# geekieo/collaborative-deep-metric-learning

Measured on AMD Instinct MI355X. Metric: triplets/sec, higher is better.
Workload: dtype f32 values as 3 exact bf16 planes (hi + mid + lo == the f32 value), 6 bf16-MFMA plane products per f32 product, f32 accumulate

## Files before the change

### __graft_entry__.py

```python
import glob
import os
import subprocess
import sys

ROOT = os.path.dirname(os.path.abspath(__file__))
PKG = os.path.join(ROOT, "collaborative-deep-metric-learning_amd")
CSRC = os.path.join(PKG, "csrc")
LIB = os.path.join(PKG, "lib", "libcdml_hip.so")
if ROOT not in sys.path:
    sys.path.insert(0, ROOT)


def _stale(target, sources):
    if not os.path.exists(target):
        return True
    t = os.path.getmtime(target)
    return any(os.path.getmtime(s) > t for s in sources)


def _ids():
    import importlib.util
    spec = importlib.util.spec_from_file_location("_cdml_lib_ids", os.path.join(PKG, "_lib.py"))
    m = importlib.util.module_from_spec(spec)
    spec.loader.exec_module(m)
    return m.source_id, m.embedded_id


def _compile_objects(srcs, hdrs, objdir, hipcc, flags, force=False):
    from concurrent.futures import ThreadPoolExecutor
    os.makedirs(objdir, exist_ok=True)
    jobs = []
    import re
    for s in srcs:
        o = os.path.join(objdir, os.path.basename(s)[:-4] + ".o")
        inc = [os.path.join(os.path.dirname(s), m) for m in re.findall(r'#include "([^"]+\.hip)"', open(s).read())]
        if force or _stale(o, [s] + inc + hdrs):
            jobs.append([hipcc] + flags + ["-c", "-o", o, s])
    if jobs:
        print("[build] compiling %d of %d sources" % (len(jobs), len(srcs)), flush=True)

        def run(c):
            r = subprocess.run(c + ["-Rpass-analysis=kernel-resource-usage"], cwd=CSRC, stderr=subprocess.PIPE, text=True)
            o = c[c.index("-o") + 1]
            with open(o[:-2] + ".remarks", "w") as f:
                f.write(r.stderr)
            if r.returncode:
                sys.stderr.write("\n".join(ln for ln in r.stderr.splitlines() if "remark:" not in ln)[-4000:] + "\n")
            return r
        with ThreadPoolExecutor(max_workers=min(len(jobs), max(1, (os.cpu_count() or 2) - 1))) as ex:
            for r in ex.map(run, jobs):
                if r.returncode:
                    raise RuntimeError("hipcc failed: " + " ".join(r.args))
    objs = [os.path.join(objdir, os.path.basename(s)[:-4] + ".o") for s in srcs]
    _check_no_scratch(objs)
    return objs


HIPCC_FLAGS = ["--offload-arch=gfx950", "-O3", "-std=c++17", "-fPIC",
               "-Wno-array-bounds"]
NPAIR_KERNELS = ("k_npair", "k_mixed", "k_npdp")
IVF_F16_KERNELS = ("k_ivf_scan_f16", "k_ivf_refine")
IVF_FILTER_KERNELS = ("k_ivf_filter_f32", "k_ivf_filter_f16")
KNN_WRITER_KERNELS = ("k_line_sizes", "k_line_write")
IVF_PQ_KERNELS = ("k_ivf_scan_pq", "k_pq_encode")
IVF_PQR_KERNELS = ("k_ivf_scan_pqr", "k_pqr_encode")


def _check_no_scratch(objs):
    import re
    bad = []
    for o in objs:
        rem = o[:-2] + ".remarks"
        if not os.path.exists(rem):
            continue
        name = None
        for ln in open(rem):
            m = re.search(r"Function Name: (\S+)", ln)
            if m:
                name = m.group(1)
            m = re.search(r"ScratchSize \[bytes/lane\]: (\d+)", ln)
            if m and name and int(m.group(1)) > 0 and any(k in name for k in ("k_gemm",) + NPAIR_KERNELS + IVF_F16_KERNELS
                                                          + IVF_FILTER_KERNELS + KNN_WRITER_KERNELS + IVF_PQ_KERNELS
                                                          + IVF_PQR_KERNELS):
                bad.append("%s: %s bytes of scratch per lane (%s)" % (name, m.group(1), os.path.basename(o)))
    if bad:
        raise RuntimeError("kernels with a scratch frame (GEMMs: spills inside hand-counted vmcnt pipelines; N-pair launches "
                           "(k_npair / k_mixed / k_npdp): spills in bandwidth-bound passes):\n  " + "\n  ".join(bad))


def build(force=False, csrc=None, lib=None, objdir=None):
    variant = csrc is not None
    csrc = csrc or CSRC
    lib = lib or LIB
    objdir = objdir or os.path.join(ROOT, "build", "obj")
    srcs = sorted(glob.glob(os.path.join(csrc, "*.hip")))
    hdrs = glob.glob(os.path.join(csrc, "*.h")) + [os.path.join(ROOT, "include", "cdml.h")] \
        + glob.glob(os.path.join(ROOT, "include", "cdml_*.h"))
    source_id, embedded_id = _ids()
    sid = source_id(csrc, os.path.join(ROOT, "include", "cdml.h"))
    if force or embedded_id(lib) != sid:
        os.makedirs(os.path.dirname(lib), exist_ok=True)
        hipcc = os.environ.get("HIPCC", "/opt/rocm/bin/hipcc")
        flags = HIPCC_FLAGS + ["-I" + CSRC]
        objs = _compile_objects(srcs, hdrs, objdir, hipcc, flags, force)
        idsrc = os.path.join(objdir, "build_id.cpp")
        with open(idsrc, "w") as f:
            f.write('extern "C" const char *cdml_build_id(void) { return "CDML_BUILD_ID=%s"; }\n' % sid)
        subprocess.run([hipcc, "-O1", "-fPIC", "-c", "-o", idsrc[:-4] + ".o", idsrc], check=True)
        objs.append(idsrc[:-4] + ".o")
        cmd = [hipcc, "--offload-arch=gfx950", "-fPIC", "-shared", "-o", lib] + objs
        print("[build]", " ".join(cmd), flush=True)
        subprocess.run(cmd, check=True, cwd=csrc)
    if variant:
        return
    import cdml_amd
    from cdml_amd import _lib
    lib = _lib.load_library()
    assert lib.cdml_version() >= 1000
    for name in list(_lib.SIGNATURES) + list(_lib.SIGNATURES_MIXED) + list(_lib.SIGNATURES_DP) + list(_lib.SIGNATURES_BF16) \
            + list(_lib.SIGNATURES_HARDNEG) + list(_lib.SIGNATURES_WIDE) + list(_lib.SIGNATURES_NEGW) \
            + list(_lib.SIGNATURES_F8) + list(_lib.SIGNATURES_IVF) + list(_lib.SIGNATURES_IVF_F16) \
            + list(_lib.SIGNATURES_IVF_FILTER) + list(_lib.SIGNATURES_KNN_WRITER) + list(_lib.SIGNATURES_IVF_PQ) \
            + list(_lib.SIGNATURES_IVF_PQR):
        getattr(lib, name)
    assert lib.cdml_build_id().decode() == "CDML_BUILD_ID=" + sid
    print("[build] ok:", LIB, "version", lib.cdml_version(), lib.cdml_build_id().decode())


def smoke():
    import numpy as np
    import torch
    build()
    from cdml_amd import engine, train
    from oracle import sampler as osampler, synth as osynth, tower as otower

    dev = torch.device("cuda:0")
    N, F, H, D, B = 512, 96, 200, 32, 128
    table = engine.FeatureTable.synthetic(N, F, seed=0, device=dev)
    feats = osynth.features_philox(0, N, F, 0)
    assert np.array_equal(table.data[:, :F].cpu().numpy(), feats), "table differs"
    pairs_np = osynth.cowatch_pairs(N, 64, seed=0)
    pairs = torch.from_numpy(pairs_np).to(dev)
    idx = osampler.device_triplets_vec(pairs_np, N, 1234, 0, B)
    x = feats[idx.reshape(-1)]
    for precision in ("f32x3", "f32", "f16x2"):
        ts = train.TrainStep(table, pairs, B, hidden_size=H, output_size=D, margin=0.8, mode="uniform",
                             optimizer="adam", base_learning_rate=0.01, device=dev, precision=precision)
        W = [t.detach().cpu().numpy().copy() for t in ts.params.unpadded()]
        ts.step()
        torch.cuda.synchronize()
        assert np.array_equal(ts.idx.view(B, 3).cpu().numpy(), idx), "sampled indices differ"
        fwd, loss, grads = otower.train_step_grads(x, W, 0.8, np.float32)
        e = ts.ws.e[:, :D].cpu().numpy()
        assert np.abs(e - fwd["l2_norm"]).max() < 1e-5, "embeddings differ (%s)" % precision
        assert abs(ts.loss() - float(loss["hinge_loss"])) < 1e-5, "loss differs (%s)" % precision
        gW1 = ts.params.unpadded(grads=True)[0].cpu().numpy()
        assert np.abs(gW1 - grads["dW1"]).max() < 1e-5, "dW1 differs (%s)" % precision
        w1, _, _ = otower.adam_step(W[0], gW1, 0 * W[0], 0 * W[0], 1, 0.01)
        assert np.abs(ts.params.unpadded()[0].cpu().numpy() - w1).max() < 1e-6, "Adam update differs (%s)" % precision
        if precision == "f32x3":
            L = ts.layout
            w1t = ts.ws.W1T[:, :L.Fp].float() + ts.ws.W1T[:, L.Fp:2 * L.Fp].float() + ts.ws.W1T[:, 2 * L.Fp:].float()
            assert torch.equal(w1t, ts.params.W1.t()), "weight planes differ from the master weights"
        if precision == "f16x2":
            L, sw = ts.layout, ts.ws.scales.w1
            w1t = (ts.ws.W1T[:, :L.Fp].double() + ts.ws.W1T[:, L.Fp:2 * L.Fp].double()) / sw
            assert (w1t - ts.params.W1.t().double()).abs().max().item() <= 2.0 ** -22 * ts.params.W1.abs().max().item(), \
                "fp16 weight planes differ from the master weights"
        print("[smoke] %s ok: loss %.6f (oracle %.6f)" % (precision, ts.loss(), float(loss["hinge_loss"])))


if __name__ == "__main__":
    build(force="--force" in sys.argv)
    if "--smoke" in sys.argv:
        smoke()
```

### collaborative-deep-metric-learning_amd/_lib.py

```python
import ctypes as C
import os

_HERE = os.path.dirname(os.path.abspath(__file__))
_LIB_NAME = "libcdml_hip.so"


class CdmlError(RuntimeError):

    def __init__(self, code, message):
        super().__init__(f"cdml status {code}: {message}")
        self.code = code


def lib_path():
    return os.environ.get("CDML_LIB_PATH") or os.path.join(_HERE, "lib", _LIB_NAME)


def source_id(csrc=None, header=None):
    import glob
    import hashlib
    csrc = csrc or os.path.join(_HERE, "csrc")
    header = header or os.path.join(os.path.dirname(_HERE), "include", "cdml.h")
    files = sorted(glob.glob(os.path.join(csrc, "*.hip")) + glob.glob(os.path.join(csrc, "*.h")))
    if not files or not os.path.exists(header):
# ... 116 lines not shown
    "cdml_gather_rows_x3": (_i, [_p, _i64, _i64, _p, _i, _i, _i, _p, _i64, _p, _p]),
    "cdml_sample_gather_x3k": (_i, [_i, _p, _i64, _u64, _u64, _p, _i, _i64, _i64, _p, _i64, _i64, _i,
                                    _p, _p, _p, _i64, _i, _i64, _i64, _p, _p, _i64, _p]),
    "cdml_split_f32_bf16x3": (_i, [_p, _i64, _i, _i, _p, _i64, _i64, _i, _p]),
    "cdml_gemm_bf16x3_workspace": (_sz, [_i, _i, _i, _i, _i]),
    "cdml_gemm_bf16x3_nt": (_i, [_i, _p, _i64, _i64, _p, _i64, _i64, _i, _i, _i, _i, _p, _i64, _i64, _p, _p, _i64, _f,
                                 _p, _p, _sz, _p]),
    "cdml_gemm_bf16x3_tn": (_i, [_p, _i64, _i64, _p, _i64, _i64, _i, _i, _i, _i, _p, _i64, _p, _f, _p, _p, _sz, _p]),
    "cdml_split_f32_f16x2": (_i, [_p, _i64, _i, _i, _p, _i64, _i64, _i, _f, _p]),
    "cdml_gemm_f16x2_workspace": (_sz, [_i, _i, _i, _i]),
    "cdml_gemm_f16x2_nt": (_i, [_i, _p, _i64, _i64, _p, _i64, _i64, _i, _i, _i, _p, _i64, _i64, _p, _p, _i64, _f, _f, _f,
                                _p, _sz, _p]),
    "cdml_gemm_f16x2_tn": (_i, [_p, _i64, _i64, _p, _i64, _i64, _i, _i, _i, _p, _i64, _f, _p, _f, _p, _sz, _p]),
    "cdml_interleave8_bf16x3": (_i, [_p, _i64, _i64, _i, _i, _p, _p]),
    "cdml_gemm_bf16x3_tnk": (_i, [_p, _i, _i, _p, _i, _i, _i, _i, _i, _p, _i64, _p, _p, _sz, _p]),
    "cdml_transpose_to_bf16": (_i, [_i, _p, _i64, _i, _i, _p, _i64, _p]),
    "cdml_cast_f32_bf16": (_i, [_p, _i64, _i, _i, _p, _i64, _p]),
    "cdml_colsum_workspace_floats": (_sz, [_i, _i]),
    "cdml_colsum": (_i, [_i, _p, _i64, _i, _i, _p, _p, _p]),
    "cdml_fill_uniform_table_f16": (_i, [_p, _i64, _i64, _i, _i64, _u64, _p]),
    "cdml_gather_rows_f16": (_i, [_p, _i64, _i64, _i64, _p, _i, _i, _p, _i64, _p, _p]),
    "cdml_ew_combine": (_i, [_i, _p, _i64, _p, _i64, _i, _i, _p, _i64, _p]),
    "cdml_ew_fusion_bwd": (_i, [_i, _p, _i64, _p, _i64, _p, _i64, _i, _i, _f, _p, _i64, _p, _i64, _p]),
    "cdml_lrelu_bwd": (_i, [_p, _i64, _p, _i64, _i, _i, _f, _p, _i64, _p]),
    "cdml_adam_step": (_i, [_p, _p, _p, _p, _i64, _f, _p, _f, _f, _f, _i64, _p, _i, _p, _p]),
    "cdml_adam_matrix_bf16": (_i, [_p, _p, _p, _p, _i, _i, _f, _p, _f, _f, _f, _i64, _p, _p, _i64, _p, _i64,
                                   _p, _p, _p, _p, _i, _i, _p, _p]),
    "cdml_adam_matrix_planes": (_i, [_p, _p, _p, _p, _i, _i, _f, _p, _f, _f, _f, _i64, _p, _p, _i64, _i64, _p, _i64, _i64,
                                     _p, _p, _p, _p, _i, _i, _p, _p]),
    "cdml_adam_matrix_h2": (_i, [_p, _p, _p, _p, _i, _i, _f, _p, _f, _f, _f, _i64, _p, _p, _i64, _i64, _p, _i64, _i64, _f,
                                 _p, _p, _p, _p, _i, _i, _p, _p]),
    "cdml_table_adam_rows": (_i, [_p, _i64, _i64, _i64, _i, _p, _i, _p, _i64, _p, _p, _p, _p, _f, _f, _p, _f, _f, _f,
                                  _i64, _p, _p]),
    "cdml_grad_prepare": (_i, [_p, _p, _i64, _f, _f, _p, _p, _p]),
    "cdml_momentum_step": (_i, [_p, _p, _p, _i64, _f, _p, _f, _i, _p]),
    "cdml_lars_scratch_floats": (_sz, []),
    "cdml_lars_step": (_i, [_p, _p, _p, _i64, _f, _p, _f, _f, _f, _f, _p, _p]),
    "cdml_lars_multi_scratch_floats": (_sz, []),
    "cdml_lars_multi": (_i, [_p, _p, _p, _p, _p, _i, _f, _p, _f, _f, _f, _f, _p, _p, _p, _p, _p]),
    "cdml_lars_multi_norms": (_i, [_p, _p, _p, _p, _i, _p, _p]),
    "cdml_lars_matrix": (_i, [_p, _p, _p, _p, _p, _i, _i, _i, _i, _i, _f, _p, _f, _f, _f, _f, _p, _p, _p, _i64, _i64, _p,
                              _i64, _i64, _i, _p, _p, _p]),
    "cdml_momentum_matrix": (_i, [_p, _p, _p, _i, _i, _f, _p, _f, _i, _p, _i64, _i64, _p, _i64, _i64, _i, _p, _p, _p, _i,
                                  _p, _p, _p]),
    "cdml_lars_matrix_h2": (_i, [_p, _p, _p, _p, _p, _i, _i, _i, _i, _i, _f, _p, _f, _f, _f, _f, _p, _p, _p, _i64, _i64, _p,
                                 _i64, _i64, _f, _p, _p, _p]),
    "cdml_momentum_matrix_h2": (_i, [_p, _p, _p, _i, _i, _f, _p, _f, _i, _p, _i64, _i64, _p, _i64, _i64, _f, _p, _p, _p, _i,
                                     _p, _p, _p]),
}

SIGNATURES_MIXED = {
    "cdml_npair_mixed_workspace": (_sz, [_i, _i]),
    "cdml_npair_mixed_stats": (_i, [_p, _i64, _p, _i, _i64, _i64, _p, _i, _p, _f, _p, _f, _i, _p, _p, _p, _sz, _p]),
    "cdml_npair_mixed_grad_x3": (_i, [_p, _i64, _p, _i, _i64, _i64, _p, _i, _p, _f, _p, _f, _i, _p, _p, _i64, _i64, _p]),
    "cdml_npair_mixed_grad_f32": (_i, [_p, _i64, _p, _i, _i64, _i64, _p, _i, _p, _f, _p, _f, _i, _p, _p, _i64, _p]),
    "cdml_npair_mixed_split_x3": (_i, [_p, _i64, _i, _i, _p, _i64, _i64, _p, _i64, _i64, _p, _i64, _i64, _i64, _p]),
}

SIGNATURES_DP = {
    "cdml_npair_dp_workspace": (_sz, [_i, _i]),
    "cdml_npair_dp_local_stats": (_i, [_p, _i64, _p, _i, _i, _i, _f, _i, _p, _p, _p, _sz, _p]),
    "cdml_npair_dp_col_fold": (_i, [_p, _i, _i, _p, _p]),
    "cdml_npair_dp_stats": (_i, [_p, _i64, _i, _i, _i, _f, _i, _p, _p, _p, _sz, _p]),
    "cdml_npair_dp_grad_x3": (_i, [_p, _i64, _p, _i, _i, _i, _f, _i, _p, _p, _p, _i64, _i64, _p]),
    "cdml_npair_dp_grad_f32": (_i, [_p, _i64, _p, _i, _i, _i, _f, _i, _p, _p, _p, _i64, _p]),
    "cdml_npair_dp_pos_fold": (_i, [_p, _i64, _i, _i, _i, _p, _i64, _p]),
}

SIGNATURES_BF16 = {
    "cdml_npair_operands_bf16": (_i, [_p, _i64, _i, _i, _p, _i64, _p, _i64, _p, _i64, _p]),
    "cdml_npair_grad_bf16": (_i, [_p, _i64, _p, _i, _f, _i, _p, _p, _i64, _p]),
    "cdml_npair_logq_grad_bf16": (_i, [_p, _i64, _p, _i, _p, _f, _i, _p, _p, _i64, _p]),
    "cdml_npair_memory_grad_bf16": (_i, [_p, _i64, _p, _i, _i64, _p, _i, _f, _i, _p, _p, _i64, _p]),
    "cdml_npair_memory_logq_grad_bf16": (_i, [_p, _i64, _p, _i, _i64, _p, _p, _i, _f, _i, _p, _p, _i64, _p]),
    "cdml_npair_memory_push_bf16": (_i, [_p, _i64, _p, _i, _i, _u64, _p, _i64, _i, _p, _i64, _p, _p, _i64, _p, _i64, _p]),
}

SIGNATURES_HARDNEG = {
    "cdml_sample_listed": (_i, [_p, _i64, _i64, _u64, _u64, _p, _i, _i64, _i64, _p, _i64, _i, _u64, _p, _p, _p]),
    "cdml_sample_gather_listed": (_i, [_p, _i64, _u64, _u64, _p, _i, _i64, _i64, _p, _i64, _i64, _i, _p, _i64, _i, _u64,
                                       _p, _p, _p, _i64, _i, _i64, _i64, _i64, _p, _p]),
    "cdml_sample_gather_listed_x3": (_i, [_p, _i64, _u64, _u64, _p, _i, _i64, _i64, _p, _i64, _i64, _i, _p, _i64, _i, _u64,
                                          _p, _p, _p, _i64, _i, _i64, _i64, _i64, _p, _p, _i64, _p]),
    "cdml_sample_gather_listed_f16": (_i, [_p, _i64, _u64, _u64, _p, _i, _i64, _i64, _p, _i64, _i64, _i, _p, _i64, _i, _u64,
                                           _p, _p, _p, _i64, _i, _i64, _i64, _i64, _p, _p]),
}

SIGNATURES_NEGW = {
    "cdml_sample_weighted": (_i, [_p, _i64, _i64, _u64, _u64, _p, _i, _i64, _i64, _p, _i64, _p, _i, _p, _p, _p]),
    "cdml_sample_gather_weighted": (_i, [_p, _i64, _u64, _u64, _p, _i, _i64, _i64, _p, _i64, _i64, _i, _p, _i64, _p, _i,
                                         _p, _p, _p, _i64, _i, _i64, _i64, _i64, _p, _p]),
    "cdml_sample_gather_weighted_x3": (_i, [_p, _i64, _u64, _u64, _p, _i, _i64, _i64, _p, _i64, _i64, _i, _p, _i64, _p, _i,
                                            _p, _p, _p, _i64, _i, _i64, _i64, _i64, _p, _p, _i64, _p]),
    "cdml_sample_gather_weighted_f16": (_i, [_p, _i64, _u64, _u64, _p, _i, _i64, _i64, _p, _i64, _i64, _i, _p, _i64, _p, _i,
                                             _p, _p, _p, _i64, _i, _i64, _i64, _i64, _p, _p]),
    "cdml_npair_mixed_stats_nb": (_i, [_p, _i64, _p, _i, _i64, _i64, _p, _i, _p, _p, _p, _f, _i, _p, _p, _p, _sz, _p]),
    "cdml_npair_mixed_grad_x3_nb": (_i, [_p, _i64, _p, _i, _i64, _i64, _p, _i, _p, _p, _p, _f, _i, _p, _p, _i64, _i64, _p]),
    "cdml_npair_mixed_grad_f32_nb": (_i, [_p, _i64, _p, _i, _i64, _i64, _p, _i, _p, _p, _p, _f, _i, _p, _p, _i64, _p]),
    "cdml_negw_bias": (_i, [_p, _i64, _p, _i, _f, _p, _p]),
}

SIGNATURES_WIDE = {
    "cdml_gemm_bf16x3_tn_kb": (_i, [_p, _i64, _i64, _p, _i, _i, _i, _i, _i, _p, _i64, _p, _p, _sz, _p]),
}

SIGNATURES_F8 = {
    "cdml_sample_gather_f8": (_i, [_i, _p, _i64, _u64, _u64, _p, _i, _i64, _i64, _p, _i64, _i64, _i,
                                   _p, _p, _p, _i64, _i, _i64, _i64, _p, _p]),
    "cdml_sample_gather_listed_f8": (_i, [_p, _i64, _u64, _u64, _p, _i, _i64, _i64, _p, _i64, _i64, _i, _p, _i64, _i, _u64,
                                          _p, _p, _p, _i64, _i, _i64, _i64, _i64, _p, _p]),
    "cdml_sample_gather_weighted_f8": (_i, [_p, _i64, _u64, _u64, _p, _i, _i64, _i64, _p, _i64, _i64, _i, _p, _i64, _p, _i,
                                            _p, _p, _p, _i64, _i, _i64, _i64, _i64, _p, _p]),
    "cdml_gather_rows_f8": (_i, [_p, _i64, _i64, _i64, _p, _i, _i, _p, _i64, _p, _p]),
    "cdml_quantize_rows_f8_f32": (_i, [_p, _i64, _i64, _i, _p, _i64, _i64, _p, _p]),
    "cdml_quantize_rows_f8_f16": (_i, [_p, _i64, _i64, _i, _p, _i64, _i64, _p, _p]),
}

SIGNATURES_IVF = {
    "cdml_ivf_centroid_sums": (_i, [_p, _i64, _p, _p, _i, _i, _p, _i64, _p]),
    "cdml_ivf_scan_f32": (_i, [_p, _i64, _i, _p, _p, _p, _p, _i64, _p, _i, _p, _i, _p, _p]),
    "cdml_ivf_merge": (_i, [_p, _p, _p, _p, _i, _i, _p, _p, _p, _p, _i, _p, _p, _p]),
}

SIGNATURES_IVF_F16 = {
    "cdml_ivf_scan_f16": (_i, [_p, _i64, _i, _p, _p, _p, _p, _i64, _p, _i, _p, _i, _p, _p]),
    "cdml_ivf_refine": (_i, [_p, _i64, _i, _p, _i64, _i64, _i, _p, _i, _i, _p, _p, _p]),
}

_IVF_FILTER_ARGS = [_p, _i64, _i, _p, _p, _p, _p, _p, _p, _i64, _p, _p, _p, _i, _p, _i, _p, _i, _p]
SIGNATURES_IVF_FILTER = {
    "cdml_ivf_filter_f32": (_i, _IVF_FILTER_ARGS),
    "cdml_ivf_filter_f16": (_i, list(_IVF_FILTER_ARGS)),
}

SIGNATURES_KNN_WRITER = {
    "cdml_f32_shortest": (_i, [_f, C.c_char_p]),
    "cdml_knn_line_sizes": (_i, [_p, _i64, _p, _i64, _i64, _i, _i, _p, _i64, _i64, _p, _p, _p]),
    "cdml_knn_line_write": (_i, [_p, _i64, _p, _i64, _i64, _i, _i, _p, _p, _i64, _i64, _p, _p, _i64, _p]),
}

SIGNATURES_IVF_PQ = {
    "cdml_pq_encode": (_i, [_p, _i64, _i64, _p, _i, _i, _p, _i64, _p, _i64, _p]),
    "cdml_pq_lut": (_i, [_p, _i64, _i, _p, _i, _i, _p, _p]),
    "cdml_ivf_pq_tile": (_i, [_i, _p, _p]),
    "cdml_ivf_scan_pq": (_i, [_p, _i, _p, _p, _p, _p, _i64, _p, _i, _p, _i, _p, _p]),
}

SIGNATURES_IVF_PQR = {
    "cdml_pqr_encode": (_i, [_p, _i64, _i64, _p, _i64, _i, _p, _p, _i, _i, _p, _i64, _p, _i64, _p]),
    "cdml_ivf_slot_dots": (_i, [_p, _i64, _i, _p, _i64, _i, _p, _p, _i, _p, _p]),
    "cdml_ivf_scan_pqr": (_i, [_p, _i, _p, _p, _p, _p, _p, _i64, _p, _i, _p, _i, _p, _p]),
}

_lib = None


def load_library():
    global _lib
    if _lib is not None:
        return _lib
    path = lib_path()
    if not os.path.exists(path):
        raise CdmlError(-2, f"{path} not found: build it with "
                            f"`python -c 'import __graft_entry__ as g; g.build()'` "
                            f"(there is no CPU fallback)")
    import torch
    lib = C.CDLL(path)
    for name, (res, args) in (list(SIGNATURES.items()) + list(SIGNATURES_MIXED.items()) + list(SIGNATURES_DP.items())
                               + list(SIGNATURES_BF16.items()) + list(SIGNATURES_HARDNEG.items()) + list(SIGNATURES_WIDE.items())
                               + list(SIGNATURES_NEGW.items()) + list(SIGNATURES_F8.items()) + list(SIGNATURES_IVF.items())
                               + list(SIGNATURES_IVF_F16.items()) + list(SIGNATURES_IVF_FILTER.items())
                               + list(SIGNATURES_KNN_WRITER.items()) + list(SIGNATURES_IVF_PQ.items())
                               + list(SIGNATURES_IVF_PQR.items())):
        fn = getattr(lib, name)
        fn.restype = res
        fn.argtypes = args
    want = source_id()
    if want is not None and not os.environ.get("CDML_LIB_PATH") and os.environ.get("CDML_ALLOW_STALE_LIB") != "1":
        have = lib.cdml_build_id().decode()
        if have != "CDML_BUILD_ID=" + want:
            raise CdmlError(-2, f"{path} was built from other sources ({have}; this tree is {want}): rebuild it with "
                                f"`python -c 'import __graft_entry__ as g; g.build()'`")
    _lib = lib
    return lib


def call(name, *args):
    lib = load_library()
    rc = getattr(lib, name)(*args)
    if rc != 0:
        raise CdmlError(rc, lib.cdml_last_error().decode("utf-8", "replace"))
    return rc
```

### collaborative-deep-metric-learning_amd/csrc/gemm_bf16.h

```cpp
#pragma once
#include "common.h"

namespace cdml {

using bf16 = __bf16;

enum { BE_BIAS_LRELU_BF16 = 0, BE_BIAS_LRELU_F32 = 1, BE_MASK_BF16 = 2, BE_F32 = 3, BE_BIAS_LRELU_BF16_BITS = 4,
       BE_MASKBITS_BF16 = 5,
       BE_BIAS_LRELU_X3 = 6, BE_MASK_X3 = 7,
       BE_ROWBIAS_LRELU_X3 = 8,
       BE_BIAS_LRELU_X3_BITS = 9, BE_MASKBITS_X3 = 10,
       BE_MINE_X3 = 11,
       BE_MASKBITS_X3_KI = 12,
       BE_KNN_X3 = 13,
       BE_RANK_X3 = 14 };

struct alignas(16) MineCand { float out_d; int out_c; float in_d; int in_c; };

struct BArgs {
  const bf16 *A; int64_t lda;
  const bf16 *B; int64_t ldb;
  void *C; int64_t ldc;
  const float *bias;
  const bf16 *aux; int64_t ldaux;
  float alpha;
  int M, N, K;
  int k_per_split;
  int64_t slab_stride;
  int tiles_m, tiles_n;
  float *colsum_partial;
  uint8_t *mask_out; int64_t ldmask;
  int aux_bits;
  int x3_tpp;
  int x3_products;
  int64_t x3_plane_a, x3_plane_b, x3_plane_c;
  int grid_tiles, narrow_first;
  int stagger_lead;
  int c_kint;
  const float *mine_sqn; const int32_t *mine_ids; const float *mine_dp; MineCand *mine_out; int64_t mine_ld;
  const float *knn_qsq, *knn_bsq, *knn_tau; int32_t *knn_cnt; uint2 *knn_cand; int knn_cap, knn_col0, knn_n_valid;
  const float *rank_qsq, *rank_tau; const int32_t *rank_pos, *rank_self; int32_t *rank_cnt; float *rank_tau_out;
  float out_scale, c_scale;
};

bool gemm_bf16_256_usable(int M, int N, int K, int64_t lda, int64_t ldb);
int launch_gemm_bf16_256(const BArgs &g, int epilogue, int splits, hipStream_t stream);
int launch_gemm_bf16_256_x3(const BArgs &g, bool tn, int epilogue, int splits, hipStream_t stream);
int launch_gemm_f16x2_256(const BArgs &g, bool tn, int epilogue, int splits, hipStream_t stream);
int launch_gemm_f16x2_mine(const BArgs &g, hipStream_t stream);
int launch_gemm_f16x2_knn(const BArgs &g, hipStream_t stream);
int launch_gemm_x3_mine(const BArgs &g, hipStream_t stream);
int launch_gemm_x3_knn(const BArgs &g, hipStream_t stream);
int launch_gemm_x3_rank(const BArgs &g, hipStream_t stream);
int launch_gemm_f16x2_rank(const BArgs &g, hipStream_t stream);
int launch_gemm_x3_tnk(const BArgs &g, int splits, hipStream_t stream);
int launch_gemm_x3_tnkb(const BArgs &g, int splits, hipStream_t stream);

bool gemm_bf16_k256_usable(int M, int N, int K, int64_t lda, int64_t ldb, int64_t ldc, int64_t ldaux, bool has_aux);
int launch_gemm_bf16_k256(const BArgs &g, hipStream_t stream);

bool gemm_bf16_tn_usable(int M, int N, int K, int64_t lda, int64_t ldb);
int launch_gemm_bf16_tn(const BArgs &g, int splits, hipStream_t stream);

size_t gemm_bf16_tn2_workspace(int M1, int N1, int M2, int N2, int K);
int launch_gemm_bf16_tn2(const BArgs &g1, const BArgs &g2, float *db1, float *db2, void *workspace,
                         size_t workspace_bytes, hipStream_t stream);

}
```

### collaborative-deep-metric-learning_amd/csrc/gemm_bf16_256.hip

```cpp
#include "gemm_tile.h"
#include <stdlib.h>

#ifndef CDML_BF16_MFMA_DEFAULT
#define CDML_BF16_MFMA_DEFAULT 16
#endif

namespace cdml {
namespace {

template <class V>
__device__ __forceinline__ void run_tile(const BArgs &g, const int tm, const int m0, const int n0, const int k_begin,
                                         const int n_ktiles, void *c_base, const int64_t c_ld, const int c_row0,
                                         const int c_col0, float *cs_row, const int64_t cs_grp_stride,
                                         unsigned char *smem) {
  constexpr bool TN = V::TN, S16 = V::S16, X3 = V::X3, F6 = V::F6, NTCS = V::NTCS, NARROW = V::NARROW, WIDEB = V::WIDEB;
  constexpr int EPI = V::EPI;
  constexpr bool KIA = V::KIA, KIB = V::KIB, kSwap = V::kSwap, kR6 = V::kR6, kFast6 = V::kFast6;
  constexpr bool kRowBias = V::kRowBias, kBiasEpi = V::kBiasEpi, kMaskEpi = V::kMaskEpi, kPlanes = V::kPlanes;
  const int t = threadIdx.x;
  const int lane = t & 63;
  const int wave = __builtin_amdgcn_readfirstlane(t >> 6);
  const int grp = wave >> 2, wc = wave & 3;
  const int l31 = lane & 31, h = lane >> 5;

  const int k_rows = X3 ? g.x3_tpp * kTileK : g.K;
  const i32x4 srd_a = make_srd(g.A, KIA ? 3 * g.x3_plane_a * 2 : (int64_t)(TN ? k_rows : g.M) * g.lda * 2);
  const i32x4 srd_b = make_srd(g.B, KIB ? 3 * g.x3_plane_b * 2 : (int64_t)(TN ? k_rows : g.N) * g.ldb * 2);

  uint32_t va[2], vb[2];
#pragma unroll
  for (int i = 0; i < 2; ++i) {
    if constexpr (!TN) {
      const int r = (wave * 2 + i) * 8 + (lane >> 3);
      const int sc = (lane & 7) ^ ((r >> 1) & 7);
      const int row_a = NARROW ? r : (r >> 6) * 128 + (r & 63);
      const int col_b = (r >> 5) * 64 + (r & 31);
      va[i] = (uint32_t)(((int64_t)(m0 + row_a) * g.lda + sc * 8) * 2);
      vb[i] = (uint32_t)(((int64_t)(n0 + col_b) * g.ldb + sc * 8) * 2);
    } else {
      const int pc = wave * 2 + i;
      const int r = pc * 4 + (lane >> 4);
      const int sc = (lane & 15) ^ (((r & 3) << 2) | ((r >> 2) & 3));
      if constexpr (KIA) va[i] = (uint32_t)(((int64_t)(pc >> 1) * g.lda + (int64_t)(m0 + (pc & 1) * 64 + lane) * 8) * 2);
      else va[i] = (uint32_t)(((int64_t)r * g.lda + m0 + sc * 8) * 2);
      if constexpr (KIB) vb[i] = (uint32_t)(((int64_t)(pc >> 1) * g.ldb + (int64_t)(n0 + (pc & 1) * 64 + lane) * 8) * 2);
      else vb[i] = (uint32_t)(((int64_t)r * g.ldb + n0 + sc * 8) * 2);
    }
  }
  const uint32_t d_a = TN ? 256u : (uint32_t)(64 * g.lda * 2), d_b = TN ? 256u : (uint32_t)(32 * g.ldb * 2);
  const uint32_t lds_piece = __builtin_amdgcn_readfirstlane(lds_off(smem) + wave * 2048);

  const bool x3_kmajor = X3 && g.x3_products > 0;
  const float x3_inv = X3 ? __builtin_bit_cast(float, __builtin_amdgcn_readfirstlane(__builtin_bit_cast(
                                int, 1.0f / (float)(x3_kmajor ? g.x3_products : g.x3_tpp)))) : 0.f;
  const int x3_t0 = k_begin / kTileK;
  auto x3_div = [&](int v) { return __builtin_amdgcn_readfirstlane((int)(((float)v + 0.5f) * x3_inv)); };
  auto x3_where = [&](int v, int &sgm, int &w) {
    const int qd = x3_div(v);
    const int rem = v - qd * (x3_kmajor ? g.x3_products : g.x3_tpp);
    sgm = x3_kmajor ? rem : qd;
    w = x3_kmajor ? qd : rem;
  };
  auto x3_segment = [&](int v) { int sgm, w; x3_where(v, sgm, w); return sgm; };
  auto stage = [&](int img, int hh, int tile, int buf) {
    int64_t k_elems;
    if constexpr (X3) {
      int sgm, w;
      x3_where(x3_t0 + tile, sgm, w);
      const int plane = ((img == 0 ? 0x120100 : 0x102010) >> (4 * sgm)) & 3;
      k_elems = (int64_t)w * kTileK * (TN ? (img == 0 ? g.lda : g.ldb) : 1) + plane * (img == 0 ? g.x3_plane_a : g.x3_plane_b);
    } else {
      k_elems = (int64_t)(k_begin + tile * kTileK) * (TN ? (img == 0 ? g.lda : g.ldb) : 1);
    }
    const uint32_t kb = tile < n_ktiles ? (uint32_t)(k_elems * 2) : 0x80000000u;
#pragma unroll
    for (int i = 0; i < 2; ++i) {
      const uint32_t voff = (img == 0 ? va[i] + hh * d_a : vb[i] + hh * d_b) + kb;
      dma(img == 0 ? srd_a : srd_b, voff, lds_piece + i * 1024 + img * (4 * IMG) + buf * (2 * IMG) + hh * IMG);
    }
  };

  const bool x3_run = X3 && !F6 && x3_kmajor;
  auto x3_pack = [&](int v) { const int qd = x3_div(v); return qd * 8 + (v - qd * g.x3_products); };
  auto x3_step = [&](int pos) { return ((pos & 7) + 1 == g.x3_products) ? (pos & ~7) + 8 : pos + 1; };
  int xp_c = 0, xp_a = 0, xp_b = 0;
  if (x3_run) { xp_c = x3_pack(x3_t0); xp_a = x3_pack(x3_t0 + 1); xp_b = x3_pack(x3_t0 + 2); }
  auto stage_pw = [&](int img, int hh, int plane, int w, int tile, int buf) {
    const int64_t k_elems = (int64_t)w * kTileK * (TN ? (img == 0 ? g.lda : g.ldb) : 1) +
                            plane * (img == 0 ? g.x3_plane_a : g.x3_plane_b);
    const uint32_t kb = tile < n_ktiles ? (uint32_t)(k_elems * 2) : 0x80000000u;
#pragma unroll
    for (int i = 0; i < 2; ++i) {
      const uint32_t voff = (img == 0 ? va[i] + hh * d_a : vb[i] + hh * d_b) + kb;
      dma(img == 0 ? srd_a : srd_b, voff, lds_piece + i * 1024 + img * (4 * IMG) + buf * (2 * IMG) + hh * IMG);
    }
  };

  const int x = (l31 >> 1) & 7;
  const unsigned char *a_rd = smem + (grp * 64 + l31) * 128;
  const unsigned char *b_rd = smem + 4 * IMG + (wc * 32 + l31) * 128;
  int sw[4];
#pragma unroll
  for (int ks = 0; ks < 4; ++ks) sw[ks] = ((2 * ks + h) ^ x) * 16;
  const int tq = (lane >> 2) & 3, tp = lane & 3, tmb = (lane >> 4) & 1;
  auto tr_off = [&](int c0, int sh) {
    const int row = 8 * h + 4 * sh + tq;
    const int swz = (tq << 2) | ((2 * h + sh) & 3);
    return 256 * row + 16 * ((c0 + tmb * 2 + (tp >> 1)) ^ swz) + 8 * (tp & 1);
  };
  int ta[2][2], tb[2];
#pragma unroll
  for (int sh = 0; sh < 2; ++sh) {
    ta[0][sh] = tr_off(grp * 8, sh);
    ta[1][sh] = tr_off(grp * 8 + 4, sh);
    tb[sh] = tr_off(wc * 4, sh);
  }
  auto tr_read = [&](const unsigned char *img, int off0, int off1) {
    const bf16x4 lo = __builtin_amdgcn_ds_read_tr16_b64_v4bf16(
        (__attribute__((address_space(3))) bf16x4 *)(img + off0));
    const bf16x4 hi = __builtin_amdgcn_ds_read_tr16_b64_v4bf16(
        (__attribute__((address_space(3))) bf16x4 *)(img + off1));
    return __builtin_shufflevector(lo, hi, 0, 1, 2, 3, 4, 5, 6, 7);
  };
  auto read_a = [&](int buf, int hh, int mi, int ks) {
    if constexpr (!TN)
      return *reinterpret_cast<const bf16x8 *>(a_rd + buf * (2 * IMG) + hh * IMG + mi * 4096 + sw[ks]);
    else
      return tr_read(smem + buf * (2 * IMG) + hh * IMG + ks * 4096, ta[mi][0], ta[mi][1]);
  };
  auto read_b = [&](int buf, int hh, int ks) {
    if constexpr (!TN)
      return *reinterpret_cast<const bf16x8 *>(b_rd + buf * (2 * IMG) + hh * IMG + sw[ks]);
    else
      return tr_read(smem + 4 * IMG + buf * (2 * IMG) + hh * IMG + ks * 4096, tb[0], tb[1]);
  };

  const int l15 = lane & 15, q16 = lane >> 4;
  const unsigned char *a16_rd = smem + (grp * 64 + l15) * 128;
  const unsigned char *b16_rd = smem + 4 * IMG + (wc * 32 + l15) * 128;
  const int sw16[2] = {((q16) ^ ((l15 >> 1) & 7)) * 16, ((4 + q16) ^ ((l15 >> 1) & 7)) * 16};
  auto tr_off16 = [&](int c0, int sh) {
    const int row = 8 * q16 + 4 * sh + tq;
    const int swz = (tq << 2) | ((2 * q16 + sh) & 3);
    return 256 * row + 16 * ((c0 + (tp >> 1)) ^ swz) + 8 * (tp & 1);
  };
  int ta16[4][2], tb16[2][2];
#pragma unroll
  for (int sh = 0; sh < 2; ++sh) {
#pragma unroll
    for (int rb = 0; rb < 4; ++rb) ta16[rb][sh] = tr_off16((WIDEB ? (grp * 2 + (wc >> 1)) * 4 : grp * 8) + 2 * rb, sh);
#pragma unroll
    for (int cb = 0; cb < 2; ++cb) tb16[cb][sh] = tr_off16(wc * 4 + 2 * cb, sh);
  }
  auto read_a16 = [&](int buf, int hh, int rb, int ks2) {
    if constexpr (!TN)
      return *reinterpret_cast<const bf16x8 *>(a16_rd + buf * (2 * IMG) + hh * IMG + rb * 2048 + sw16[ks2]);
    else
      return tr_read(smem + buf * (2 * IMG) + hh * IMG + ks2 * 8192, ta16[rb][0], ta16[rb][1]);
  };
  auto read_b16 = [&](int buf, int hh, int cb, int ks2) {
    if constexpr (!TN)
      return *reinterpret_cast<const bf16x8 *>(b16_rd + buf * (2 * IMG) + hh * IMG + cb * 2048 + sw16[ks2]);
    else
      return tr_read(smem + 4 * IMG + buf * (2 * IMG) + hh * IMG + ks2 * 8192, tb16[cb][0], tb16[cb][1]);
  };

  f32x16 acc[S16 ? 1 : 4][S16 ? 1 : 2];
  f32x4 acc16[S16 ? 8 : 1][S16 ? 4 : 1];
#pragma unroll
  for (int i = 0; i < (S16 ? 1 : 4); ++i)
#pragma unroll
    for (int j = 0; j < (S16 ? 1 : 2); ++j)
#pragma unroll
      for (int r = 0; r < 16; ++r) acc[i][j][r] = 0.f;
#pragma unroll
  for (int i = 0; i < (S16 ? 8 : 1); ++i)
#pragma unroll
    for (int j = 0; j < (S16 ? 4 : 1); ++j) acc16[i][j] = f32x4{0.f, 0.f, 0.f, 0.f};
  bf16x8 fbx[WIDEB ? 16 : 1];
  float csw[WIDEB ? 8 : 1];
#pragma unroll
  for (int i = 0; i < (WIDEB ? 8 : 1); ++i) csw[i] = 0.f;
  bf16x8 fa[2][4], fb0[4], fb1[4];

  float cs[2] = {0.f, 0.f};
  float cs16[4] = {0.f, 0.f, 0.f, 0.f};
  const bool cs_on = (TN || (NTCS && X3 && S16)) && cs_row != nullptr;
  const int cs_period = 2 * g.tiles_m;
  const int cs_owner = (2 * tm + grp + cs_period - (k_begin / kTileK) % cs_period) % cs_period;
  auto dot_sum = [&](const bf16x8 &f, float acc) {
#ifdef CDML_F16X2
    const half8 hf = __builtin_bit_cast(half8, f);
    const half2v one = {(_Float16)1.0f, (_Float16)1.0f};
#pragma unroll
    for (int e = 0; e < 4; ++e) {
      const half2v pr = {hf[2 * e], hf[2 * e + 1]};
      acc = __builtin_amdgcn_fdot2(pr, one, acc, false);
    }
#else
    using bf16x2 = __attribute__((ext_vector_type(2))) __bf16;
    const bf16x2 one = {(__bf16)1.0f, (__bf16)1.0f};
#pragma unroll
    for (int e = 0; e < 4; ++e) {
      const bf16x2 pr = {f[2 * e], f[2 * e + 1]};
      acc = __builtin_amdgcn_fdot2_f32_bf16(pr, one, acc, false);
    }
#endif
    return acc;
  };
  int cs_left = __builtin_amdgcn_readfirstlane(cs_on ? cs_owner : 0x40000000);
  auto frag_sum = [&](const bf16x8 &f) {
    float s = 0.f;
#pragma unroll
    for (int e = 0; e < 8; ++e) s += (float)f[e];
    return s;
  };

  auto pin_a = [&]() {
    if constexpr (WIDEB)
      asm volatile("" : "+v"(fa[0][0]), "+v"(fa[0][1]), "+v"(fa[1][0]), "+v"(fa[1][1]));
    else
      asm volatile("" : "+v"(fa[0][0]), "+v"(fa[0][1]), "+v"(fa[0][2]), "+v"(fa[0][3]),
                        "+v"(fa[1][0]), "+v"(fa[1][1]), "+v"(fa[1][2]), "+v"(fa[1][3]));
  };
  auto pin_b = [&]() {
    if constexpr (WIDEB)
      asm volatile("" : "+v"(fbx[0]), "+v"(fbx[1]), "+v"(fbx[2]), "+v"(fbx[3]), "+v"(fbx[4]), "+v"(fbx[5]), "+v"(fbx[6]), "+v"(fbx[7]),
                        "+v"(fbx[8]), "+v"(fbx[9]), "+v"(fbx[10]), "+v"(fbx[11]), "+v"(fbx[12]), "+v"(fbx[13]), "+v"(fbx[14]), "+v"(fbx[15]));
    else
      asm volatile("" : "+v"(fb0[0]), "+v"(fb0[1]), "+v"(fb0[2]), "+v"(fb0[3]),
                        "+v"(fb1[0]), "+v"(fb1[1]), "+v"(fb1[2]), "+v"(fb1[3]));
  };
  auto load_b16 = [&](auto rd) {
    if constexpr (WIDEB) {
#pragma unroll
      for (int hh = 0; hh < 2; ++hh)
#pragma unroll
        for (int cb = 0; cb < 4; ++cb)
#pragma unroll
          for (int ks2 = 0; ks2 < 2; ++ks2) fbx[hh * 8 + cb * 2 + ks2] = rd(hh, cb, ks2);
    } else {
#pragma unroll
      for (int cb = 0; cb < 2; ++cb)
#pragma unroll
        for (int ks2 = 0; ks2 < 2; ++ks2) {
          fb0[2 * cb + ks2] = rd(0, cb, ks2);
          fb1[2 * cb + ks2] = rd(1, cb, ks2);
        }
    }
  };
  auto load_a16 = [&](auto rd) {
#pragma unroll
    for (int ks2 = 0; ks2 < 2; ++ks2)
#pragma unroll
      for (int rb = 0; rb < (WIDEB ? 2 : 4); ++rb) fa[ks2][rb] = rd(rb, ks2);
  };
  auto sum_b16 = [&](auto add) {
    if constexpr (WIDEB) {
#pragma unroll
      for (int hc = 0; hc < 8; ++hc)
#pragma unroll
        for (int ks2 = 0; ks2 < 2; ++ks2) csw[hc] = add(fbx[hc * 2 + ks2], csw[hc]);
    } else {
#pragma unroll
      for (int cb = 0; cb < 2; ++cb)
#pragma unroll
        for (int ks2 = 0; ks2 < 2; ++ks2) {
          cs16[cb] = add(fb0[2 * cb + ks2], cs16[cb]);
          cs16[2 + cb] = add(fb1[2 * cb + ks2], cs16[2 + cb]);
        }
    }
  };
  auto mfma16 = [&](const int r0) {
    __builtin_amdgcn_s_setprio(1);
    if constexpr (WIDEB) {
#pragma unroll
      for (int ks2 = 0; ks2 < 2; ++ks2)
#pragma unroll
        for (int rb = 0; rb < 2; ++rb)
#pragma unroll
          for (int hh = 0; hh < 2; ++hh)
#pragma unroll
            for (int cb = 0; cb < 4; ++cb)
              acc16[r0 + 2 * hh + rb][cb] = CDML_MFMA16(fa[ks2][rb], fbx[hh * 8 + cb * 2 + ks2], acc16[r0 + 2 * hh + rb][cb]);
    } else {
#pragma unroll
      for (int ks2 = 0; ks2 < 2; ++ks2)
#pragma unroll
        for (int rb = 0; rb < 4; ++rb)
#pragma unroll
          for (int cb = 0; cb < 2; ++cb) {
            if constexpr (kSwap) {
              acc16[r0 + rb][cb] = CDML_MFMA16(fb0[2 * cb + ks2], fa[ks2][rb], acc16[r0 + rb][cb]);
              acc16[r0 + rb][2 + cb] = CDML_MFMA16(fb1[2 * cb + ks2], fa[ks2][rb], acc16[r0 + rb][2 + cb]);
            } else {
              acc16[r0 + rb][cb] = CDML_MFMA16(fa[ks2][rb], fb0[2 * cb + ks2], acc16[r0 + rb][cb]);
              acc16[r0 + rb][2 + cb] = CDML_MFMA16(fa[ks2][rb], fb1[2 * cb + ks2], acc16[r0 + rb][2 + cb]);
            }
          }
    }
    __builtin_amdgcn_s_setprio(0);
  };
  auto do_tile2_s16 = [&](const int buf, const int tile) {
    load_b16([&](int hh, int cb, int ks2) { return read_b16(buf, hh, cb, ks2); });
    load_a16([&](int rb, int ks2) { return read_a16(buf, 0, rb, ks2); });
    if (X3 && x3_run) {
      const int pl = (0x120100 >> (4 * (xp_a & 7))) & 3;
      stage_pw(0, 0, pl, xp_a >> 3, tile + 1, buf ^ 1);
      stage_pw(0, 1, pl, xp_a >> 3, tile + 1, buf ^ 1);
    } else {
      stage(0, 0, tile + 1, buf ^ 1);
      stage(0, 1, tile + 1, buf ^ 1);
    }
    asm volatile("s_waitcnt vmcnt(8)" ::: "memory");
    pin_b();
    pin_a();
    const bool cs_mine = cs_left == 0;
    cs_left = cs_mine ? cs_period - 1 : cs_left - 1;
    if (cs_mine && (!X3 || ((0xB >> (x3_run ? (xp_c & 7) : x3_segment(x3_t0 + tile))) & 1))) sum_b16(dot_sum);
    CDML_BARRIER();
    mfma16(0);
    CDML_BARRIER();
    load_a16([&](int rb, int ks2) { return read_a16(buf, 1, rb, ks2); });
    if (X3 && x3_run) {
      const int pl = (0x102010 >> (4 * (xp_b & 7))) & 3;
      stage_pw(1, 0, pl, xp_b >> 3, tile + 2, buf);
      stage_pw(1, 1, pl, xp_b >> 3, tile + 2, buf);
    } else {
      stage(1, 0, tile + 2, buf);
      stage(1, 1, tile + 2, buf);
    }
    asm volatile("s_waitcnt vmcnt(6)" ::: "memory");
    pin_a();
    CDML_BARRIER();
    mfma16(4);
    CDML_BARRIER();
    if (X3 && x3_run) { xp_c = x3_step(xp_c); xp_a = x3_step(xp_a); xp_b = x3_step(xp_b); }
  };
  auto step6 = [&](auto Sc, const int tile, const int w) {
    constexpr int S = decltype(Sc)::value;
    constexpr int PA[6] = {0, 0, 1, 0, 2, 1}, PB[6] = {0, 1, 0, 2, 0, 1};
    constexpr int buf = S & 1;
    constexpr bool skip_a = (S >= 1 && S <= 4) && PA[(S + 1) % 6] == PA[(S + 5) % 6];
    constexpr bool skip_b = (S <= 3) && PB[(S + 2) % 6] == PB[S];
    constexpr int SP = (S + 5) % 6;
    constexpr bool b_next_issued = !((SP <= 3) && PB[(SP + 2) % 6] == PB[SP]);
    load_b16([&](int hh, int cb, int ks2) { return read_b16(buf, hh, cb, ks2); });
    load_a16([&](int rb, int ks2) { return read_a16(buf, 0, rb, ks2); });
    if constexpr (!skip_a) {
      stage_pw(0, 0, PA[(S + 1) % 6], w + (S == 5 ? 1 : 0), tile + 1, buf ^ 1);
      stage_pw(0, 1, PA[(S + 1) % 6], w + (S == 5 ? 1 : 0), tile + 1, buf ^ 1);
    }
    asm volatile("s_waitcnt vmcnt(%0)" :: "n"(4 * (int)b_next_issued + 4 * (int)!skip_a) : "memory");
    pin_b();
    pin_a();
    if (cs_on && ((0xB >> S) & 1) && (tile % cs_period) == cs_owner)
      sum_b16([&](const bf16x8 &f, float sum) { return sum + frag_sum(f); });
    CDML_BARRIER();
    mfma16(0);
    CDML_BARRIER();
    load_a16([&](int rb, int ks2) { return read_a16(buf, 1, rb, ks2); });
    if constexpr (!skip_b) {
      stage_pw(1, 0, PB[(S + 2) % 6], w + (S >= 4 ? 1 : 0), tile + 2, buf);
      stage_pw(1, 1, PB[(S + 2) % 6], w + (S >= 4 ? 1 : 0), tile + 2, buf);
    }
    asm volatile("s_waitcnt vmcnt(%0)" :: "n"(2 * (int)!skip_a + 4 * (int)!skip_b) : "memory");
    pin_a();
    CDML_BARRIER();
    mfma16(4);
    CDML_BARRIER();
  };
  auto do_tile2 = [&](const int buf, const int tile) {
#pragma unroll
    for (int ks = 0; ks < 4; ++ks) fb0[ks] = read_b(buf, 0, ks);
#pragma unroll
    for (int ks = 0; ks < 4; ++ks) fb1[ks] = read_b(buf, 1, ks);
#pragma unroll
    for (int mi = 0; mi < 2; ++mi)
#pragma unroll
      for (int ks = 0; ks < 4; ++ks) fa[mi][ks] = read_a(buf, 0, mi, ks);
    stage(0, 0, tile + 1, buf ^ 1);
    stage(0, 1, tile + 1, buf ^ 1);
    asm volatile("s_waitcnt vmcnt(8)" ::: "memory");
    pin_b();
    pin_a();
    if (TN && cs_on && (tile % cs_period) == cs_owner && (!X3 || ((0xB >> x3_segment(x3_t0 + tile)) & 1))) {
#pragma unroll
      for (int ks = 0; ks < 4; ++ks) {
        cs[0] += frag_sum(fb0[ks]);
        cs[1] += frag_sum(fb1[ks]);
      }
    }
    CDML_BARRIER();
    __builtin_amdgcn_s_setprio(1);
#pragma unroll
    for (int ks = 0; ks < 4; ++ks)
#pragma unroll
      for (int mi = 0; mi < 2; ++mi) {
        acc[mi][0] = __builtin_amdgcn_mfma_f32_32x32x16_bf16(fa[mi][ks], fb0[ks], acc[mi][0], 0, 0, 0);
        acc[mi][1] = __builtin_amdgcn_mfma_f32_32x32x16_bf16(fa[mi][ks], fb1[ks], acc[mi][1], 0, 0, 0);
      }
    __builtin_amdgcn_s_setprio(0);
    CDML_BARRIER();
#pragma unroll
    for (int mi = 0; mi < 2; ++mi)
#pragma unroll
      for (int ks = 0; ks < 4; ++ks) fa[mi][ks] = read_a(buf, 1, mi, ks);
    stage(1, 0, tile + 2, buf);
    stage(1, 1, tile + 2, buf);
    asm volatile("s_waitcnt vmcnt(6)" ::: "memory");
    pin_a();
    CDML_BARRIER();
    __builtin_amdgcn_s_setprio(1);
#pragma unroll
    for (int ks = 0; ks < 4; ++ks)
#pragma unroll
      for (int mi = 0; mi < 2; ++mi) {
        acc[2 + mi][0] = __builtin_amdgcn_mfma_f32_32x32x16_bf16(fa[mi][ks], fb0[ks], acc[2 + mi][0], 0, 0, 0);
        acc[2 + mi][1] = __builtin_amdgcn_mfma_f32_32x32x16_bf16(fa[mi][ks], fb1[ks], acc[2 + mi][1], 0, 0, 0);
      }
    __builtin_amdgcn_s_setprio(0);
    CDML_BARRIER();
  };

  if constexpr (kR6) {
    constexpr int kPer = kF16 ? 3 : 6;
    const int n_per = n_ktiles / kPer;
    if (n_per > 0) {
      const int w_first = x3_t0 / kPer, w_last = w_first + n_per - 1;
      const uint32_t ws_a = KIA ? (uint32_t)(8 * g.lda * 2) : TN ? (uint32_t)(kTileK * g.lda * 2) : (uint32_t)(kTileK * 2);
      const uint32_t ws_b = KIB ? (uint32_t)(8 * g.ldb * 2) : TN ? (uint32_t)(kTileK * g.ldb * 2) : (uint32_t)(kTileK * 2);
      const uint32_t ps_a = (uint32_t)(g.x3_plane_a * 2), ps_b = (uint32_t)(g.x3_plane_b * 2);
      const unsigned char *b16r = smem + 6 * IMG + (wc * 32 + l15) * 128;
      int ta_w2[4][2], tb_w[2][2];
      if constexpr (TN && !KIA) {
#pragma unroll
        for (int sh = 0; sh < 2; ++sh)
#pragma unroll
          for (int rb = 0; rb < (WIDEB ? 2 : 4); ++rb) {
            ta_w2[rb][sh] = ta16[rb][sh] + 4 * IMG;
            asm volatile("" : "+v"(ta_w2[rb][sh]));
          }
      }
      if constexpr (TN && !KIB) {
#pragma unroll
        for (int sh = 0; sh < 2; ++sh)
#pragma unroll
          for (int cb = 0; cb < 2; ++cb) {
            tb_w[cb][sh] = tb16[cb][sh] + 6 * IMG;
            asm volatile("" : "+v"(tb_w[cb][sh]));
          }
      }
      const unsigned char *ka_rd = smem + (q16 * 128 + grp * 64 + l15) * 16;
      const unsigned char *kb_rd = smem + 6 * IMG + (q16 * 128 + (WIDEB ? (wc & 1) * 64 : wc * 32) + l15) * 16;
      auto rd_a = [&](int slot, int hh, int rb, int ks2) {
        if constexpr (!TN)
          return *reinterpret_cast<const bf16x8 *>(a16_rd + slot * 2 * IMG + hh * IMG + rb * 2048 + sw16[ks2]);
        else if constexpr (KIA)
          return *reinterpret_cast<const bf16x8 *>(ka_rd + slot * 2 * IMG + hh * IMG + ks2 * 8192 + rb * 256);
        else if (slot < 2)
          return tr_read(smem + slot * 2 * IMG + hh * IMG + ks2 * 8192, ta16[rb][0], ta16[rb][1]);
        else
          return tr_read(smem + hh * IMG + ks2 * 8192, ta_w2[rb][0], ta_w2[rb][1]);
      };
      auto rd_b = [&](int slot, int hh, int cb, int ks2) {
        if constexpr (!TN)
          return *reinterpret_cast<const bf16x8 *>(b16r + slot * 2 * IMG + hh * IMG + cb * 2048 + sw16[ks2]);
        else if constexpr (KIB)
          return *reinterpret_cast<const bf16x8 *>(kb_rd + slot * 2 * IMG + hh * IMG + ks2 * 8192 + cb * 256);
        else
          return tr_read(smem + slot * 2 * IMG + hh * IMG + ks2 * 8192, tb_w[cb][0], tb_w[cb][1]);
      };
      uint32_t va_h1[2] = {va[0] + d_a, va[1] + d_a}, vb_h1[2] = {vb[0] + d_b, vb[1] + d_b};
      auto issue = [&](int img, int pl, int hh, int slot, uint32_t kw) {
        const uint32_t so = (img == 0 ? pl * ps_a : pl * ps_b) + kw + ((img == 0 ? KIA : KIB) ? hh * 2048u : TN ? hh * 256u : 0u);
        const uint32_t dst = lds_piece + (img == 0 ? 0 : 6 * IMG) + slot * 2 * IMG + hh * IMG;
        const bool h1 = !TN && hh == 1;
        dma_s(img == 0 ? srd_a : srd_b, img == 0 ? (h1 ? va_h1[0] : va[0]) : (h1 ? vb_h1[0] : vb[0]), so, dst);
        dma_s(img == 0 ? srd_a : srd_b, img == 0 ? (h1 ? va_h1[1] : va[1]) : (h1 ? vb_h1[1] : vb[1]), so, dst + 1024);
      };
      if constexpr (kF16) {
      auto phase3 = [&](auto phc, auto parc, const uint32_t kwb_c, const uint32_t kwa_n, const uint32_t kwb_n, const bool own) {
        constexpr int PH = decltype(phc)::value, PAR = decltype(parc)::value;
        constexpr int S = PH >> 1, HALF = PH & 1;
        constexpr int PA3[3] = {0, 1, 0}, PB3[3] = {0, 0, 1};
        constexpr int SLOT_A3[2][2] = {{0, 1}, {2, 1}};
        constexpr int sa = SLOT_A3[PAR][PA3[S]];
        constexpr bool rdB = HALF == 0 && (S == 0 || S == 2);
        if constexpr (rdB) {
          constexpr int sb = PB3[S];
          load_b16([&](int hh, int cb, int ks2) { return rd_b(sb, hh, cb, ks2); });
        }
        load_a16([&](int rb, int ks2) { return rd_a(sa, HALF, rb, ks2); });
        constexpr int SCH = TN ? 0 : 1;
        if constexpr (SCH == 0 && PH == 0) { issue(1, 1, 0, 1, kwb_c); issue(1, 1, 1, 1, kwb_c); }
        if constexpr (SCH == 0 && PH == 1) { issue(0, 0, 0, SLOT_A3[PAR ^ 1][0], kwa_n); }
        if constexpr (SCH == 0 && PH == 2) { issue(0, 0, 1, SLOT_A3[PAR ^ 1][0], kwa_n); }
        if constexpr (SCH == 0 && PH == 3) { issue(1, 0, 0, 0, kwb_n); }
        if constexpr (SCH == 0 && PH == 4) { issue(1, 0, 1, 0, kwb_n); issue(0, 1, 0, 1, kwa_n); }
        if constexpr (SCH == 0 && PH == 5) { issue(0, 1, 1, 1, kwa_n); }
        if constexpr (SCH == 1 && PH == 0) { issue(1, 1, 0, 1, kwb_c); }
        if constexpr (SCH == 1 && PH == 1) { issue(1, 1, 1, 1, kwb_c); issue(0, 0, 0, SLOT_A3[PAR ^ 1][0], kwa_n); }
        if constexpr (SCH == 1 && PH == 2) { issue(0, 0, 1, SLOT_A3[PAR ^ 1][0], kwa_n); }
        if constexpr (SCH == 1 && PH == 3) { issue(1, 0, 0, 0, kwb_n); issue(1, 0, 1, 0, kwb_n); }
        if constexpr (SCH == 1 && PH == 4) { issue(0, 1, 0, 1, kwa_n); }
        if constexpr (SCH == 1 && PH == 5) { issue(0, 1, 1, 1, kwa_n); }
        constexpr int VM3[2][6] = {{8, 8, 8, 6, 10, 4}, {6, 8, 8, 8, 10, 4}};
        asm volatile("s_waitcnt vmcnt(%0)" :: "n"(VM3[SCH][PH]) : "memory");
        if constexpr (rdB) pin_b();
        pin_a();
        if constexpr (rdB) {
          if (own) sum_b16(dot_sum);
        }
        CDML_BARRIER();
        mfma16(4 * HALF);
        CDML_BARRIER();
      };
      auto period3 = [&](auto parc, const int w, const bool own) {
        const int wn = min(w + 1, w_last);
        const uint32_t kwb_c = (uint32_t)w * ws_b, kwa_n = (uint32_t)wn * ws_a, kwb_n = (uint32_t)wn * ws_b;
        unroll<6>([&](auto phc) { phase3(phc, parc, kwb_c, kwa_n, kwb_n, own); });
      };
      {
        const uint32_t ka3 = (uint32_t)w_first * ws_a, kb3 = (uint32_t)w_first * ws_b;
        issue(0, 0, 0, 0, ka3); issue(0, 0, 1, 0, ka3);
        issue(1, 0, 0, 0, kb3); issue(1, 0, 1, 0, kb3);
        issue(0, 1, 0, 1, ka3); issue(0, 1, 1, 1, ka3);
        asm volatile("s_waitcnt vmcnt(4)" ::: "memory");
      }
      CDML_BARRIER();
      if (grp == 1) CDML_BARRIER();
      int cs_wait3 = __builtin_amdgcn_readfirstlane(cs_on ? (2 * tm + grp + cs_period - w_first % cs_period) % cs_period : 0x40000000);
      for (int w = w_first;;) {
        bool own = cs_wait3 == 0;
        cs_wait3 = own ? cs_period - 1 : cs_wait3 - 1;
        period3(std::integral_constant<int, 0>{}, w, own);
        if (++w > w_last) break;
        own = cs_wait3 == 0;
        cs_wait3 = own ? cs_period - 1 : cs_wait3 - 1;
        period3(std::integral_constant<int, 1>{}, w, own);
        if (++w > w_last) break;
      }
      } else if constexpr (!NARROW) {
      auto phase = [&](auto phc, auto parc, const uint32_t kwa_c, const uint32_t kwb_c, const uint32_t kwa_n,
                       const uint32_t kwb_n, const bool own) {
        constexpr int PH = decltype(phc)::value, PAR = decltype(parc)::value;
        constexpr int S = PH >> 1, HALF = PH & 1;
        constexpr int PA[6] = {0, 1, 2, 0, 1, 0}, PB[6] = {0, 0, 0, 1, 1, 2};
        constexpr int SLOT_A[2][3] = {{0, 1, 2}, {2, 1, 0}};
        constexpr int sa = SLOT_A[PAR][PA[S]];
        constexpr bool rdB = HALF == 0 && (S == 0 || S == 3 || S == 5);
        if constexpr (rdB) {
          constexpr int sb = (PB[S] & 1) ^ PAR;
          load_b16([&](int hh, int cb, int ks2) { return rd_b(sb, hh, cb, ks2); });
        }
        load_a16([&](int rb, int ks2) { return rd_a(sa, HALF, rb, ks2); });
        if constexpr (PH == 0) issue(0, 2, 1, SLOT_A[PAR][2], kwa_c);
        if constexpr (PH == 1) issue(1, 1, 0, 1 ^ PAR, kwb_c);
        if constexpr (PH == 2) issue(1, 1, 1, 1 ^ PAR, kwb_c);
        if constexpr (PH == 3) issue(1, 2, 0, PAR, kwb_c);
        if constexpr (PH == 4) issue(1, 2, 1, PAR, kwb_c);
        if constexpr (PH == 5) issue(0, 0, 0, SLOT_A[PAR ^ 1][0], kwa_n);
        if constexpr (PH == 6) issue(0, 0, 1, SLOT_A[PAR ^ 1][0], kwa_n);
        if constexpr (PH == 7) issue(1, 0, 0, PAR ^ 1, kwb_n);
        if constexpr (PH == 8) issue(1, 0, 1, PAR ^ 1, kwb_n);
        if constexpr (PH == 9) issue(0, 1, 0, 1, kwa_n);
        if constexpr (PH == 10) issue(0, 1, 1, 1, kwa_n);
        if constexpr (PH == 11) issue(0, 2, 0, SLOT_A[PAR ^ 1][2], kwa_n);
        constexpr int VM[12] = {8, 8, 8, 8, 8, 6, 8, 10, 12, 10, 12, 6};
        asm volatile("s_waitcnt vmcnt(%0)" :: "n"(VM[PH]) : "memory");
        if constexpr (rdB) pin_b();
        pin_a();
        if constexpr (rdB) {
          if constexpr (WIDEB) {
            if (own && (wc >> 1) == 0) sum_b16(dot_sum);
          } else {
            if (own) sum_b16(dot_sum);
          }
        }
        CDML_BARRIER();
        mfma16(4 * HALF);
        CDML_BARRIER();
      };
      auto period = [&](auto parc, const int w, const bool own) {
        const int wn = min(w + 1, w_last);
        const uint32_t kwa_c = (uint32_t)w * ws_a, kwb_c = (uint32_t)w * ws_b;
        const uint32_t kwa_n = (uint32_t)wn * ws_a, kwb_n = (uint32_t)wn * ws_b;
        unroll<12>([&](auto phc) { phase(phc, parc, kwa_c, kwb_c, kwa_n, kwb_n, own); });
      };
      {
        const uint32_t ka = (uint32_t)w_first * ws_a, kb_ = (uint32_t)w_first * ws_b;
        issue(0, 0, 0, 0, ka); issue(0, 0, 1, 0, ka);
        issue(1, 0, 0, 0, kb_); issue(1, 0, 1, 0, kb_);
        issue(0, 1, 0, 1, ka); issue(0, 1, 1, 1, ka);
        issue(0, 2, 0, 2, ka);
        asm volatile("s_waitcnt vmcnt(6)" ::: "memory");
      }
      CDML_BARRIER();
      if (grp == 1) CDML_BARRIER();
      int cs_wait = __builtin_amdgcn_readfirstlane(cs_on ? (2 * tm + grp + cs_period - w_first % cs_period) % cs_period : 0x40000000);
      for (int w = w_first;;) {
        bool own = cs_wait == 0;
        cs_wait = own ? cs_period - 1 : cs_wait - 1;
        period(std::integral_constant<int, 0>{}, w, own);
        if (++w > w_last) break;
        own = cs_wait == 0;
        cs_wait = own ? cs_period - 1 : cs_wait - 1;
        period(std::integral_constant<int, 1>{}, w, own);
        if (++w > w_last) break;
      }
      } else {
      auto rd_an = [&](int slot, int rb, int ks2) {
        return *reinterpret_cast<const bf16x8 *>(a16_rd + slot * IMG + rb * 2048 + sw16[ks2]);
      };
      const unsigned char *b16n = smem + 4 * IMG + (wc * 32 + l15) * 128;
      auto rd_bn = [&](int slot, int hh, int cb, int ks2) {
        return *reinterpret_cast<const bf16x8 *>(b16n + slot * 2 * IMG + hh * IMG + cb * 2048 + sw16[ks2]);
      };
      auto issue_n = [&](int img, int pl, int hh, int slot, uint32_t kw) {
        const uint32_t so = (img == 0 ? pl * ps_a : pl * ps_b) + kw;
        const uint32_t dst = lds_piece + (img == 0 ? slot * IMG : 4 * IMG + slot * 2 * IMG + hh * IMG);
        const bool h1 = hh == 1;
        dma_s(img == 0 ? srd_a : srd_b, img == 0 ? va[0] : (h1 ? vb_h1[0] : vb[0]), so, dst);
        dma_s(img == 0 ? srd_a : srd_b, img == 0 ? va[1] : (h1 ? vb_h1[1] : vb[1]), so, dst + 1024);
      };
      auto phase_n = [&](auto sc, auto parc, const uint32_t kwb_c, const uint32_t kwa_n, const uint32_t kwb_n) {
        constexpr int S = decltype(sc)::value, PAR = decltype(parc)::value;
        constexpr int PA[6] = {0, 1, 2, 0, 1, 0}, PB[6] = {0, 0, 0, 1, 1, 2};
        constexpr int NSLOT_A[2][3] = {{0, 1, 2}, {3, 2, 1}};
        constexpr bool rdB = S == 0 || S == 3 || S == 5;
        if constexpr (rdB) load_b16([&](int hh, int cb, int ks2) { return rd_bn(PB[S], hh, cb, ks2); });
        load_a16([&](int rb, int ks2) { return rd_an(NSLOT_A[PAR][PA[S]], rb, ks2); });
        if constexpr (S == 0) { issue_n(1, 2, 0, 2, kwb_c); issue_n(1, 2, 1, 2, kwb_c); }
        if constexpr (S == 1) { issue_n(1, 0, 0, 0, kwb_n); issue_n(0, 0, 0, NSLOT_A[PAR ^ 1][0], kwa_n); }
        if constexpr (S == 2) { issue_n(1, 0, 1, 0, kwb_n); }
        if constexpr (S == 3) { issue_n(0, 1, 0, NSLOT_A[PAR ^ 1][1], kwa_n); }
        if constexpr (S == 4) { issue_n(1, 1, 0, 1, kwb_n); issue_n(1, 1, 1, 1, kwb_n); }
        if constexpr (S == 5) { issue_n(0, 2, 0, NSLOT_A[PAR ^ 1][2], kwa_n); }
        constexpr int NVM[6] = {10, 8, 10, 12, 12, 8};
        asm volatile("s_waitcnt vmcnt(%0)" :: "n"(NVM[S]) : "memory");
        if constexpr (rdB) pin_b();
        pin_a();
        CDML_BARRIER();
        mfma16(0);
        CDML_BARRIER();
      };
      auto period_n = [&](auto parc, const int w) {
        const int wn = min(w + 1, w_last);
        const uint32_t kwb_c = (uint32_t)w * ws_b, kwa_n = (uint32_t)wn * ws_a, kwb_n = (uint32_t)wn * ws_b;
        unroll<6>([&](auto sc) { phase_n(sc, parc, kwb_c, kwa_n, kwb_n); });
      };
      {
        const uint32_t ka = (uint32_t)w_first * ws_a, kb_ = (uint32_t)w_first * ws_b;
        issue_n(1, 0, 0, 0, kb_); issue_n(0, 0, 0, 0, ka);
        issue_n(1, 0, 1, 0, kb_);
        issue_n(0, 1, 0, 1, ka);
        issue_n(1, 1, 0, 1, kb_); issue_n(1, 1, 1, 1, kb_);
        issue_n(0, 2, 0, 2, ka);
        asm volatile("s_waitcnt vmcnt(8)" ::: "memory");
      }
      CDML_BARRIER();
      if (grp == 1) CDML_BARRIER();
      for (int w = w_first;;) {
        period_n(std::integral_constant<int, 0>{}, w);
        if (++w > w_last) break;
        period_n(std::integral_constant<int, 1>{}, w);
        if (++w > w_last) break;
      }
      }
      if (grp == 0) CDML_BARRIER();
      asm volatile("s_waitcnt vmcnt(0)" ::: "memory");
      CDML_BARRIER();
    }
  } else {
  stage(1, 0, 0, 0); stage(1, 1, 0, 0); stage(0, 0, 0, 0); stage(0, 1, 0, 0);
  stage(1, 0, 1, 1); stage(1, 1, 1, 1);
  asm volatile("s_waitcnt vmcnt(6)" ::: "memory");
  CDML_BARRIER();
  if (grp == 1) CDML_BARRIER();
  if constexpr (kFast6) {
    {
      int w = x3_t0 / 6;
      for (int tile = 0; tile < n_ktiles; tile += 6, ++w) {
        step6(std::integral_constant<int, 0>{}, tile, w);
        step6(std::integral_constant<int, 1>{}, tile + 1, w);
        step6(std::integral_constant<int, 2>{}, tile + 2, w);
        step6(std::integral_constant<int, 3>{}, tile + 3, w);
        step6(std::integral_constant<int, 4>{}, tile + 4, w);
        step6(std::integral_constant<int, 5>{}, tile + 5, w);
      }
    }
  } else {
    for (int tile = 0; tile < n_ktiles; tile += 2) {
      if constexpr (S16) {
        do_tile2_s16(0, tile);
        do_tile2_s16(1, tile + 1);
      } else {
        do_tile2(0, tile);
        do_tile2(1, tile + 1);
      }
    }
  }

  if (grp == 0) CDML_BARRIER();
  asm volatile("s_waitcnt vmcnt(0)" ::: "memory");
  CDML_BARRIER();
  }

  if (TN && cs_on && !S16) {
#pragma unroll
    for (int ct = 0; ct < 2; ++ct) {
      const float v = cs[ct] + __shfl_xor(cs[ct], 32, 64);
      if (h == 0) cs_row[grp * cs_grp_stride + ct * 128 + wc * 32 + l31] = v;
    }
  }
  if (!TN && cs_on && S16) {
#pragma unroll
    for (int cbt = 0; cbt < 4; ++cbt) {
      float v = cs16[cbt] + __shfl_xor(cs16[cbt], 16, 64);
      v += __shfl_xor(v, 32, 64);
      if (q16 == 0) cs_row[grp * cs_grp_stride + wc * 64 + (cbt >> 1) * 32 + (cbt & 1) * 16 + l15] = v;
    }
  }
  if (WIDEB && cs_on) {
    if ((wc >> 1) == 0) {
#pragma unroll
      for (int hc = 0; hc < 8; ++hc) {
        float v = csw[hc] + __shfl_xor(csw[hc], 16, 64);
        v += __shfl_xor(v, 32, 64);
        if (q16 == 0) cs_row[grp * cs_grp_stride + (hc >> 2) * 128 + (wc & 1) * 64 + (hc & 3) * 16 + l15] = v;
      }
    }
  }
  if (TN && !WIDEB && cs_on && S16) {
#pragma unroll
    for (int cbt = 0; cbt < 4; ++cbt) {
      float v = cs16[cbt] + __shfl_xor(cs16[cbt], 16, 64);
      v += __shfl_xor(v, 32, 64);
      if (q16 == 0) cs_row[grp * cs_grp_stride + (cbt >> 1) * 128 + wc * 32 + (cbt & 1) * 16 + l15] = v;
    }
  }

  if constexpr (EPI == BE_MINE_X3) {
    int lane_e = lane;
    asm volatile("" : "+v"(lane_e));
    const int l15 = lane_e & 15, q16 = lane_e >> 4;
    const float inf = __builtin_huge_valf();
    const int cbase = n0 + wc * 64 + 4 * q16;
    f32x4 ncv[4];
    i32x4 idv[4];
#pragma unroll
    for (int cb = 0; cb < 4; ++cb) {
      ncv[cb] = *reinterpret_cast<const f32x4 *>(g.mine_sqn + cbase + cb * 16);
      idv[cb] = *reinterpret_cast<const i32x4 *>(g.mine_ids + cbase + cb * 16);
    }
    const int row_base = m0 + grp * 128 + l15;
    float sa8[8], dp8[8];
    int va8[8], vp8[8];
#pragma unroll
    for (int rbb = 0; rbb < 8; ++rbb) {
      const int i = min(row_base + rbb * 16, g.M - 1);
      sa8[rbb] = g.mine_sqn[2 * i];
      dp8[rbb] = g.mine_dp[i];
      va8[rbb] = g.mine_ids[2 * i];
      vp8[rbb] = g.mine_ids[2 * i + 1];
    }
    const float two_s = kF16 ? 2.0f * g.out_scale : 2.0f;
    auto closer = [](float d, int c, float bd, int bc) { return d < bd || (d == bd && c < bc); };
    auto farther = [](float d, int c, float bd, int bc) { return d > bd || (d == bd && c < bc); };
    MineCand *dst = g.mine_out + (int64_t)((n0 / kTileN) * 4 + wc) * g.mine_ld;
#pragma unroll
    for (int rbb = 0; rbb < 8; ++rbb) {
      const float sa = sa8[rbb], dpv = dp8[rbb];
      const int va = va8[rbb], vp = vp8[rbb];
      float od = inf, id_ = -inf;
      int oc = 0x7fffffff, ic = 0x7fffffff;
#pragma unroll
      for (int cb = 0; cb < 4; ++cb)
#pragma unroll
        for (int r = 0; r < 4; ++r) {
          const int c = cbase + cb * 16 + r;
          const float d = (sa + ncv[cb][r]) - two_s * acc16[rbb][cb][r];
          const int vid = idv[cb][r];
          if (vid != va && vid != vp && d > dpv && d < od) { od = d; oc = c; }
        }
#pragma unroll
      for (int off = 16; off < 64; off <<= 1) {
        const float od2 = __shfl_xor(od, off, 64);
        const int oc2 = __shfl_xor(oc, off, 64);
        if (closer(od2, oc2, od, oc)) { od = od2; oc = oc2; }
      }
      if (__ballot(oc == 0x7fffffff) != 0ull) {
#pragma unroll
        for (int cb = 0; cb < 4; ++cb)
#pragma unroll
          for (int r = 0; r < 4; ++r) {
            const int c = cbase + cb * 16 + r;
            const float d = (sa + ncv[cb][r]) - two_s * acc16[rbb][cb][r];
            const int vid = idv[cb][r];
            if (vid != va && vid != vp && d > id_) { id_ = d; ic = c; }
          }
#pragma unroll
        for (int off = 16; off < 64; off <<= 1) {
          const float id2 = __shfl_xor(id_, off, 64);
          const int ic2 = __shfl_xor(ic, off, 64);
          if (farther(id2, ic2, id_, ic)) { id_ = id2; ic = ic2; }
        }
        if (oc != 0x7fffffff) { id_ = -inf; ic = 0x7fffffff; }
      }
      const int i = row_base + rbb * 16;
      if (q16 == 0 && i < g.M) dst[i] = MineCand{od, oc, id_, ic};
    }
    return;
  }

  if constexpr (EPI == BE_KNN_X3) {
    int lane_e = lane;
    asm volatile("" : "+v"(lane_e));
    const int l15 = lane_e & 15, q16 = lane_e >> 4;
    const int cbase = n0 + wc * 64 + 4 * q16;
// ... 765 lines not shown
```

### collaborative-deep-metric-learning_amd/csrc/gemm_bf16x3.hip

```cpp
#include "gemm_bf16.h"
#include "../../include/cdml_x3_wide.h"
#include <stdlib.h>

namespace cdml {
namespace {

using bf16x4 = __attribute__((ext_vector_type(4))) __bf16;
using f32x4 = __attribute__((ext_vector_type(4))) float;
constexpr int kThreads = 256;

__device__ __forceinline__ void split3(float v, bf16 &h, bf16 &m, bf16 &l) {
  h = (bf16)v;
  const float r = v - (float)h;
  m = (bf16)r;
  l = (bf16)(r - (float)m);
}

__global__ void __launch_bounds__(kThreads)
k_split3(const float *__restrict__ src, int64_t lds_, int rows, int cols, bf16 *__restrict__ dst, int64_t ldd,
         int64_t plane) {
  const int c4n = cols >> 2;
  const int64_t total = (int64_t)rows * c4n;
  for (int64_t i = (int64_t)blockIdx.x * blockDim.x + threadIdx.x; i < total; i += (int64_t)gridDim.x * blockDim.x) {
    const int64_t r = i / c4n;
    const int c = (int)(i - r * c4n) * 4;
    const f32x4 v = *reinterpret_cast<const f32x4 *>(src + r * lds_ + c);
    bf16x4 h, m, l;
#pragma unroll
    for (int j = 0; j < 4; ++j) {
      bf16 a, b, c_;
      split3(v[j], a, b, c_);
      h[j] = a; m[j] = b; l[j] = c_;
    }
    bf16 *d = dst + r * ldd + c;
    *reinterpret_cast<bf16x4 *>(d) = h;
    *reinterpret_cast<bf16x4 *>(d + plane) = m;
    *reinterpret_cast<bf16x4 *>(d + 2 * plane) = l;
  }
}

__global__ void __launch_bounds__(kThreads)
k_split3_transpose(const float *__restrict__ src, int64_t lds_, int rows, int cols, bf16 *__restrict__ dst,
                   int64_t ldd, int64_t plane) {
  __shared__ float tile[64][65];
  const int r0 = blockIdx.y * 64, c0 = blockIdx.x * 64;
  const int tx = threadIdx.x & 63, ty = threadIdx.x >> 6;
  for (int j = ty; j < 64; j += 4) {
    const int r = r0 + j, c = c0 + tx;
    tile[j][tx] = (r < rows && c < cols) ? src[(int64_t)r * lds_ + c] : 0.f;
  }
  __syncthreads();
  for (int j = ty; j < 64; j += 4) {
    const int c = c0 + j, r = r0 + tx;
    if (c < cols && r < rows) {
      bf16 h, m, l;
      split3(tile[tx][j], h, m, l);
      bf16 *d = dst + (int64_t)c * ldd + r;
      d[0] = h; d[plane] = m; d[2 * plane] = l;
    }
  }
}

using half4v = __attribute__((ext_vector_type(4))) _Float16;
__device__ __forceinline__ void split2h(float v, float scale, _Float16 &h, _Float16 &l) {
  const float s = __builtin_amdgcn_fmed3f(v * scale, -65504.f, 65504.f);
  h = (_Float16)s;
  l = (_Float16)(s - (float)h);
}

__global__ void __launch_bounds__(kThreads)
k_split2h(const float *__restrict__ src, int64_t lds_, int rows, int cols, _Float16 *__restrict__ dst, int64_t ldd,
          int64_t plane, float scale) {
  const int c4n = cols >> 2;
  const int64_t total = (int64_t)rows * c4n;
  for (int64_t i = (int64_t)blockIdx.x * blockDim.x + threadIdx.x; i < total; i += (int64_t)gridDim.x * blockDim.x) {
    const int64_t r = i / c4n;
    const int c = (int)(i - r * c4n) * 4;
    const f32x4 v = *reinterpret_cast<const f32x4 *>(src + r * lds_ + c);
    half4v h, l;
#pragma unroll
    for (int j = 0; j < 4; ++j) {
      _Float16 a, b;
      split2h(v[j], scale, a, b);
      h[j] = a; l[j] = b;
    }
    _Float16 *d = dst + r * ldd + c;
    *reinterpret_cast<half4v *>(d) = h;
    *reinterpret_cast<half4v *>(d + plane) = l;
  }
}

__global__ void __launch_bounds__(kThreads)
k_split2h_transpose(const float *__restrict__ src, int64_t lds_, int rows, int cols, _Float16 *__restrict__ dst,
                    int64_t ldd, int64_t plane, float scale) {
  __shared__ float tile[64][65];
  const int r0 = blockIdx.y * 64, c0 = blockIdx.x * 64;
  const int tx = threadIdx.x & 63, ty = threadIdx.x >> 6;
  for (int j = ty; j < 64; j += 4) {
    const int r = r0 + j, c = c0 + tx;
    tile[j][tx] = (r < rows && c < cols) ? src[(int64_t)r * lds_ + c] : 0.f;
  }
  __syncthreads();
  for (int j = ty; j < 64; j += 4) {
    const int c = c0 + j, r = r0 + tx;
    if (c < cols && r < rows) {
      _Float16 h, l;
      split2h(tile[tx][j], scale, h, l);
      _Float16 *d = dst + (int64_t)c * ldd + r;
      d[0] = h; d[plane] = l;
    }
  }
}

int grid1d(int64_t n) {
  const int64_t b = (n + kThreads - 1) / kThreads;
  return (int)(b < 1 ? 1 : (b > 65535 * 16 ? 65535 * 16 : b));
}

bool x3_kmajor() {
  const char *e = getenv("CDML_X3_ORDER");
  return !(e && e[0] == 'p');
}

thread_local int tl_slab_steps = 0;
int x3_slab_steps() {
  const char *e = getenv("CDML_X3_SLAB_STEPS");
  return e && atoi(e) >= 12 ? atoi(e) / 6 * 6 : tl_slab_steps;
}

}
}

using namespace cdml;

extern "C" int cdml_split_f32_bf16x3(const float *src, int64_t ld_src, int rows, int cols, uint16_t *dst,
                                     int64_t ld_dst, int64_t plane, int transpose, cdml_stream_t stream) {
  CDML_REQUIRE(src && dst && rows > 0 && cols > 0, CDML_E_BADARG, "split_f32_bf16x3: bad argument");
  const int out_cols = transpose ? rows : cols;
  CDML_REQUIRE(plane >= out_cols && ld_dst >= 2 * plane + out_cols && ld_src >= cols, CDML_E_BADARG,
               "split_f32_bf16x3: planes of %d columns need plane >= %d and ld_dst >= 2 plane + %d", out_cols, out_cols, out_cols);
  hipStream_t s = (hipStream_t)stream;
  if (transpose) {
    hipLaunchKernelGGL(k_split3_transpose, dim3((cols + 63) / 64, (rows + 63) / 64), dim3(kThreads), 0, s, src, ld_src,
                       rows, cols, reinterpret_cast<bf16 *>(dst), ld_dst, plane);
  } else {
    CDML_REQUIRE((cols & 3) == 0 && (ld_src & 3) == 0 && (ld_dst & 3) == 0 && (plane & 3) == 0 && aligned16(src) &&
                     (reinterpret_cast<uintptr_t>(dst) & 7) == 0,
                 CDML_E_ALIGN, "split_f32_bf16x3: columns, strides and plane must be multiples of 4");
    hipLaunchKernelGGL(k_split3, dim3(grid1d((int64_t)rows * (cols / 4))), dim3(kThreads), 0, s, src, ld_src, rows, cols,
                       reinterpret_cast<bf16 *>(dst), ld_dst, plane);
  }
  return check_launch("split_f32_bf16x3");
}

extern "C" int cdml_split_f32_f16x2(const float *src, int64_t ld_src, int rows, int cols, uint16_t *dst, int64_t ld_dst,
                                    int64_t plane, int transpose, float scale, cdml_stream_t stream) {
  CDML_REQUIRE(src && dst && rows > 0 && cols > 0 && scale > 0.f, CDML_E_BADARG, "split_f32_f16x2: bad argument");
  const int out_cols = transpose ? rows : cols;
  CDML_REQUIRE(plane >= out_cols && ld_dst >= plane + out_cols && ld_src >= cols, CDML_E_BADARG,
               "split_f32_f16x2: planes of %d columns need plane >= %d and ld_dst >= plane + %d", out_cols, out_cols, out_cols);
  hipStream_t s = (hipStream_t)stream;
  if (transpose) {
    hipLaunchKernelGGL(k_split2h_transpose, dim3((cols + 63) / 64, (rows + 63) / 64), dim3(kThreads), 0, s, src, ld_src,
                       rows, cols, reinterpret_cast<_Float16 *>(dst), ld_dst, plane, scale);
  } else {
    CDML_REQUIRE((cols & 3) == 0 && (ld_src & 3) == 0 && (ld_dst & 3) == 0 && (plane & 3) == 0 && aligned16(src) &&
                     (reinterpret_cast<uintptr_t>(dst) & 7) == 0,
                 CDML_E_ALIGN, "split_f32_f16x2: columns, strides and plane must be multiples of 4");
    hipLaunchKernelGGL(k_split2h, dim3(grid1d((int64_t)rows * (cols / 4))), dim3(kThreads), 0, s, src, ld_src, rows, cols,
                       reinterpret_cast<_Float16 *>(dst), ld_dst, plane, scale);
  }
  return check_launch("split_f32_f16x2");
}

extern "C" int cdml_x3_slab_steps(int steps) {
  const int prev = tl_slab_steps;
  tl_slab_steps = steps >= 12 ? steps / 6 * 6 : 0;
  return prev;
}

extern "C" size_t cdml_gemm_bf16x3_workspace(int tn, int M, int N, int K, int products) {
  return x3_workspace_bytes(tn, M, N, K, products, tn ? 0 : x3_slab_steps());
}

extern "C" size_t cdml_gemm_f16x2_workspace(int tn, int M, int N, int K) {
  const size_t a = cdml_gemm_bf16x3_workspace(tn, M, N, K, 6), b = cdml_gemm_bf16x3_workspace(tn, M, N, K, 3);
  return a > b ? a : b;
}

namespace cdml {
namespace {
__device__ __forceinline__ void x3_colsum_block(const float *__restrict__ partial, int n_rows, int N, float *__restrict__ out,
                                                int blk, float scale) {
  __shared__ float red[16][17];
  const int cl = threadIdx.x & 15, rl = threadIdx.x >> 4;
  const int c = blk * 16 + cl;
  float s0 = 0.f, s1 = 0.f, s2 = 0.f, s3 = 0.f;
  if (c < N) {
    int r = rl;
    for (; r + 48 < n_rows; r += 64) {
      s0 += partial[(int64_t)r * N + c];
      s1 += partial[(int64_t)(r + 16) * N + c];
      s2 += partial[(int64_t)(r + 32) * N + c];
      s3 += partial[(int64_t)(r + 48) * N + c];
    }
    for (; r < n_rows; r += 16) s0 += partial[(int64_t)r * N + c];
  }
  red[rl][cl] = (s0 + s1) + (s2 + s3);
  __syncthreads();
  if (rl == 0 && c < N) {
    float t = red[0][cl];
#pragma unroll
    for (int j = 1; j < 16; ++j) t += red[j][cl];
    out[c] = t * scale;
  }
}

__global__ void __launch_bounds__(kThreads)
k_x3_sum_slabs(const float *__restrict__ slabs, int64_t slab_stride, int splits, int rows, int N,
               const float *__restrict__ bias, float alpha, float *__restrict__ out, int64_t ldo, int slab_blocks,
               const float *__restrict__ cs_partial, int cs_rows, float *__restrict__ cs_out, float cs_scale) {
  if ((int)blockIdx.x >= slab_blocks) {
    x3_colsum_block(cs_partial, cs_rows, N, cs_out, blockIdx.x - slab_blocks, cs_scale);
    return;
  }
  const int n4 = N >> 2;
  const int64_t total = (int64_t)rows * n4;
  for (int64_t i = (int64_t)blockIdx.x * blockDim.x + threadIdx.x; i < total; i += (int64_t)slab_blocks * blockDim.x) {
    const int64_t r = i / n4;
    const int c = (int)(i - r * n4);
    f32x4 s = reinterpret_cast<const f32x4 *>(slabs)[i];
    for (int z = 1; z < splits; ++z) s += reinterpret_cast<const f32x4 *>(slabs + (int64_t)z * slab_stride)[i];
    if (bias) {
      s += reinterpret_cast<const f32x4 *>(bias)[c];
      s.x = fmaxf(s.x, s.x * alpha); s.y = fmaxf(s.y, s.y * alpha);
      s.z = fmaxf(s.z, s.z * alpha); s.w = fmaxf(s.w, s.w * alpha);
    }
    reinterpret_cast<f32x4 *>(out + r * ldo)[c] = s;
  }
}

int x3_sum_slabs(const char *entry, const char *stage, const BArgs &g, const KSplitPlan &p, const void *slabs, const float *bias,
                 float alpha, float *C, int64_t ldc, float *colsum, float cs_scale, hipStream_t s) {
  const int sb = slabs ? grid1d((int64_t)g.M * g.N / 4) : 0, cb = colsum ? (g.N + 15) / 16 : 0;
  hipLaunchKernelGGL(k_x3_sum_slabs, dim3(sb + cb), dim3(kThreads), 0, s, static_cast<const float *>(slabs), g.slab_stride,
                     p.splits, g.M, g.N, bias, alpha, C, ldc, sb, g.colsum_partial, (int)p.cs_rows, colsum, cs_scale);
  const hipError_t e = hipGetLastError();
  return e == hipSuccess ? CDML_OK : fail(CDML_E_HIP, "%s %s: %s", entry, stage, hipGetErrorString(e));
}

int x3_run_tn(const char *entry, BArgs &g, const KSplitPlan &p, int (*launch)(const BArgs &, int, hipStream_t), float *C, int64_t ldc,
              const float *bias, float alpha, float *colsum, float cs_scale, void *workspace, size_t workspace_bytes, hipStream_t s) {
  CDML_REQUIRE(p.need == 0 || (workspace && workspace_bytes >= p.need && aligned16(workspace)), CDML_E_BADARG,
               "%s: workspace of %zu bytes required (cdml_gemm_bf16x3_workspace)", entry, p.need);
  g.K = p.ktiles * 64;
  g.tiles_m = g.M / 256; g.tiles_n = g.N / 256;
  g.k_per_split = p.per * 64;
  g.slab_stride = (int64_t)g.M * g.N;
  g.C = p.slabs ? workspace : static_cast<void *>(C);
  g.ldc = p.slabs ? g.N : ldc;
  g.colsum_partial = colsum ? reinterpret_cast<float *>(static_cast<char *>(workspace) + p.slab_bytes) : nullptr;
  const int rc = launch(g, p.splits, s);
  if (rc || !(p.slabs || colsum)) return rc;
  return x3_sum_slabs(entry, "combine", g, p, p.slabs ? workspace : nullptr, bias, alpha, C, ldc, colsum, cs_scale, s);
}
}
}

static int gemm_x3_nt_impl(bool f16, float out_scale, float c_scale, int epilogue, const uint16_t *A, int64_t lda, int64_t plane_a,
                           const uint16_t *B, int64_t ldb, int64_t plane_b, int M, int N, int K, int products, void *C,
                           int64_t ldc, int64_t plane_c, const float *bias, const uint16_t *aux,
                           int64_t ldaux, float alpha, float *colsum, void *workspace,
                           size_t workspace_bytes, cdml_stream_t stream) {
  CDML_REQUIRE(A && B && C && M > 0 && N > 0 && K > 0, CDML_E_BADARG, "gemm_bf16x3_nt: bad argument");
  const int np1 = f16 ? 1 : 2;
  CDML_REQUIRE(!f16 || (products == 3 && epilogue != BE_MASKBITS_X3_KI && epilogue != BE_ROWBIAS_LRELU_X3 && !colsum &&
                        out_scale > 0.f && c_scale > 0.f),
               CDML_E_UNSUPPORTED, "gemm_f16x2_nt: epilogues 1, 3, 6, 7, 9, 10, positive scales, no column sums");
  const bool kint_out = epilogue == BE_MASKBITS_X3_KI;
  const bool bits_out = epilogue == BE_BIAS_LRELU_X3_BITS, bits_in = epilogue == BE_MASKBITS_X3 || (kint_out && aux);
  if (bits_out) epilogue = BE_BIAS_LRELU_X3;
  if (bits_in || kint_out) epilogue = BE_MASK_X3;
  CDML_REQUIRE(epilogue == BE_BIAS_LRELU_F32 || epilogue == BE_F32 || epilogue == BE_BIAS_LRELU_X3 || epilogue == BE_MASK_X3 ||
                   epilogue == BE_ROWBIAS_LRELU_X3,
               CDML_E_BADARG, "gemm_bf16x3_nt: epilogue must be 1, 3, 6, 7, 8, 9, 10 or 12");
  CDML_REQUIRE(!(bits_out || bits_in) || (aux && N % 8 == 0 && ldaux >= N / 8), CDML_E_BADARG,
               "gemm_bf16x3_nt: epilogues 9 / 10 need the bitmask in aux (ldaux >= N / 8 bytes)");
  CDML_REQUIRE(products == 3 || products == 6, CDML_E_BADARG, "gemm_bf16x3_nt: products must be 3 or 6");
  CDML_REQUIRE(N % 256 == 0 && K % 64 == 0, CDML_E_UNSUPPORTED,
               "gemm_bf16x3_nt: N must be a multiple of 256 and K of 64, got N=%d K=%d", N, K);
  CDML_REQUIRE(aligned16(A) && aligned16(B) && aligned16(C) && !(lda & 7) && !(ldb & 7) && !(plane_a & 7) && !(plane_b & 7) &&
                   plane_a >= K && plane_b >= K && lda >= np1 * plane_a + K && ldb >= np1 * plane_b + K,
               CDML_E_ALIGN, "gemm_bf16x3_nt: 16-B aligned bases, strides multiples of 8, ld >= 2 plane + K (fp16 form: plane + K)");
  const bool planes_out = epilogue == BE_BIAS_LRELU_X3 || epilogue == BE_MASK_X3 || epilogue == BE_ROWBIAS_LRELU_X3;
  CDML_REQUIRE(kint_out ? (M % 8 == 0 && !(ldc & 7) && ldc >= N && plane_c >= (int64_t)(M / 8) * ldc * 8 &&
                           (int64_t)3 * plane_c * 2 < ((int64_t)1 << 32))
                        : planes_out ? (!(ldc & 7) && !(plane_c & 7) && plane_c >= N && ldc >= np1 * plane_c + N) : (!(ldc & 3) && ldc >= N),
               CDML_E_ALIGN, "gemm_bf16x3_nt: ldc (plane outputs: ldc and plane_c multiples of 8, ldc >= 2 plane_c + N; epilogue 12: M a "
               "multiple of 8, ldc = columns per row group >= N, plane_c >= M ldc)");
  CDML_REQUIRE(epilogue != BE_MASK_X3 || !aux || bits_in || (aligned16(aux) && !(ldaux & 7) && ldaux >= N), CDML_E_ALIGN,
               "gemm_bf16x3_nt: aux must be 16-B aligned with ldaux a multiple of 8");
  CDML_REQUIRE((epilogue != BE_BIAS_LRELU_F32 && epilogue != BE_BIAS_LRELU_X3 && epilogue != BE_ROWBIAS_LRELU_X3) || bias,
               CDML_E_BADARG, "gemm_bf16x3_nt: bias required");
  CDML_REQUIRE(!colsum || (M % 256 == 0 && products == 6 && epilogue == BE_F32), CDML_E_UNSUPPORTED,
               "gemm_bf16x3_nt: colsum (sum over k of B[n][k]) goes with epilogue 3, M a multiple of 256 and six products");
  CDML_REQUIRE(((int64_t)M + 256) * lda * 2 < ((int64_t)1 << 31) && (int64_t)N * ldb * 2 < ((int64_t)1 << 31), CDML_E_UNSUPPORTED,
               "gemm_bf16x3_nt: an operand exceeds the 2 GiB buffer-descriptor range");
  BArgs g{};
  g.A = reinterpret_cast<const bf16 *>(A); g.lda = lda;
  g.B = reinterpret_cast<const bf16 *>(B); g.ldb = ldb;
  g.C = C; g.ldc = ldc; g.bias = bias; g.alpha = alpha;
  g.aux = reinterpret_cast<const bf16 *>(aux); g.ldaux = ldaux;
  if (bits_out) { g.mask_out = reinterpret_cast<uint8_t *>(const_cast<uint16_t *>(aux)); g.ldmask = ldaux; g.aux = nullptr; g.ldaux = 0; }
  g.aux_bits = bits_in ? 1 : 0;
  g.c_kint = kint_out ? 1 : 0;
  g.M = M; g.N = N;
  g.x3_tpp = K / 64; g.x3_plane_a = plane_a; g.x3_plane_b = plane_b; g.x3_plane_c = plane_c;
  g.x3_products = (f16 || x3_kmajor()) ? products : 0;
  g.out_scale = out_scale; g.c_scale = c_scale;
  CDML_REQUIRE(products * g.x3_tpp % 2 == 0, CDML_E_UNSUPPORTED, "gemm_bf16x3_nt: products * K / 64 must be even");
  const KSplitPlan p = x3_plan_nt(M, N, K, products, f16, planes_out, colsum != nullptr, planes_out ? 0 : x3_slab_steps(), 6,
                                  workspace != nullptr);
  g.K = p.ktiles * 64; g.k_per_split = g.K;
  g.tiles_m = (M + 255) / 256; g.tiles_n = N / 256;
  hipStream_t s = (hipStream_t)stream;
  auto launch = [&](int epi, int n_splits) {
    return f16 ? launch_gemm_f16x2_256(g, false, epi, n_splits, s) : launch_gemm_bf16_256_x3(g, false, epi, n_splits, s);
  };
  CDML_REQUIRE(!p.slabs || (workspace_bytes >= p.need && aligned16(workspace)), CDML_E_BADARG,
               "gemm_bf16x3_nt: the slab form needs a 16-B aligned workspace of %zu bytes (cdml_gemm_bf16x3_workspace); pass "
               "NULL for the single-pass form", p.need);
  if (colsum) {
    CDML_REQUIRE(workspace && aligned16(workspace) && workspace_bytes >= p.need, CDML_E_BADARG,
                 "gemm_bf16x3_nt: colsum needs a workspace (cdml_gemm_bf16x3_workspace)");
    g.colsum_partial = reinterpret_cast<float *>(static_cast<char *>(workspace) + p.slab_bytes);
  }
  if (!p.slabs) {
    const int rc = launch(epilogue, 1);
    if (rc || !colsum) return rc;
    return x3_sum_slabs("gemm_bf16x3_nt", "bias gradient", g, p, nullptr, nullptr, 0.f, nullptr, 0, colsum, 1.0f, s);
  }
  g.k_per_split = p.per * 64;
  g.slab_stride = (int64_t)M * N;
  g.C = workspace; g.ldc = N;
  const int rc = launch(BE_F32, p.splits);
  if (rc) return rc;
  return x3_sum_slabs("gemm_bf16x3_nt", "combine", g, p, workspace, epilogue == BE_BIAS_LRELU_F32 ? bias : nullptr, alpha,
                      static_cast<float *>(C), ldc, colsum, 1.0f, s);
}

extern "C" int cdml_gemm_bf16x3_nt(int epilogue, const uint16_t *A, int64_t lda, int64_t plane_a, const uint16_t *B,
                                   int64_t ldb, int64_t plane_b, int M, int N, int K, int products, void *C,
                                   int64_t ldc, int64_t plane_c, const float *bias, const uint16_t *aux,
                                   int64_t ldaux, float alpha, float *colsum, void *workspace,
                                   size_t workspace_bytes, cdml_stream_t stream) {
  return gemm_x3_nt_impl(false, 1.0f, 1.0f, epilogue, A, lda, plane_a, B, ldb, plane_b, M, N, K, products, C, ldc, plane_c, bias, aux,
                         ldaux, alpha, colsum, workspace, workspace_bytes, stream);
}

extern "C" int cdml_gemm_f16x2_nt(int epilogue, const uint16_t *A, int64_t lda, int64_t plane_a, const uint16_t *B,
                                  int64_t ldb, int64_t plane_b, int M, int N, int K, void *C, int64_t ldc, int64_t plane_c,
                                  const float *bias, const uint16_t *aux, int64_t ldaux, float alpha, float out_scale,
                                  float c_scale, void *workspace, size_t workspace_bytes, cdml_stream_t stream) {
  return gemm_x3_nt_impl(true, out_scale, c_scale, epilogue, A, lda, plane_a, B, ldb, plane_b, M, N, K, 3, C, ldc, plane_c, bias, aux,
                         ldaux, alpha, nullptr, workspace, workspace_bytes, stream);
}

static int gemm_x3_tn_impl(bool f16, float out_scale, float cs_scale, const uint16_t *A, int64_t lda, int64_t plane_a,
                           const uint16_t *B, int64_t ldb, int64_t plane_b, int M, int N, int K, int products, float *C, int64_t ldc,
                           const float *bias, float alpha, float *colsum, void *workspace,
                           size_t workspace_bytes, cdml_stream_t stream) {
  CDML_REQUIRE(A && B && C && M > 0 && N > 0 && K > 0, CDML_E_BADARG, "gemm_bf16x3_tn: bad argument");
  const int np1 = f16 ? 1 : 2;
  CDML_REQUIRE(!f16 || (products == 3 && out_scale > 0.f && cs_scale > 0.f), CDML_E_BADARG, "gemm_f16x2_tn: positive scales");
  CDML_REQUIRE(products == 3 || products == 6, CDML_E_BADARG, "gemm_bf16x3_tn: products must be 3 or 6");
  CDML_REQUIRE(M % 256 == 0 && N % 256 == 0 && K % 128 == 0, CDML_E_UNSUPPORTED,
               "gemm_bf16x3_tn: M, N must be multiples of 256 and K of 128, got M=%d N=%d K=%d", M, N, K);
  CDML_REQUIRE(aligned16(A) && aligned16(B) && aligned16(C) && !(lda & 7) && !(ldb & 7) && !(plane_a & 7) && !(plane_b & 7) &&
                   !(ldc & 3) && plane_a >= M && plane_b >= N && lda >= np1 * plane_a + M && ldb >= np1 * plane_b + N && ldc >= N,
               CDML_E_ALIGN, "gemm_bf16x3_tn: 16-B aligned bases, strides multiples of 8, ld >= 2 plane + columns");
  CDML_REQUIRE((int64_t)K * lda * 2 < ((int64_t)1 << 31) && (int64_t)K * ldb * 2 < ((int64_t)1 << 31), CDML_E_UNSUPPORTED,
               "gemm_bf16x3_tn: an operand exceeds the 2 GiB buffer-descriptor range");
  BArgs g{};
  g.A = reinterpret_cast<const bf16 *>(A); g.lda = lda;
  g.B = reinterpret_cast<const bf16 *>(B); g.ldb = ldb;
  g.M = M; g.N = N;
  g.x3_tpp = K / 64; g.x3_plane_a = plane_a; g.x3_plane_b = plane_b;
  g.x3_products = (f16 || x3_kmajor()) ? products : 0;
  g.out_scale = out_scale; g.c_scale = 1.0f;
  const KSplitPlan p = x3_plan_tn(M, N, K, products, x3_tn_period(products, g.x3_products != 0, f16), bias != nullptr, colsum != nullptr);
  const auto launch = f16 ? +[](const BArgs &a, int splits, hipStream_t s) { return launch_gemm_f16x2_256(a, true, BE_F32, splits, s); }
                          : +[](const BArgs &a, int splits, hipStream_t s) { return launch_gemm_bf16_256_x3(a, true, BE_F32, splits, s); };
  return x3_run_tn("gemm_bf16x3_tn", g, p, launch, C, ldc, bias, alpha, colsum, cs_scale, workspace, workspace_bytes, (hipStream_t)stream);
}

extern "C" int cdml_gemm_bf16x3_tn(const uint16_t *A, int64_t lda, int64_t plane_a, const uint16_t *B, int64_t ldb,
                                   int64_t plane_b, int M, int N, int K, int products, float *C, int64_t ldc,
                                   const float *bias, float alpha, float *colsum, void *workspace,
                                   size_t workspace_bytes, cdml_stream_t stream) {
  return gemm_x3_tn_impl(false, 1.0f, 1.0f, A, lda, plane_a, B, ldb, plane_b, M, N, K, products, C, ldc, bias, alpha, colsum, workspace,
                         workspace_bytes, stream);
}

extern "C" int cdml_gemm_f16x2_tn(const uint16_t *A, int64_t lda, int64_t plane_a, const uint16_t *B, int64_t ldb,
                                  int64_t plane_b, int M, int N, int K, float *C, int64_t ldc, float out_scale, float *colsum,
                                  float colsum_scale, void *workspace, size_t workspace_bytes, cdml_stream_t stream) {
  return gemm_x3_tn_impl(true, out_scale, colsum_scale, A, lda, plane_a, B, ldb, plane_b, M, N, K, 3, C, ldc, nullptr, 0.f, colsum,
                         workspace, workspace_bytes, stream);
}

namespace cdml {
namespace {

__global__ void __launch_bounds__(kThreads)
k_mine_prep(const float *__restrict__ e_in, float *__restrict__ e_out, int64_t lde, const float *__restrict__ z, int64_t ldz,
            int B, int D, bf16 *__restrict__ e3, int64_t ld3, int64_t plane, float *__restrict__ sqn, float *__restrict__ dp,
            float h2_scale) {
  const int lane = threadIdx.x & 63, wave = threadIdx.x >> 6;
  const int nq = D >> 2;
  for (int i = blockIdx.x * (kThreads / 64) + wave; i < B; i += gridDim.x * (kThreads / 64)) {
    if (z) {
      const float *za = z + (int64_t)(2 * i) * ldz, *zp = za + ldz;
      float *ea = e_out + (int64_t)(2 * i) * lde, *ep = ea + lde;
      float s0 = 0.f, s1 = 0.f;
      for (int q = lane; q < nq; q += 64) {
        const f32x4 x = reinterpret_cast<const f32x4 *>(za)[q], y = reinterpret_cast<const f32x4 *>(zp)[q];
        s0 += x.x * x.x + x.y * x.y + x.z * x.z + x.w * x.w;
        s1 += y.x * y.x + y.y * y.y + y.z * y.z + y.w * y.w;
      }
      s0 = wave_sum(s0);
      s1 = wave_sum(s1);
      const float i0 = 1.0f / sqrtf(fmaxf(s0, 1e-12f)), i1 = 1.0f / sqrtf(fmaxf(s1, 1e-12f));
      for (int q = lane; q < nq; q += 64) {
        const f32x4 x = reinterpret_cast<const f32x4 *>(za)[q], y = reinterpret_cast<const f32x4 *>(zp)[q];
        reinterpret_cast<f32x4 *>(ea)[q] = f32x4{x.x * i0, x.y * i0, x.z * i0, x.w * i0};
        reinterpret_cast<f32x4 *>(ep)[q] = f32x4{y.x * i1, y.y * i1, y.z * i1, y.w * i1};
      }
    }
    const float *e = z ? e_out : e_in;
    const float *a = e + (int64_t)(2 * i) * lde, *p = a + lde;
    float sa = 0.f, sp = 0.f, ap = 0.f;
    for (int q = lane; q < nq; q += 64) {
      const f32x4 x = reinterpret_cast<const f32x4 *>(a)[q], y = reinterpret_cast<const f32x4 *>(p)[q];
      sa += x.x * x.x + x.y * x.y + x.z * x.z + x.w * x.w;
      sp += y.x * y.x + y.y * y.y + y.z * y.z + y.w * y.w;
      ap += x.x * y.x + x.y * y.y + x.z * y.z + x.w * y.w;
      bf16x4 h, m, l;
#pragma unroll
      for (int r = 0; r < 2; ++r) {
        const f32x4 v = r ? y : x;
        if (h2_scale > 0.f) {
          half4v hh, hl;
#pragma unroll
          for (int j = 0; j < 4; ++j) {
            _Float16 a, b;
            split2h(v[j], h2_scale, a, b);
            hh[j] = a; hl[j] = b;
          }
          _Float16 *d = reinterpret_cast<_Float16 *>(e3) + (int64_t)(2 * i + r) * ld3 + 4 * q;
          *reinterpret_cast<half4v *>(d) = hh;
          *reinterpret_cast<half4v *>(d + plane) = hl;
          continue;
        }
#pragma unroll
        for (int j = 0; j < 4; ++j) {
          bf16 b0, b1, b2;
          split3(v[j], b0, b1, b2);
          h[j] = b0; m[j] = b1; l[j] = b2;
        }
        bf16 *d = e3 + (int64_t)(2 * i + r) * ld3 + 4 * q;
        *reinterpret_cast<bf16x4 *>(d) = h;
        *reinterpret_cast<bf16x4 *>(d + plane) = m;
        *reinterpret_cast<bf16x4 *>(d + 2 * plane) = l;
      }
    }
    sa = wave_sum(sa); sp = wave_sum(sp); ap = wave_sum(ap);
    if (lane == 0) {
      sqn[2 * i] = sa;
      sqn[2 * i + 1] = sp;
      dp[i] = (sa + sp) - 2.0f * ap;
    }
  }
}

__global__ void __launch_bounds__(kThreads)
k_semihard_finish(const MineCand *__restrict__ part, int64_t ld, int n_strips, int B, int32_t *__restrict__ neg_row) {
  __shared__ MineCand red[4][64];
  const int a = blockIdx.x * 64 + (threadIdx.x & 63), grp = threadIdx.x >> 6;
  const float inf = __builtin_huge_valf();
  MineCand best{inf, 0x7fffffff, -inf, 0x7fffffff};
  auto merge = [&](const MineCand &o) {
    if (o.out_d < best.out_d || (o.out_d == best.out_d && o.out_c < best.out_c)) { best.out_d = o.out_d; best.out_c = o.out_c; }
    if (o.in_d > best.in_d || (o.in_d == best.in_d && o.in_c < best.in_c)) { best.in_d = o.in_d; best.in_c = o.in_c; }
  };
  if (a < B) {
    int s = grp;
    for (; s + 12 < n_strips; s += 16) {
      const MineCand c0 = part[(int64_t)s * ld + a], c1 = part[(int64_t)(s + 4) * ld + a];
      const MineCand c2 = part[(int64_t)(s + 8) * ld + a], c3 = part[(int64_t)(s + 12) * ld + a];
      merge(c0); merge(c1); merge(c2); merge(c3);
    }
    for (; s < n_strips; s += 4) merge(part[(int64_t)s * ld + a]);
  }
  red[grp][threadIdx.x & 63] = best;
  __syncthreads();
  if (grp == 0 && a < B) {
    merge(red[1][threadIdx.x]); merge(red[2][threadIdx.x]); merge(red[3][threadIdx.x]);
    neg_row[a] = best.out_c != 0x7fffffff ? best.out_c : (best.in_c != 0x7fffffff ? best.in_c : -1);
  }
}

}
}

extern "C" size_t cdml_semihard_mine_x3_workspace(int B) {
  if (B < 1 || (2 * (int64_t)B) % 256) return 0;
  return (size_t)(2 * B / 256) * 4 * (size_t)B * sizeof(MineCand);
// ... 145 lines not shown
```

### collaborative-deep-metric-learning_amd/csrc/gemm_plan.h

```cpp
#pragma once
#include <stddef.h>
#include <stdint.h>

namespace cdml {

constexpr int kPlanNumCU = 256;

inline int gemm_bf16_256_splits(int M, int N, int K) {
  const int64_t tiles = (int64_t)((M + 255) / 256) * (N / 256);
  const int max_by_k = K / 1024 > 0 ? K / 1024 : 1;
  int best = 1;
  double best_eff = 0.0;
  for (int s = 1; s <= 16 && s <= max_by_k; ++s) {
    const int64_t blocks = tiles * s;
    const double eff = (double)blocks / (double)(((blocks + kPlanNumCU - 1) / kPlanNumCU) * kPlanNumCU);
    if (eff > best_eff + 0.02) { best_eff = eff; best = s; }
  }
  return best;
}

inline int x3_nt_splits(int N, int ktiles, int tiles_m, int slab_steps, bool half_steps = false) {
  if (N / 256 != 1) return 1;
  if (half_steps) ktiles *= 2;
  int steps = slab_steps;
  if (steps < 12) {
    int s120 = ktiles / 120;
    s120 = s120 < 1 ? 1 : (s120 > 16 ? 16 : s120);
    steps = tiles_m * s120 <= 64 ? 60 : 120;
  }
  const int s = ktiles / steps;
  return s < 1 ? 1 : (s > 16 ? 16 : s);
}

inline void x3_split_geometry(int ktiles, int requested, int period, int &per, int &splits) {
  per = (ktiles + requested - 1) / requested;
  per = (per + period - 1) / period * period;
  splits = (ktiles + per - 1) / per;
}

struct KSplitPlan {
  int ktiles, period, per, splits;
  bool slabs;
  size_t slab_bytes, cs_rows, cs_bytes, need;
};

inline void ksplit_bytes(KSplitPlan &p, int M, int N, bool unsplit_slab, bool colsum) {
  p.slabs = p.splits > 1 || unsplit_slab;
  p.slab_bytes = p.slabs ? (size_t)p.splits * M * N * sizeof(float) : 0;
  p.cs_rows = (size_t)p.splits * ((M + 255) / 256) * 2;
  p.cs_bytes = p.cs_rows * N * sizeof(float);
  p.need = p.slab_bytes + (colsum ? p.cs_bytes : 0);
}

inline KSplitPlan ksplit_plan(int M, int N, int ktiles, int requested, int period, bool unsplit_slab, bool colsum) {
  KSplitPlan p{};
  p.ktiles = ktiles; p.period = period;
  x3_split_geometry(ktiles, requested, period, p.per, p.splits);
  ksplit_bytes(p, M, N, unsplit_slab, colsum);
  return p;
}

inline int x3_tn_period(int products, bool kmajor, bool f16) { return ((products == 6 && kmajor) || f16) ? 6 : 2; }

inline KSplitPlan x3_plan_tn(int M, int N, int K, int products, int period, bool bias, bool colsum) {
  const int ktiles = products * (K / 64);
  return ksplit_plan(M, N, ktiles, gemm_bf16_256_splits(M, N, ktiles * 64), period, bias, colsum);
}

inline KSplitPlan x3_plan_nt(int M, int N, int K, int products, bool f16, bool planes_out, bool colsum, int slab_steps,
                             int period, bool have_workspace) {
  const int ktiles = products * (K / 64);
  int requested = planes_out ? 1 : x3_nt_splits(N, ktiles, (M + 255) / 256, slab_steps, f16);
  if (requested > 1) {
    const KSplitPlan p = ksplit_plan(M, N, ktiles, requested, period, false, colsum);
    if (p.splits > 1 && have_workspace) return p;
  }
  KSplitPlan p = ksplit_plan(M, N, ktiles, 1, 1, false, colsum);
  p.period = period;
  return p;
}

inline size_t x3_workspace_bytes(int tn, int M, int N, int K, int products, int slab_steps = 0) {
  if (M <= 0 || N <= 0 || K <= 0 || (products != 3 && products != 6) || K % 64) return 0;
  size_t need = 0;
  auto take = [&](const KSplitPlan &p) { if (p.need > need) need = p.need; };
  const int periods[2] = {6, 2}, lengths[3] = {60, 120, slab_steps};
  for (int period : periods) {
    take(ksplit_plan(M, N, products * (K / 64), 1, period, true, true));
    if (tn) take(x3_plan_tn(M, N, K, products, period, true, true));
    else for (int steps : lengths) take(x3_plan_nt(M, N, K, products, false, false, true, steps, period, true));
  }
  return need + (size_t)N * sizeof(float);
}

inline KSplitPlan bf16_tn_plan(int M, int N, int K, bool colsum) {
  KSplitPlan p{};
  p.ktiles = K / 64; p.period = 2;
  p.splits = gemm_bf16_256_splits(M, N, K);
  p.per = p.splits > 1 ? ((K + p.splits - 1) / p.splits + 127) / 128 * 2 : p.ktiles;
  ksplit_bytes(p, M, N, false, colsum);
  return p;
}

}
```

### collaborative-deep-metric-learning_amd/csrc/gemm_tile.h

```cpp
#pragma once
#include "gemm_bf16.h"
#include <type_traits>
#include <utility>

namespace cdml {
namespace {

using bf16x8 = __attribute__((ext_vector_type(8))) __bf16;
using bf16x4 = __attribute__((ext_vector_type(4))) __bf16;
using f32x16 = __attribute__((ext_vector_type(16))) float;
using f32x4 = __attribute__((ext_vector_type(4))) float;
using f32x2 = __attribute__((ext_vector_type(2))) float;
using i32x4 = __attribute__((ext_vector_type(4))) int;

constexpr int kT = 512;
constexpr int kTileM = 256, kTileN = 256, kTileK = 64;
constexpr int IMG = 16384;
constexpr int BUF = 4 * IMG;
constexpr int SMEM = 2 * BUF;
constexpr int SMEM_R6 = 10 * IMG;

__device__ __forceinline__ uint32_t lds_off(const void *p) {
  return (uint32_t)(uintptr_t)(__attribute__((address_space(3))) const void *)p;
}
__device__ __forceinline__ void dma(i32x4 srd, uint32_t voff, uint32_t lds_base) {
  asm volatile("s_mov_b32 m0, %0\n\ts_nop 0\n\tbuffer_load_dwordx4 %1, %2, 0 offen lds"
               :: "s"(lds_base), "v"(voff), "s"(srd) : "memory", "m0");
}
__device__ __forceinline__ void dma_s(i32x4 srd, uint32_t voff, uint32_t soff, uint32_t lds_base) {
  asm volatile("s_mov_b32 m0, %0\n\ts_nop 0\n\tbuffer_load_dwordx4 %1, %2, %3 offen lds"
               :: "s"(lds_base), "v"(voff), "s"(srd), "s"(soff) : "memory", "m0");
}
using u32x4 = __attribute__((ext_vector_type(4))) uint32_t;
using bf16x2 = __attribute__((ext_vector_type(2))) __bf16;
#ifdef CDML_F16X2
constexpr bool kF16 = true;
using half8 = __attribute__((ext_vector_type(8))) _Float16;
using half2v = __attribute__((ext_vector_type(2))) _Float16;
#define CDML_MFMA16(a, b, c) \
  __builtin_amdgcn_mfma_f32_16x16x32_f16(__builtin_bit_cast(half8, a), __builtin_bit_cast(half8, b), c, 0, 0, 0)
__device__ __forceinline__ uint32_t pack2(float a, float b) {
  uint32_t w = __builtin_bit_cast(uint32_t, half2v{(_Float16)a, (_Float16)b});
  asm("" : "+v"(w));
  return w;
}
__device__ __forceinline__ float lo_of(uint32_t w) { return (float)__builtin_bit_cast(half2v, w)[0]; }
__device__ __forceinline__ float hi_of(uint32_t w) { return (float)__builtin_bit_cast(half2v, w)[1]; }
#else
constexpr bool kF16 = false;
#define CDML_MFMA16(a, b, c) __builtin_amdgcn_mfma_f32_16x16x32_bf16(a, b, c, 0, 0, 0)
__device__ __forceinline__ uint32_t pack2(float a, float b) {
  uint32_t w = __builtin_bit_cast(uint32_t, bf16x2{(__bf16)a, (__bf16)b});
  asm("" : "+v"(w));
  return w;
}
__device__ __forceinline__ float lo_of(uint32_t w) { return __builtin_bit_cast(float, w << 16); }
__device__ __forceinline__ float hi_of(uint32_t w) { return __builtin_bit_cast(float, w & 0xffff0000u); }
#endif
constexpr int kPlanesOut = kF16 ? 2 : 3;
__device__ __forceinline__ i32x4 make_srd(const void *base, int64_t bytes) {
  const uint64_t a = (uint64_t)(uintptr_t)base;
  i32x4 r;
  r.x = __builtin_amdgcn_readfirstlane((int)(uint32_t)a);
  r.y = __builtin_amdgcn_readfirstlane((int)(uint32_t)((a >> 32) & 0xffff));
  r.z = __builtin_amdgcn_readfirstlane((int)(bytes > 0 ? bytes : 0));
  r.w = 0x00020000;
  return r;
}

template <class F, int... I>
__device__ __forceinline__ void unroll_seq(F &&f, std::integer_sequence<int, I...>) {
  (f(std::integral_constant<int, I>{}), ...);
}
template <int N, class F>
__device__ __forceinline__ void unroll(F &&f) {
  unroll_seq(f, std::make_integer_sequence<int, N>{});
}

#define CDML_BARRIER()                         \
  do {                                         \
    __builtin_amdgcn_sched_barrier(0);         \
    asm volatile("s_barrier" ::: "memory");    \
    __builtin_amdgcn_sched_barrier(0);         \
  } while (0)

template <bool TN_, int EPI_, bool S16_, bool X3_ = false, bool F6_ = false, bool NTCS_ = false, bool R6_ = false,
          bool NARROW_ = false, bool KI_ = false, bool WIDEB_ = false>
struct Variant {
  static constexpr bool TN = TN_, S16 = S16_, X3 = X3_, F6 = F6_, NTCS = NTCS_, R6 = R6_, NARROW = NARROW_, KI = KI_, WIDEB = WIDEB_;
  static constexpr int EPI = EPI_;
  static constexpr bool KIA = KI, KIB = KI || WIDEB;
  static constexpr bool kR6 = X3 && S16 && R6;
  static constexpr bool kFast6 = X3 && S16 && F6;
  static constexpr bool kSwap = EPI == BE_MINE_X3 || EPI == BE_KNN_X3 || EPI == BE_RANK_X3;
  static constexpr bool kRowBias = EPI == BE_ROWBIAS_LRELU_X3;
  static constexpr bool kBiasEpi = EPI == BE_BIAS_LRELU_BF16 || EPI == BE_BIAS_LRELU_X3 || kRowBias;
  static constexpr bool kMaskEpi = EPI == BE_MASK_BF16 || EPI == BE_MASK_X3;
  static constexpr bool kPlanes = EPI == BE_BIAS_LRELU_X3 || EPI == BE_MASK_X3 || kRowBias;
  static constexpr int kSmem = R6 ? SMEM_R6 : SMEM;
  static_assert(!TN || EPI == BE_F32, "the k-strided form only serves the weight gradients");
  static_assert(!NARROW || (X3 && S16 && R6 && !TN && (EPI == BE_BIAS_LRELU_X3 || EPI == BE_MASK_X3 || EPI == BE_ROWBIAS_LRELU_X3 || EPI == BE_F32)),
                "the 128 x 256 half tile exists for the plane-output products of the resident-plane walk and for the fp32 slabs of the narrow layer");
  static_assert(X3 || (EPI != BE_BIAS_LRELU_X3 && EPI != BE_MASK_X3 && EPI != BE_ROWBIAS_LRELU_X3),
                "plane outputs belong to the split-fp32 form");
  static_assert((EPI != BE_MINE_X3 && EPI != BE_KNN_X3 && EPI != BE_RANK_X3) || (X3 && S16 && R6 && !TN && !NARROW),
                "the mining / kNN-filter / rank-count epilogues ride on the resident-plane walk");
  static_assert(!KI || (TN && X3 && S16 && R6), "the k8-interleaved operands exist for the k-strided resident-plane walk");
  static_assert(!WIDEB || (TN && X3 && S16 && R6 && !KI && !kF16 && !NARROW && EPI == BE_F32),
                "the wide column operand exists for the bf16 k-strided resident-plane walk");
  static_assert(!(kF16 && kR6) || (!NARROW && !KI), "the fp16 form has the full tile on row-major operands only");
};
template <bool TN, int EPI, bool S16> using PlainLoop = Variant<TN, EPI, S16>;
template <bool TN, int EPI> using X3General = Variant<TN, EPI, true, true>;
template <int EPI> using X3GeneralColsum = Variant<false, EPI, true, true, false, true>;
template <int EPI> using X3SixStep = Variant<false, EPI, true, true, true>;
template <bool TN, int EPI> using X3Resident = Variant<TN, EPI, true, true, false, false, true>;
template <int EPI> using X3ResidentHalf = Variant<false, EPI, true, true, false, false, true, true>;
using X3ResidentK8 = Variant<true, BE_F32, true, true, false, false, true, false, true>;
using X3ResidentWideB = Variant<true, BE_F32, true, true, false, false, true, false, false, true>;
using X3Mine = X3Resident<false, BE_MINE_X3>;
using X3Knn = X3Resident<false, BE_KNN_X3>;
using X3Rank = X3Resident<false, BE_RANK_X3>;

}
}
```

### collaborative-deep-metric-learning_amd/engine_x3.py

```python
import os

import torch

from . import ops
from .engine import EngineWorkspace, TowerLayout, dw1_in_blocks


def layout_x3(feature_size, hidden=5000, output_size=256):
    return TowerLayout(feature_size, hidden, output_size, pad=(256, 256, 256))


class TowerWorkspaceX3(EngineWorkspace):
    ROWS, WIDTHS, MAX_ROWS, INFERENCE, EXCHANGE_PLANES = 128, 256, 65536, "f32x3", True

    def __init__(self, layout, n_rows, device, products=6, planes_in=True, backward=True, transposed=None,
                 fc2_single_pass=False, kint=None, wide_dz1=None):
        L, R = layout, int(n_rows)
        if R % 128:
            raise ValueError("precision 'f32x3' needs a row count that is a multiple of 128 (got %d)" % R)
        if products not in (3, 6):
            raise ValueError("products must be 6 (fp32-equivalent) or 3 (16-bit operands)")
        self.layout, self.R, self.products = L, R, products
        bf = lambda *s: torch.zeros(s, dtype=torch.bfloat16, device=device)
        f32 = lambda *s: torch.zeros(s, dtype=torch.float32, device=device)
        if transposed is None:
            transposed = (os.environ.get("CDML_X3_TRANSPOSED") == "1" and backward and R % 256 == 0 and products == 6)
        if transposed and (R % 256 or not backward):
            raise ValueError("the transposed activation layout needs a training workspace with rows % 256 == 0")
        self.transposed = bool(transposed)
        maskbits = backward and not self.transposed and os.environ.get("CDML_X3_MASKBITS", "1") != "0"
        if kint is None:
            kint = os.environ.get("CDML_X3_KI", "0") == "1" and planes_in
        self.kint = bool(kint) and maskbits and products == 6 and R % 8 == 0
        self.wide_dz1 = (wide_dz1 is None or bool(wide_dz1)) and maskbits and products == 6 and R % 8 == 0 and not self.kint
        self.xk = None
        self.x3 = bf(R, 3 * L.Fp)
        self.x_hat = self.x3 if planes_in else f32(R, L.Fp)
        self.h1 = bf(L.Hp, 3 * R) if self.transposed else bf(R, 3 * L.Hp)
        self.z, self.e = f32(R, L.Dp), f32(R, L.Dp)
        self.W1T, self.W2T, self.W2 = bf(L.Hp, 3 * L.Fp), bf(L.Dp, 3 * L.Hp), bf(L.Hp, 3 * L.Dp)
        q = products
        self.fc2_single_pass = bool(fc2_single_pass) and not backward and R // 256 >= 192
        self.slab_steps = None if backward else 120
        nb = 16 if self.fc2_single_pass else max(ops.gemm_bf16x3_workspace(False, R, L.Dp, L.Hp, q), 16)
        self.h1_bits = None
        if maskbits:
            self.h1_bits = torch.zeros((R, L.Hp // 8), dtype=torch.uint8, device=device)
        if backward:
            ki = self.kint or self.wide_dz1
            self.dz1 = bf(L.Hp, 3 * R) if self.transposed else (None if ki else bf(R, 3 * L.Hp))
            self.dz1k = torch.zeros(3 * R * L.Hp, dtype=torch.bfloat16, device=device) if ki else None
            self.de, self.dz2 = f32(R, L.Dp), f32(R, L.Dp)
            self.dz2_3 = bf(R, 3 * L.Dp)
            nb = max(nb, ops.gemm_bf16x3_workspace(True, L.Fp, L.Hp, R, q), ops.gemm_bf16x3_workspace(True, L.Hp, L.Dp, R, q))
            if L.Fp % 512 == 0:
                nb = max(nb, ops.gemm_bf16x3_workspace(True, L.Fp // 2, L.Hp, R, q))
            if self.transposed:
                self.xT = bf(L.Fp, 3 * R)
                self.dz2T = bf(L.Dp, 3 * R)
                nb = max(nb, ops.gemm_bf16x3_workspace(True, R, L.Dp, L.Hp, q),
                         ops.gemm_bf16x3_workspace(False, L.Fp, L.Hp, R, q), ops.gemm_bf16x3_workspace(False, L.Hp, L.Dp, R, q))
                if L.Fp % 512 == 0:
                    nb = max(nb, ops.gemm_bf16x3_workspace(False, L.Fp // 2, L.Hp, R, q))
        self.gemm_ws = torch.empty(nb // 4, dtype=torch.float32, device=device)
        self.tail_done = False

    def tail_operands(self, indexed=False):
        return {"dz2_bf16": self.dz2_3, "plane_bf": self.layout.Dp}, True

    def miner_operands(self):
        return (3, torch.bfloat16, 0.0) if self.products == 6 else None

    def optimizer_operands(self):
        return plane_operands(self)

    def enable_row_gradient(self, p):
        L = self.layout
        if self.transposed or self.dz1 is None:
            raise ValueError("train_table needs the row-major activation layout of the f32x3 path and dz1 in it (kint=False, wide_dz1=False)")
        self.W1n = torch.zeros((L.Fp, 3 * L.Hp), dtype=torch.bfloat16, device=self.z.device)
        refresh_weights(p, self)

    def row_gradient(self, p, dxh):
        L = self.layout
        ops.gemm_bf16x3_nt(ops.BE_F32, self.dz1, L.Hp, self.W1n, L.Hp, dxh, self.R, L.Fp, L.Hp, products=self.products)

    def _sum_planes(self, t, width):
        return t[:, :width].float() + t[:, width:2 * width].float() + t[:, 2 * width:3 * width].float()

    def x_hat_f32(self):
        return self.x_hat if self.x_hat.dtype == torch.float32 else self._sum_planes(self.x_hat, self.layout.Fp)

    def dz1_f32(self):
        if self.transposed:
            return self._sum_planes(self.dz1, self.R).t().contiguous()
        if self.dz1 is None:
            v = self.dz1k.view(3, self.R // 8, self.layout.Hp, 8).permute(0, 1, 3, 2).reshape(3, self.R, self.layout.Hp)
            return v[0].float() + v[1].float() + v[2].float()
        return self._sum_planes(self.dz1, self.layout.Hp)

    def h1_f32(self):
        H, R = self.layout.Hp, self.R
        return self._sum_planes(self.h1, R).t().contiguous() if self.transposed else self._sum_planes(self.h1, H)


def plane_operands(ws):
    L = ws.layout
    w1 = {"wt": ws.W1T, "plane_t": L.Fp}
    if ws.W1n is not None:
        w1.update(wc=ws.W1n, plane_c=L.Hp)
    return w1, {"wt": ws.W2T, "plane_t": L.Hp, "wc": ws.W2, "plane_c": L.Dp}


def refresh_weights(p, ws):
    L = p.layout
    ops.split_f32_bf16x3(p.W1, ws.W1T, L.Fp, transpose=True)
    ops.split_f32_bf16x3(p.W2, ws.W2T, L.Hp, transpose=True)
    ops.split_f32_bf16x3(p.W2, ws.W2, L.Dp)
    if ws.W1n is not None:
        ops.split_f32_bf16x3(p.W1, ws.W1n, L.Hp)


def tower_forward(p, ws, normalize=True):
    L, R, q = p.layout, ws.R, ws.products
    if ws.x_hat.dtype == torch.float32:
        ops.split_f32_bf16x3(ws.x_hat, ws.x3, L.Fp)
    else:
        ws.x3 = ws.x_hat
    if ws.transposed:
        ops.gemm_bf16x3_nt(ops.BE_ROWBIAS_LRELU_X3, ws.W1T, L.Fp, ws.x3, L.Fp, ws.h1, L.Hp, R, L.Fp, products=q,
                           plane_c=R, bias=p.b1)
        ops.gemm_bf16x3_tn(ws.h1, R, ws.W2, L.Dp, ws.z, R, L.Dp, L.Hp, products=q, workspace=ws.gemm_ws, bias=p.b2)
    else:
        if ws.h1_bits is not None:
            ops.gemm_bf16x3_nt(ops.BE_BIAS_LRELU_X3_BITS, ws.x3, L.Fp, ws.W1T, L.Fp, ws.h1, R, L.Hp, L.Fp, products=q,
                               plane_c=L.Hp, bias=p.b1, aux=ws.h1_bits)
        else:
            ops.gemm_bf16x3_nt(ops.BE_BIAS_LRELU_X3, ws.x3, L.Fp, ws.W1T, L.Fp, ws.h1, R, L.Hp, L.Fp, products=q,
                               plane_c=L.Hp, bias=p.b1)
        ops.gemm_bf16x3_nt(ops.BE_BIAS_LRELU_F32, ws.h1, L.Hp, ws.W2T, L.Hp, ws.z, R, L.Dp, L.Hp, products=q,
                           bias=p.b2, workspace=None if ws.fc2_single_pass else ws.gemm_ws,
                           slab_steps=ws.slab_steps)
    ws.tail_done = False
    ws.dz2_planes_done = False
    if normalize:
        ops.l2norm_fwd(ws.z, L.Dp, ws.e)
    return ws.e


def tower_backward(p, ws, after_w1=None, w1_chunks=1, after_w1_chunk=None):
    L, R, q = p.layout, ws.R, ws.products
    if not ws.tail_done:
        ops.l2norm_bwd(ws.z, ws.de, L.Dp, ws.dz2, lrelu_alpha=ops.LRELU_ALPHA)
    if not (ws.tail_done and ws.dz2_planes_done):
        ops.split_f32_bf16x3(ws.dz2, ws.dz2_3, L.Dp)
    T = ws.transposed
    if T:
        ops.split_f32_bf16x3(ws.dz2, ws.dz2T, R, transpose=True)
        w2 = lambda: ops.gemm_bf16x3_nt(ops.BE_F32, ws.h1, R, ws.dz2T, R, p.gW2, L.Hp, L.Dp, R, products=q,
                                        workspace=ws.gemm_ws, colsum=p.gb2)
    else:
        w2 = lambda: ops.gemm_bf16x3_tn(ws.h1, L.Hp, ws.dz2_3, L.Dp, p.gW2, L.Hp, L.Dp, R, products=q,
                                        workspace=ws.gemm_ws, colsum=p.gb2)
    single = after_w1 is None and after_w1_chunk is None
    if single:
        w2()
    if T:
        ops.gemm_bf16x3_nt(ops.BE_MASK_X3, ws.W2, L.Dp, ws.dz2_3, L.Dp, ws.dz1, L.Hp, R, L.Dp, products=q, plane_c=R,
                           aux=ws.h1)
        for pl in range(3):
            ops.transpose_to_bf16(ws.x3[:, pl * L.Fp:(pl + 1) * L.Fp], ws.xT[:, pl * R:(pl + 1) * R], R, L.Fp)
    else:
        kint = ws.kint and ws.xk is not None and ws.h1_bits is not None
        if ws.kint and not kint:
            raise RuntimeError("this workspace holds dz1 k8-interleaved only: it needs the gather's interleaved x_hat (ws.xk) and "
                               "the sign bitmask of h1 (CDML_X3_MASKBITS); build it with kint=False otherwise")
        if kint or ws.wide_dz1:
            ops.gemm_bf16x3_nt(ops.BE_MASKBITS_X3_KI, ws.dz2_3, L.Dp, ws.W2, L.Dp, ws.dz1k, R, L.Hp, L.Dp, products=q,
                               plane_c=R * L.Hp, aux=ws.h1_bits, ldc=L.Hp)
        elif ws.h1_bits is not None:
            ops.gemm_bf16x3_nt(ops.BE_MASKBITS_X3, ws.dz2_3, L.Dp, ws.W2, L.Dp, ws.dz1, R, L.Hp, L.Dp, products=q,
                               plane_c=L.Hp, aux=ws.h1_bits)
        else:
            ops.gemm_bf16x3_nt(ops.BE_MASK_X3, ws.dz2_3, L.Dp, ws.W2, L.Dp, ws.dz1, R, L.Hp, L.Dp, products=q, plane_c=L.Hp,
                               aux=ws.h1)

    def dw1(lo, hi, db):
        if T:
            ops.gemm_bf16x3_nt(ops.BE_F32, ws.xT[lo:hi], R, ws.dz1, R, p.gW1[lo:hi], hi - lo, L.Hp, R, products=q,
                               workspace=ws.gemm_ws, colsum=db)
        elif ws.kint:
            ops.gemm_bf16x3_tnk(ws.xk, L.Fp, lo, ws.dz1k, L.Hp, 0, p.gW1[lo:hi], hi - lo, L.Hp, R, workspace=ws.gemm_ws, colsum=db)
        elif ws.wide_dz1:
            ops.gemm_bf16x3_tn(ws.x3[:, lo:], L.Fp, ws.dz1k, L.Hp, p.gW1[lo:hi], hi - lo, L.Hp, R, products=q,
                               workspace=ws.gemm_ws, colsum=db, b_kint=(L.Hp, 0))
        else:
            ops.gemm_bf16x3_tn(ws.x3[:, lo:], L.Fp, ws.dz1, L.Hp, p.gW1[lo:hi], hi - lo, L.Hp, R, products=q,
                               workspace=ws.gemm_ws, colsum=db)
    dw1_in_blocks(p, dw1, w1_chunks, after_w1_chunk, lambda rows: rows % 256 == 0)
    if after_w1 is not None:
        after_w1()
    if not single:
        w2()
    return p.grad
```

### collaborative-deep-metric-learning_amd/ops.py

```python
import ctypes as C

import torch

from ._lib import call, load_library

LRELU_ALPHA = 0.2


def _stream():
    return C.c_void_p(torch.cuda.current_stream().cuda_stream)


def _p(t, dtype=None):
    if t is None:
        return C.c_void_p(0)
    if not t.is_cuda:
        raise ValueError("cdml ops need device tensors (there is no CPU path)")
    if dtype is not None and t.dtype != dtype:
        raise ValueError(f"expected {dtype}, got {t.dtype}")
    return C.c_void_p(t.data_ptr())


def _mat(t, dtype=torch.float32):
    if t.dim() != 2 or t.stride(1) != 1:
        raise ValueError("expected a 2-D tensor with unit inner stride")
    return _p(t, dtype), t.stride(0)


def version():
    return load_library().cdml_version()


def fill_uniform_table(table, row0, feature_size, seed):
    ptr, ld = _mat(table)
    call("cdml_fill_uniform_table", ptr, row0, table.shape[0], feature_size, ld, seed, _stream())
    return table


def sample_uniform(pairs, n_rows, seed, step, batch, idx_out, slot0=0, batch_global=None,
                   step_dev=None):
    bg = batch if batch_global is None else batch_global
    call("cdml_sample_uniform", _p(pairs, torch.int32), pairs.shape[0], n_rows, seed,
         0 if step is None else step, _p(step_dev, torch.int64), batch, slot0, bg,
         _p(idx_out, torch.int32), _stream())
    return idx_out


def sample_inbatch(pairs, seed, step, batch, rows_out, shift_out, slot0=0, batch_global=None,
                   step_dev=None):
    bg = batch if batch_global is None else batch_global
    call("cdml_sample_inbatch", _p(pairs, torch.int32), pairs.shape[0], seed,
         0 if step is None else step, _p(step_dev, torch.int64), batch, slot0, bg,
         _p(rows_out, torch.int32), _p(shift_out, torch.int32), _stream())
    return rows_out, shift_out


def step_advance(step_dev):
    call("cdml_step_advance", _p(step_dev, torch.int64), _stream())


def gather_rows(table, row0, idx, feature_size, x_out, normalize=True, inv_norm_out=None,
                oob_flag=None, nan_missing=False):
    tp, tld = _mat(table)
    xp, xld = _mat(x_out)
    call("cdml_gather_rows", tp, row0, table.shape[0], tld, _p(idx, torch.int32), idx.numel(),
         feature_size, (1 if normalize else 0) | (2 if nan_missing else 0), xp, xld, _p(inv_norm_out),
         _p(oob_flag, torch.int32), _stream())
    return x_out


def gather_rows_x3(src, idx, feature_size, x_out_planes, nan_missing=False, oob_flag=None):
    sp, sld = _mat(src)
    xp, xld = _mat16(x_out_planes)
    call("cdml_gather_rows_x3", sp, src.shape[0], sld, _p(idx, torch.int32), idx.numel(), feature_size, 2 if nan_missing else 0,
         xp, xld, _p(oob_flag, torch.int32), _stream())
    return x_out_planes


def _gather_format(table, x_out):
    if table.dtype == torch.float16:
        return "_f16"
    if table.dtype == torch.float8_e4m3fn:
        return "_f8"
    return {torch.bfloat16: "_x3", torch.float16: "_h2"}.get(x_out.dtype, "")


def _gather_io(fmt, table, x_out, idx_out, n_steps, x_ki, x_ki_errors, kind_out=None, batch=0, lists=None):
    tp, tld = {"_f16": _mat16, "_f8": _mat8}.get(fmt, _mat)(table)
    listed = None if lists is None else _lists_args(lists[0], table.shape[0], lists[1])
    omat = _mat16 if fmt else _mat
    if n_steps > 1:
        if x_out.dim() != 3 or idx_out.dim() != 2 or x_out.shape[0] != n_steps or idx_out.shape[0] != n_steps:
            raise ValueError("n_steps > 1 needs x_out [n_steps, rows, stride] and idx_out [n_steps, rows]")
        if kind_out is not None and (kind_out.dim() != 2 or kind_out.shape[0] != n_steps or kind_out.stride(1) != 1):
            raise ValueError("n_steps > 1 needs kind_out [n_steps, batch]")
        xp, xld = omat(x_out[0])
        xss, iss = x_out.stride(0), idx_out.stride(0)
        kss = kind_out.stride(0) if kind_out is not None else 0
    else:
        xp, xld = omat(x_out)
        xss = iss = kss = 0
    if kind_out is not None and kind_out.numel() < n_steps * batch:
        raise ValueError("kind_out needs one int32 per triplet")
    kis = 0
    if x_ki is not None:
        if fmt != "_x3":
            raise ValueError(x_ki_errors[0])
        if x_ki.dtype != torch.bfloat16 or not x_ki.is_contiguous():
            raise ValueError(x_ki_errors[1])
        kis = x_ki.stride(0) if (n_steps > 1 and x_ki.dim() > 1) else 0
    return (tp, tld), (xp, xld), (xss, iss, kss, kis), listed


def sample_gather(mode, pairs, seed, step, batch, table, feature_size, idx_out, x_out,
                  shift_out=None, slot0=0, batch_global=None, step_dev=None, n_steps=1, oob_flag=None, x_ki=None):
    bg = batch if batch_global is None else batch_global
    fmt = _gather_format(table, x_out)
    (tp, tld), (xp, xld), (xss, iss, _, kis), _ = _gather_io(
        fmt, table, x_out, idx_out, n_steps, x_ki, ("x_ki goes with the three-plane output and must be a contiguous bf16 buffer",) * 2)
    ki = () if x_ki is None else (C.c_void_p(x_ki.data_ptr()), kis)
    call("cdml_sample_gather" + (fmt if x_ki is None else "_x3k"), mode, _p(pairs, torch.int32), pairs.shape[0], seed,
         0 if step is None else step, _p(step_dev, torch.int64), batch, slot0, bg, tp,
         table.shape[0], tld, feature_size, _p(idx_out, torch.int32), _p(shift_out, torch.int32),
         xp, xld, n_steps, xss, iss, _p(oob_flag, torch.int32), *ki, _stream())
    return x_out


def hard_threshold(hard_fraction):
    h = float(hard_fraction)
    if not 0.0 <= h <= 1.0:
        raise ValueError("hard_fraction must be in [0, 1], got %r" % (hard_fraction,))
    return int(round(h * 4294967296.0))


def _lists_args(lists, n_rows, hard_fraction):
    if lists.dim() != 2 or lists.stride(1) != 1 or lists.shape[0] != n_rows or lists.shape[1] < 1:
        raise ValueError("negative lists must be an int32 [n_rows = %d, L >= 1] tensor with unit inner stride, got %s"
                         % (n_rows, tuple(lists.shape)))
    return _p(lists, torch.int32), lists.stride(0), lists.shape[1], hard_threshold(hard_fraction)


def sample_listed(pairs, n_rows, seed, step, batch, lists, hard_fraction, idx_out, kind_out=None, slot0=0, batch_global=None,
                  step_dev=None):
    bg = batch if batch_global is None else batch_global
    lp, ldl, L, thresh = _lists_args(lists, n_rows, hard_fraction)
    call("cdml_sample_listed", _p(pairs, torch.int32), pairs.shape[0], n_rows, seed, 0 if step is None else step,
         _p(step_dev, torch.int64), batch, slot0, bg, lp, ldl, L, thresh, _p(idx_out, torch.int32), _p(kind_out, torch.int32),
         _stream())
    return idx_out


def sample_gather_listed(pairs, seed, step, batch, table, feature_size, lists, hard_fraction, idx_out, x_out, kind_out=None,
                         slot0=0, batch_global=None, step_dev=None, n_steps=1, oob_flag=None, x_ki=None):
# ... 1514 lines not shown
def knn_desim_prep(fI, fD, fI_end, threshold, out):
    if fI.dtype not in (torch.int32, torch.int64):
        raise ValueError("fI must be int32 or int64")
    fp, fld = _mat(fI, fI.dtype)
    dp, dld = _mat(fD)
    op, _ = _mat(out, torch.int32)
    if not out.is_contiguous() or out.shape[0] != fI.shape[0] or fD.shape[0] != fI.shape[0]:
        raise ValueError("fI, fD and out must have the same rows (out contiguous)")
    call("cdml_knn_desim_prep", fp, int(fI.dtype == torch.int64), fld, dp, dld, fI.shape[0], int(fI_end), float(threshold),
         op, out.shape[1], _stream())
    return out


def knn_desim(eI, f_filtered, out, query_id=None, row0=0):
    ep, eld = _mat(eI, torch.int32)
    op, old = _mat(out, torch.int32)
    fp, _ = _mat(f_filtered, torch.int32)
    if not f_filtered.is_contiguous() or out.shape[0] < eI.shape[0] or out.shape[1] < eI.shape[1]:
        raise ValueError("f_filtered must be contiguous and out at least eI's shape")
    if query_id is not None and (not query_id.is_contiguous() or query_id.numel() < eI.shape[0]):
        raise ValueError("query_id must be a contiguous int32 vector of nq ids")
    call("cdml_knn_desim", ep, eld, eI.shape[0], eI.shape[1], _p(query_id, torch.int32), int(row0), fp, f_filtered.shape[1],
         f_filtered.shape[0], op, old, _stream())
    return out


def _knn_lines_args(D, I, row0, guid_off):
    if D.dim() != 2 or tuple(D.shape) != tuple(I.shape):
        raise ValueError("D and I of one shape [n, k]")
    dp, dld = _mat(D)
    ip, ild = _mat(I, torch.int64)
    if not guid_off.is_contiguous() or guid_off.dim() != 1 or guid_off.numel() < 2:
        raise ValueError("guid_off must be a contiguous int64 vector of n_guid + 1 offsets")
    return dp, dld, ip, ild, int(row0), D.shape[0], D.shape[1], _p(guid_off, torch.int64), guid_off.numel() - 1


def knn_line_sizes(D, I, row0, guid_off, guid_total, sizes, flags):
    a = _knn_lines_args(D, I, row0, guid_off)
    if sizes.numel() < D.shape[0] or flags.numel() < D.shape[0] or not sizes.is_contiguous() or not flags.is_contiguous():
        raise ValueError("sizes and flags: contiguous vectors of n entries")
    call("cdml_knn_line_sizes", *a, int(guid_total), _p(sizes, torch.int64), _p(flags, torch.int32), _stream())
    return sizes, flags


def knn_line_write(D, I, row0, guid_bytes, guid_off, off, out):
    a = _knn_lines_args(D, I, row0, guid_off)
    if off.numel() < D.shape[0] + 1 or not off.is_contiguous() or not out.is_contiguous() or not guid_bytes.is_contiguous():
        raise ValueError("off: a contiguous vector of n + 1 entries; out and guid_bytes contiguous")
    call("cdml_knn_line_write", *a[:7], _p(guid_bytes, torch.uint8), a[7], a[8], guid_bytes.numel(), _p(off, torch.int64),
         _p(out, torch.uint8), out.numel(), _stream())
    return out


EW_MUL, EW_MUL_RES, EW_ADD = 0, 1, 2


def ew_combine(mode, a, b, out, M, N):
    ap, ald = _mat(a)
    bp, bld = _mat(b)
    op, old = _mat(out)
    call("cdml_ew_combine", mode, ap, ald, bp, bld, M, N, op, old, _stream())
    return out


def ew_fusion_bwd(residual, g, a, b, da, db, M, N, alpha=LRELU_ALPHA):
    gp, gld = _mat(g)
    ap, ald = _mat(a)
    bp, bld = _mat(b)
    dap, dald = _mat(da)
    dbp, dbld = _mat(db)
    call("cdml_ew_fusion_bwd", 1 if residual else 0, gp, gld, ap, ald, bp, bld, M, N, alpha, dap, dald,
         dbp, dbld, _stream())


def lrelu_bwd(g, y, out, M, N, alpha=LRELU_ALPHA):
    gp, gld = _mat(g)
    yp, yld = _mat(y)
    op, old = _mat(out)
    call("cdml_lrelu_bwd", gp, gld, yp, yld, M, N, alpha, op, old, _stream())
    return out


BE_BIAS_LRELU_BF16, BE_BIAS_LRELU_F32, BE_MASK_BF16, BE_F32 = 0, 1, 2, 3
BE_BIAS_LRELU_BF16_BITS, BE_MASKBITS_BF16 = 4, 5


def gemm_bf16_epilogue_supported(epilogue, M, N, K, lda, ldb, ldc, ldaux):
    return bool(load_library().cdml_gemm_bf16_epilogue_supported(epilogue, M, N, K, lda, ldb, ldc, ldaux))


def _mat16(t):
    if t.dim() != 2 or t.stride(1) != 1 or t.element_size() != 2:
        raise ValueError("expected a 2-D 16-bit tensor with unit inner stride")
    return _p(t), t.stride(0)


def _mat8(t):
    if t.dim() != 2 or t.stride(1) != 1 or t.dtype != torch.float8_e4m3fn:
        raise ValueError("expected a 2-D float8_e4m3fn tensor with unit inner stride")
    return _p(t), t.stride(0)


def gemm_bf16_workspace(M, N, K):
    return int(load_library().cdml_gemm_bf16_workspace(M, N, K))


def gemm_bf16_nt(epilogue, A, B, C, M, N, K, bias=None, aux=None, alpha=LRELU_ALPHA, workspace=None):
    ap, ald = _mat16(A)
    bp, bld = _mat16(B)
    if C.dim() != 2 or C.stride(1) != 1:
        raise ValueError("C must be 2-D with unit inner stride")
    xld = aux.stride(0) if aux is not None else 0
    if aux is not None and (aux.dtype == torch.uint8) != (epilogue in (BE_BIAS_LRELU_BF16_BITS, BE_MASKBITS_BF16)):
        raise ValueError("epilogues 4 / 5 take a uint8 bitmask as aux, epilogue 2 bf16 values")
    call("cdml_gemm_bf16_nt", epilogue, ap, ald, bp, bld, M, N, K, _p(C), C.stride(0), _p(bias),
         _p(aux), xld, alpha, _p(workspace), 0 if workspace is None else workspace.numel() * workspace.element_size(),
         _stream())
    return C


def gemm_bf16_tn_supported(M, N, K, lda, ldb):
    return bool(load_library().cdml_gemm_bf16_tn_supported(M, N, K, lda, ldb))


def gemm_bf16_tn_workspace(M, N, K):
    return int(load_library().cdml_gemm_bf16_tn_workspace(M, N, K))


def gemm_bf16_tn(A, B, C, M, N, K, workspace=None, colsum=None):
    ap, ald = _mat16(A)
    bp, bld = _mat16(B)
    cp, cld = _mat(C)
    call("cdml_gemm_bf16_tn", ap, ald, bp, bld, M, N, K, cp, cld, _p(colsum, torch.float32), _p(workspace),
         0 if workspace is None else workspace.numel() * workspace.element_size(), _stream())
    return C


BE_BIAS_LRELU_X3, BE_MASK_X3, BE_ROWBIAS_LRELU_X3 = 6, 7, 8
BE_BIAS_LRELU_X3_BITS, BE_MASKBITS_X3 = 9, 10
BE_MASKBITS_X3_KI = 12


def split_f32_bf16x3(src, dst, plane, transpose=False):
    sp, sld = _mat(src)
    dp, dld = _mat16(dst)
    call("cdml_split_f32_bf16x3", sp, sld, src.shape[0], src.shape[1], dp, dld, plane, 1 if transpose else 0, _stream())
    return dst


def gemm_bf16x3_workspace(tn, M, N, K, products=6):
    return int(load_library().cdml_gemm_bf16x3_workspace(1 if tn else 0, M, N, K, products))


def gemm_bf16x3_nt(epilogue, A, plane_a, B, plane_b, C, M, N, K, products=6, plane_c=0, bias=None, aux=None,
                   alpha=LRELU_ALPHA, workspace=None, colsum=None, ldc=None, slab_steps=None):
    if slab_steps:
        lib = load_library()
        prev = lib.cdml_x3_slab_steps(int(slab_steps))
        try:
            return gemm_bf16x3_nt(epilogue, A, plane_a, B, plane_b, C, M, N, K, products=products, plane_c=plane_c, bias=bias,
                                  aux=aux, alpha=alpha, workspace=workspace, colsum=colsum, ldc=ldc)
        finally:
            lib.cdml_x3_slab_steps(prev)
    ap, ald = _mat16(A)
    bp, bld = _mat16(B)
    if epilogue == BE_MASKBITS_X3_KI:
        if ldc is None or not C.is_contiguous() or C.dtype != torch.bfloat16:
            raise ValueError("epilogue 12 writes a contiguous bf16 buffer and needs ldc (columns per row group)")
    elif C.dim() != 2 or C.stride(1) != 1:
        raise ValueError("C must be 2-D with unit inner stride")
    if aux is not None and (aux.dtype == torch.uint8) != (epilogue in (BE_BIAS_LRELU_X3_BITS, BE_MASKBITS_X3, BE_MASKBITS_X3_KI)):
        raise ValueError("epilogues 9 / 10 / 12 take a uint8 bitmask as aux, epilogue 7 bf16 values")
    call("cdml_gemm_bf16x3_nt", epilogue, ap, ald, plane_a, bp, bld, plane_b, M, N, K, products, _p(C), C.stride(0) if ldc is None else ldc,
         plane_c, _p(bias), _p(aux), aux.stride(0) if aux is not None else 0, alpha, _p(colsum, torch.float32),
         _p(workspace), 0 if workspace is None else workspace.numel() * workspace.element_size(), _stream())
    return C


def interleave8_bf16x3(src, plane_src, rows, cols, dst):
    sp, sld = _mat16(src)
    if dst.dtype != torch.bfloat16 or not dst.is_contiguous() or dst.numel() < 3 * rows * cols:
        raise ValueError("interleave8_bf16x3: dst must be a contiguous bf16 buffer of 3 * rows * cols elements")
    call("cdml_interleave8_bf16x3", sp, sld, plane_src, rows, cols, C.c_void_p(dst.data_ptr()), _stream())
    return dst


def gemm_bf16x3_tnk(A, ma, a_col0, B, nb, b_col0, out, M, N, K, workspace=None, colsum=None):
    cp, cld = _mat(out)
    ws, wb = (C.c_void_p(0), 0) if workspace is None else (C.c_void_p(workspace.data_ptr()), workspace.numel() * workspace.element_size())
    call("cdml_gemm_bf16x3_tnk", C.c_void_p(A.data_ptr()), ma, a_col0, C.c_void_p(B.data_ptr()), nb, b_col0, M, N, K, cp, cld,
         _p(colsum, torch.float32), ws, wb, _stream())
    return out


def gemm_bf16x3_tn_kb(A, plane_a, B, nb, b_col0, out, M, N, K, workspace=None, colsum=None):
    ap, ald = _mat16(A)
    cp, cld = _mat(out)
    ws, wb = (C.c_void_p(0), 0) if workspace is None else (C.c_void_p(workspace.data_ptr()), workspace.numel() * workspace.element_size())
    call("cdml_gemm_bf16x3_tn_kb", ap, ald, plane_a, C.c_void_p(B.data_ptr()), nb, b_col0, M, N, K, cp, cld,
         _p(colsum, torch.float32), ws, wb, _stream())
    return out


def gemm_bf16x3_tn(A, plane_a, B, plane_b, C, M, N, K, products=6, workspace=None, colsum=None, bias=None,
                   alpha=LRELU_ALPHA, b_kint=None):
    if b_kint is not None:
        if products != 6 or bias is not None:
            raise ValueError("gemm_bf16x3_tn: the interleaved B operand takes six products and no bias")
        return gemm_bf16x3_tn_kb(A, plane_a, B, b_kint[0], b_kint[1], C, M, N, K, workspace=workspace, colsum=colsum)
    ap, ald = _mat16(A)
    bp, bld = _mat16(B)
    cp, cld = _mat(C)
    call("cdml_gemm_bf16x3_tn", ap, ald, plane_a, bp, bld, plane_b, M, N, K, products, cp, cld, _p(bias), alpha,
         _p(colsum, torch.float32), _p(workspace),
         0 if workspace is None else workspace.numel() * workspace.element_size(), _stream())
    return C


def split_f32_f16x2(src, dst, plane, scale, transpose=False):
    sp, sld = _mat(src)
    dp, dld = _mat16(dst)
    call("cdml_split_f32_f16x2", sp, sld, src.shape[0], src.shape[1], dp, dld, plane, 1 if transpose else 0, float(scale), _stream())
    return dst


def gemm_f16x2_workspace(tn, M, N, K):
    return int(load_library().cdml_gemm_f16x2_workspace(1 if tn else 0, M, N, K))


def gemm_f16x2_nt(epilogue, A, plane_a, B, plane_b, C, M, N, K, out_scale, c_scale=1.0, plane_c=0, bias=None, aux=None,
                  alpha=LRELU_ALPHA, workspace=None, slab_steps=None):
    if slab_steps:
        lib = load_library()
        prev = lib.cdml_x3_slab_steps(int(slab_steps))
        try:
            return gemm_f16x2_nt(epilogue, A, plane_a, B, plane_b, C, M, N, K, out_scale, c_scale=c_scale, plane_c=plane_c,
                                 bias=bias, aux=aux, alpha=alpha, workspace=workspace)
        finally:
            lib.cdml_x3_slab_steps(prev)
    ap, ald = _mat16(A)
    bp, bld = _mat16(B)
    if C.dim() != 2 or C.stride(1) != 1:
        raise ValueError("C must be 2-D with unit inner stride")
    if aux is not None and (aux.dtype == torch.uint8) != (epilogue in (BE_BIAS_LRELU_X3_BITS, BE_MASKBITS_X3)):
        raise ValueError("epilogues 9 / 10 take a uint8 bitmask as aux, epilogue 7 16-bit values")
    call("cdml_gemm_f16x2_nt", epilogue, ap, ald, plane_a, bp, bld, plane_b, M, N, K, _p(C), C.stride(0), plane_c, _p(bias),
         _p(aux), aux.stride(0) if aux is not None else 0, alpha, float(out_scale), float(c_scale), _p(workspace),
         0 if workspace is None else workspace.numel() * workspace.element_size(), _stream())
    return C


def gemm_f16x2_tn(A, plane_a, B, plane_b, C, M, N, K, out_scale, workspace=None, colsum=None, colsum_scale=1.0):
    ap, ald = _mat16(A)
    bp, bld = _mat16(B)
    cp, cld = _mat(C)
    call("cdml_gemm_f16x2_tn", ap, ald, plane_a, bp, bld, plane_b, M, N, K, cp, cld, float(out_scale), _p(colsum, torch.float32),
         float(colsum_scale), _p(workspace), 0 if workspace is None else workspace.numel() * workspace.element_size(), _stream())
    return C


def gemm_bf16_tn2_workspace(M1, N1, M2, N2, K):
    return int(load_library().cdml_gemm_bf16_tn2_workspace(M1, N1, M2, N2, K))


def gemm_bf16_tn2(A1, B1, C1, M1, N1, A2, B2, C2, M2, N2, K, workspace, colsum1=None, colsum2=None):
    a1, lda1 = _mat16(A1)
    b1, ldb1 = _mat16(B1)
    c1, ldc1 = _mat(C1)
    a2, lda2 = _mat16(A2)
    b2, ldb2 = _mat16(B2)
    c2, ldc2 = _mat(C2)
    call("cdml_gemm_bf16_tn2", a1, lda1, b1, ldb1, M1, N1, c1, ldc1, _p(colsum1, torch.float32), a2, lda2, b2, ldb2,
         M2, N2, c2, ldc2, _p(colsum2, torch.float32), K, _p(workspace), workspace.numel() * workspace.element_size(),
         _stream())


def transpose_to_bf16(src, dst, rows, cols):
    call("cdml_transpose_to_bf16", 1 if src.dtype == torch.float32 else 0, _p(src), src.stride(0), rows, cols,
         _p(dst, torch.bfloat16), dst.stride(0), _stream())
    return dst


def cast_f32_bf16(src, dst, rows, cols):
    call("cdml_cast_f32_bf16", _p(src, torch.float32), src.stride(0), rows, cols, _p(dst, torch.bfloat16),
         dst.stride(0), _stream())
    return dst


def colsum_workspace_floats(rows, cols):
    return int(load_library().cdml_colsum_workspace_floats(rows, cols))


def colsum(src, rows, cols, out, workspace):
    call("cdml_colsum", 1 if src.dtype == torch.bfloat16 else 0, _p(src), src.stride(0), rows, cols,
         _p(out, torch.float32), _p(workspace, torch.float32), _stream())
    return out


def fill_uniform_table_f16(table, row0, feature_size, seed):
    call("cdml_fill_uniform_table_f16", _p(table, torch.float16), row0, table.shape[0], feature_size,
         table.stride(0), seed, _stream())
    return table


def gather_rows_f16(table, row0, idx, feature_size, x_out, oob_flag=None):
    call("cdml_gather_rows_f16", _p(table, torch.float16), row0, table.shape[0], table.stride(0),
         _p(idx, torch.int32), idx.numel(), feature_size, _p(x_out, torch.bfloat16), x_out.stride(0),
         _p(oob_flag, torch.int32), _stream())
    return x_out


def gather_rows_f8(table, row0, idx, feature_size, x_out, oob_flag=None):
    tp, tld = _mat8(table)
    call("cdml_gather_rows_f8", tp, row0, table.shape[0], tld, _p(idx, torch.int32), idx.numel(), feature_size,
         _p(x_out, torch.bfloat16), x_out.stride(0), _p(oob_flag, torch.int32), _stream())
    return x_out


def quantize_rows_f8(src, feature_size, codes, scale):
    if src.dim() != 2 or src.stride(1) != 1 or src.dtype not in (torch.float32, torch.float16):
        raise ValueError("quantize_rows_f8 needs a 2-D fp32 or fp16 source with unit inner stride")
    cp, cld = _mat8(codes)
    if codes.shape[0] != src.shape[0] or scale.numel() != src.shape[0] or not scale.is_contiguous():
        raise ValueError("quantize_rows_f8 needs one row of codes and one contiguous fp32 scale per source row")
    call("cdml_quantize_rows_f8_" + ("f32" if src.dtype == torch.float32 else "f16"), _p(src), src.shape[0], src.stride(0),
         feature_size, cp, cld, codes.shape[1], _p(scale, torch.float32), _stream())
# ... 119 lines not shown
```

Before: 3.044 million.

## Trim zero-padded K tail in bf16x3 NT GEMMs via valid-K argument

```diff
diff --git a/__graft_entry__.py b/__graft_entry__.py
--- a/__graft_entry__.py
+++ b/__graft_entry__.py
@@ -121,7 +121,7 @@
             + list(_lib.SIGNATURES_HARDNEG) + list(_lib.SIGNATURES_WIDE) + list(_lib.SIGNATURES_NEGW) \
             + list(_lib.SIGNATURES_F8) + list(_lib.SIGNATURES_IVF) + list(_lib.SIGNATURES_IVF_F16) \
             + list(_lib.SIGNATURES_IVF_FILTER) + list(_lib.SIGNATURES_KNN_WRITER) + list(_lib.SIGNATURES_IVF_PQ) \
-            + list(_lib.SIGNATURES_IVF_PQR):
+            + list(_lib.SIGNATURES_IVF_PQR) + list(_lib.SIGNATURES_KTRIM):
         getattr(lib, name)
     assert lib.cdml_build_id().decode() == "CDML_BUILD_ID=" + sid
     print("[build] ok:", LIB, "version", lib.cdml_version(), lib.cdml_build_id().decode())
diff --git a/collaborative-deep-metric-learning_amd/_lib.py b/collaborative-deep-metric-learning_amd/_lib.py
--- a/collaborative-deep-metric-learning_amd/_lib.py
+++ b/collaborative-deep-metric-learning_amd/_lib.py
@@ -292,6 +292,12 @@
     "cdml_ivf_scan_pqr": (_i, [_p, _i, _p, _p, _p, _p, _p, _i64, _p, _i, _p, _i, _p, _p]),
 }
 
+SIGNATURES_KTRIM = {
+    "cdml_gemm_bf16x3_nt_kv": (_i, [_i, _p, _i64, _i64, _p, _i64, _i64, _i, _i, _i, _i, _i, _p, _i64, _i64, _p, _p, _i64, _f,
+                                    _p, _p, _sz, _p]),
+    "cdml_x3_ktrim_ksteps": (_i, [_i, _i, _i]),
+}
+
 _lib = None
 
 
@@ -311,7 +317,7 @@
                                + list(SIGNATURES_NEGW.items()) + list(SIGNATURES_F8.items()) + list(SIGNATURES_IVF.items())
                                + list(SIGNATURES_IVF_F16.items()) + list(SIGNATURES_IVF_FILTER.items())
                                + list(SIGNATURES_KNN_WRITER.items()) + list(SIGNATURES_IVF_PQ.items())
-                               + list(SIGNATURES_IVF_PQR.items())):
+                               + list(SIGNATURES_IVF_PQR.items()) + list(SIGNATURES_KTRIM.items())):
         fn = getattr(lib, name)
         fn.restype = res
         fn.argtypes = args
diff --git a/collaborative-deep-metric-learning_amd/csrc/gemm_bf16.h b/collaborative-deep-metric-learning_amd/csrc/gemm_bf16.h
--- a/collaborative-deep-metric-learning_amd/csrc/gemm_bf16.h
+++ b/collaborative-deep-metric-learning_amd/csrc/gemm_bf16.h
@@ -33,6 +33,7 @@
   int aux_bits;
   int x3_tpp;
   int x3_products;
+  int k_valid;
   int64_t x3_plane_a, x3_plane_b, x3_plane_c;
   int grid_tiles, narrow_first;
   int stagger_lead;
diff --git a/collaborative-deep-metric-learning_amd/csrc/gemm_bf16_256.hip b/collaborative-deep-metric-learning_amd/csrc/gemm_bf16_256.hip
--- a/collaborative-deep-metric-learning_amd/csrc/gemm_bf16_256.hip
+++ b/collaborative-deep-metric-learning_amd/csrc/gemm_bf16_256.hip
@@ -17,6 +17,7 @@
   constexpr int EPI = V::EPI;
   constexpr bool KIA = V::KIA, KIB = V::KIB, kSwap = V::kSwap, kR6 = V::kR6, kFast6 = V::kFast6;
   constexpr bool kRowBias = V::kRowBias, kBiasEpi = V::kBiasEpi, kMaskEpi = V::kMaskEpi, kPlanes = V::kPlanes;
+  constexpr bool kKTrim = V::kKTrim;
   const int t = threadIdx.x;
   const int lane = t & 63;
   const int wave = __builtin_amdgcn_readfirstlane(t >> 6);
@@ -231,7 +232,12 @@
       asm volatile("" : "+v"(fb0[0]), "+v"(fb0[1]), "+v"(fb0[2]), "+v"(fb0[3]),
                         "+v"(fb1[0]), "+v"(fb1[1]), "+v"(fb1[2]), "+v"(fb1[3]));
   };
-  auto load_b16 = [&](auto rd) {
+  auto pin_a1 = [&]() { asm volatile("" : "+v"(fa[0][0]), "+v"(fa[0][1]), "+v"(fa[0][2]), "+v"(fa[0][3])); };
+  auto pin_b1 = [&]() { asm volatile("" : "+v"(fb0[0]), "+v"(fb0[2]), "+v"(fb1[0]), "+v"(fb1[2])); };
+  using KSteps2 = std::integral_constant<int, 2>;
+  using KSteps1 = std::integral_constant<int, 1>;
+  auto load_b16_n = [&](auto rd, auto nksc) {
+    constexpr int NKS = decltype(nksc)::value;
     if constexpr (WIDEB) {
 #pragma unroll
       for (int hh = 0; hh < 2; ++hh)
@@ -243,18 +249,20 @@
 #pragma unroll
       for (int cb = 0; cb < 2; ++cb)
 #pragma unroll
-        for (int ks2 = 0; ks2 < 2; ++ks2) {
+        for (int ks2 = 0; ks2 < NKS; ++ks2) {
           fb0[2 * cb + ks2] = rd(0, cb, ks2);
           fb1[2 * cb + ks2] = rd(1, cb, ks2);
         }
     }
   };
-  auto load_a16 = [&](auto rd) {
-#pragma unroll
-    for (int ks2 = 0; ks2 < 2; ++ks2)
+  auto load_b16 = [&](auto rd) { load_b16_n(rd, KSteps2{}); };
+  auto load_a16_n = [&](auto rd, auto nksc) {
+#pragma unroll
+    for (int ks2 = 0; ks2 < decltype(nksc)::value; ++ks2)
 #pragma unroll
       for (int rb = 0; rb < (WIDEB ? 2 : 4); ++rb) fa[ks2][rb] = rd(rb, ks2);
   };
+  auto load_a16 = [&](auto rd) { load_a16_n(rd, KSteps2{}); };
   auto sum_b16 = [&](auto add) {
     if constexpr (WIDEB) {
 #pragma unroll
@@ -271,7 +279,8 @@
         }
     }
   };
-  auto mfma16 = [&](const int r0) {
+  auto mfma16_n = [&](const int r0, auto nksc) {
+    constexpr int NKS = decltype(nksc)::value;
     __builtin_amdgcn_s_setprio(1);
     if constexpr (WIDEB) {
 #pragma unroll
@@ -285,7 +294,7 @@
               acc16[r0 + 2 * hh + rb][cb] = CDML_MFMA16(fa[ks2][rb], fbx[hh * 8 + cb * 2 + ks2], acc16[r0 + 2 * hh + rb][cb]);
     } else {
 #pragma unroll
-      for (int ks2 = 0; ks2 < 2; ++ks2)
+      for (int ks2 = 0; ks2 < NKS; ++ks2)
 #pragma unroll
         for (int rb = 0; rb < 4; ++rb)
 #pragma unroll
@@ -301,6 +310,7 @@
     }
     __builtin_amdgcn_s_setprio(0);
   };
+  auto mfma16 = [&](const int r0) { mfma16_n(r0, KSteps2{}); };
   auto do_tile2_s16 = [&](const int buf, const int tile) {
     load_b16([&](int hh, int cb, int ks2) { return read_b16(buf, hh, cb, ks2); });
     load_a16([&](int rb, int ks2) { return read_a16(buf, 0, rb, ks2); });
@@ -428,6 +438,8 @@
     const int n_per = n_ktiles / kPer;
     if (n_per > 0) {
       const int w_first = x3_t0 / kPer, w_last = w_first + n_per - 1;
+      const bool half_last = kKTrim && n_per > 1 && g.k_valid > 0 && (w_last + 1) * kTileK - g.k_valid >= kTileK / 2;
+      const int w_full = half_last ? w_last - 1 : w_last;
       const uint32_t ws_a = KIA ? (uint32_t)(8 * g.lda * 2) : TN ? (uint32_t)(kTileK * g.lda * 2) : (uint32_t)(kTileK * 2);
       const uint32_t ws_b = KIB ? (uint32_t)(8 * g.ldb * 2) : TN ? (uint32_t)(kTileK * g.ldb * 2) : (uint32_t)(kTileK * 2);
       const uint32_t ps_a = (uint32_t)(g.x3_plane_a * 2), ps_b = (uint32_t)(g.x3_plane_b * 2);
@@ -471,6 +483,13 @@
         else
           return tr_read(smem + slot * 2 * IMG + hh * IMG + ks2 * 8192, tb_w[cb][0], tb_w[cb][1]);
       };
+      int trim_off = 0;
+      auto rd_a1 = [&](int slot, int hh, int rb, int ks2) {
+        return *reinterpret_cast<const bf16x8 *>(a16_rd + trim_off + slot * 2 * IMG + hh * IMG + rb * 2048 + sw16[ks2]);
+      };
+      auto rd_b1 = [&](int slot, int hh, int cb, int ks2) {
+        return *reinterpret_cast<const bf16x8 *>(b16r + trim_off + slot * 2 * IMG + hh * IMG + cb * 2048 + sw16[ks2]);
+      };
       uint32_t va_h1[2] = {va[0] + d_a, va[1] + d_a}, vb_h1[2] = {vb[0] + d_b, vb[1] + d_b};
       auto issue = [&](int img, int pl, int hh, int slot, uint32_t kw) {
         const uint32_t so = (img == 0 ? pl * ps_a : pl * ps_b) + kw + ((img == 0 ? KIA : KIB) ? hh * 2048u : TN ? hh * 256u : 0u);
@@ -542,19 +561,23 @@
         if (++w > w_last) break;
       }
       } else if constexpr (!NARROW) {
-      auto phase = [&](auto phc, auto parc, const uint32_t kwa_c, const uint32_t kwb_c, const uint32_t kwa_n,
+      auto phase = [&](auto phc, auto parc, auto nksc, auto partc, const uint32_t kwa_c, const uint32_t kwb_c, const uint32_t kwa_n,
                        const uint32_t kwb_n, const bool own) {
-        constexpr int PH = decltype(phc)::value, PAR = decltype(parc)::value;
+        constexpr int PH = decltype(phc)::value, PAR = decltype(parc)::value, PART = decltype(partc)::value;
+        constexpr bool kFullK = decltype(nksc)::value == 2;
         constexpr int S = PH >> 1, HALF = PH & 1;
         constexpr int PA[6] = {0, 1, 2, 0, 1, 0}, PB[6] = {0, 0, 0, 1, 1, 2};
         constexpr int SLOT_A[2][3] = {{0, 1, 2}, {2, 1, 0}};
         constexpr int sa = SLOT_A[PAR][PA[S]];
         constexpr bool rdB = HALF == 0 && (S == 0 || S == 3 || S == 5);
+        if constexpr (PART != 2) {
         if constexpr (rdB) {
           constexpr int sb = (PB[S] & 1) ^ PAR;
-          load_b16([&](int hh, int cb, int ks2) { return rd_b(sb, hh, cb, ks2); });
-        }
-        load_a16([&](int rb, int ks2) { return rd_a(sa, HALF, rb, ks2); });
+          if constexpr (kFullK) load_b16_n([&](int hh, int cb, int ks2) { return rd_b(sb, hh, cb, ks2); }, nksc);
+          else load_b16_n([&](int hh, int cb, int ks2) { return rd_b1(sb, hh, cb, ks2); }, nksc);
+        }
+        if constexpr (kFullK) load_a16_n([&](int rb, int ks2) { return rd_a(sa, HALF, rb, ks2); }, nksc);
+        else load_a16_n([&](int rb, int ks2) { return rd_a1(sa, HALF, rb, ks2); }, nksc);
         if constexpr (PH == 0) issue(0, 2, 1, SLOT_A[PAR][2], kwa_c);
         if constexpr (PH == 1) issue(1, 1, 0, 1 ^ PAR, kwb_c);
         if constexpr (PH == 2) issue(1, 1, 1, 1 ^ PAR, kwb_c);
@@ -567,11 +590,18 @@
         if constexpr (PH == 9) issue(0, 1, 0, 1, kwa_n);
         if constexpr (PH == 10) issue(0, 1, 1, 1, kwa_n);
         if constexpr (PH == 11) issue(0, 2, 0, SLOT_A[PAR ^ 1][2], kwa_n);
+        }
+        if constexpr (PART != 1) {
         constexpr int VM[12] = {8, 8, 8, 8, 8, 6, 8, 10, 12, 10, 12, 6};
         asm volatile("s_waitcnt vmcnt(%0)" :: "n"(VM[PH]) : "memory");
-        if constexpr (rdB) pin_b();
-        pin_a();
-        if constexpr (rdB) {
+        if constexpr (kFullK) {
+          if constexpr (rdB) pin_b();
+          pin_a();
+        } else {
+          if constexpr (rdB) pin_b1();
+          pin_a1();
+        }
+        if constexpr (rdB && kFullK) {
           if constexpr (WIDEB) {
             if (own && (wc >> 1) == 0) sum_b16(dot_sum);
           } else {
@@ -579,14 +609,25 @@
           }
         }
         CDML_BARRIER();
-        mfma16(4 * HALF);
+        mfma16_n(4 * HALF, nksc);
         CDML_BARRIER();
+        }
+      };
+      using Par0 = std::integral_constant<int, 0>;
+      using Par1 = std::integral_constant<int, 1>;
+      auto period_t = [&](const bool odd, const int w) {
+        const uint32_t kwa_c = (uint32_t)w * ws_a, kwb_c = (uint32_t)w * ws_b;
+        unroll<12>([&](auto phc) {
+          if (odd) phase(phc, Par1{}, KSteps1{}, Par1{}, kwa_c, kwb_c, kwa_c, kwb_c, false);
+          else phase(phc, Par0{}, KSteps1{}, Par1{}, kwa_c, kwb_c, kwa_c, kwb_c, false);
+          phase(phc, Par0{}, KSteps1{}, std::integral_constant<int, 2>{}, kwa_c, kwb_c, kwa_c, kwb_c, false);
+        });
       };
       auto period = [&](auto parc, const int w, const bool own) {
         const int wn = min(w + 1, w_last);
         const uint32_t kwa_c = (uint32_t)w * ws_a, kwb_c = (uint32_t)w * ws_b;
         const uint32_t kwa_n = (uint32_t)wn * ws_a, kwb_n = (uint32_t)wn * ws_b;
-        unroll<12>([&](auto phc) { phase(phc, parc, kwa_c, kwb_c, kwa_n, kwb_n, own); });
+        unroll<12>([&](auto phc) { phase(phc, parc, KSteps2{}, Par0{}, kwa_c, kwb_c, kwa_n, kwb_n, own); });
       };
       {
         const uint32_t ka = (uint32_t)w_first * ws_a, kb_ = (uint32_t)w_first * ws_b;
@@ -599,6 +640,19 @@
       CDML_BARRIER();
       if (grp == 1) CDML_BARRIER();
       int cs_wait = __builtin_amdgcn_readfirstlane(cs_on ? (2 * tm + grp + cs_period - w_first % cs_period) % cs_period : 0x40000000);
+      if constexpr (kKTrim) {
+        int w = w_first;
+        for (;;) {
+          period(std::integral_constant<int, 0>{}, w, false);
+          if (++w > w_full) break;
+          period(std::integral_constant<int, 1>{}, w, false);
+          if (++w > w_full) break;
+        }
+        if (half_last) {
+          asm volatile("" : "+v"(trim_off));
+          period_t(((w - w_first) & 1) != 0, w);
+        }
+      } else {
       for (int w = w_first;;) {
         bool own = cs_wait == 0;
         cs_wait = own ? cs_period - 1 : cs_wait - 1;
@@ -608,6 +662,7 @@
         cs_wait = own ? cs_period - 1 : cs_wait - 1;
         period(std::integral_constant<int, 1>{}, w, own);
         if (++w > w_last) break;
+      }
       }
       } else {
       auto rd_an = [&](int slot, int rb, int ks2) {
@@ -624,13 +679,14 @@
         dma_s(img == 0 ? srd_a : srd_b, img == 0 ? va[0] : (h1 ? vb_h1[0] : vb[0]), so, dst);
         dma_s(img == 0 ? srd_a : srd_b, img == 0 ? va[1] : (h1 ? vb_h1[1] : vb[1]), so, dst + 1024);
       };
-      auto phase_n = [&](auto sc, auto parc, const uint32_t kwb_c, const uint32_t kwa_n, const uint32_t kwb_n) {
+      auto phase_n = [&](auto sc, auto parc, auto nksc, const uint32_t kwb_c, const uint32_t kwa_n, const uint32_t kwb_n) {
         constexpr int S = decltype(sc)::value, PAR = decltype(parc)::value;
+        constexpr bool kFullK = decltype(nksc)::value == 2;
         constexpr int PA[6] = {0, 1, 2, 0, 1, 0}, PB[6] = {0, 0, 0, 1, 1, 2};
         constexpr int NSLOT_A[2][3] = {{0, 1, 2}, {3, 2, 1}};
         constexpr bool rdB = S == 0 || S == 3 || S == 5;
-        if constexpr (rdB) load_b16([&](int hh, int cb, int ks2) { return rd_bn(PB[S], hh, cb, ks2); });
-        load_a16([&](int rb, int ks2) { return rd_an(NSLOT_A[PAR][PA[S]], rb, ks2); });
+        if constexpr (rdB) load_b16_n([&](int hh, int cb, int ks2) { return rd_bn(PB[S], hh, cb, ks2); }, nksc);
+        load_a16_n([&](int rb, int ks2) { return rd_an(NSLOT_A[PAR][PA[S]], rb, ks2); }, nksc);
         if constexpr (S == 0) { issue_n(1, 2, 0, 2, kwb_c); issue_n(1, 2, 1, 2, kwb_c); }
         if constexpr (S == 1) { issue_n(1, 0, 0, 0, kwb_n); issue_n(0, 0, 0, NSLOT_A[PAR ^ 1][0], kwa_n); }
         if constexpr (S == 2) { issue_n(1, 0, 1, 0, kwb_n); }
@@ -639,17 +695,23 @@
         if constexpr (S == 5) { issue_n(0, 2, 0, NSLOT_A[PAR ^ 1][2], kwa_n); }
         constexpr int NVM[6] = {10, 8, 10, 12, 12, 8};
         asm volatile("s_waitcnt vmcnt(%0)" :: "n"(NVM[S]) : "memory");
-        if constexpr (rdB) pin_b();
-        pin_a();
+        if constexpr (kFullK) {
+          if constexpr (rdB) pin_b();
+          pin_a();
+        } else {
+          if constexpr (rdB) pin_b1();
+          pin_a1();
+        }
         CDML_BARRIER();
-        mfma16(0);
+        mfma16_n(0, nksc);
         CDML_BARRIER();
       };
-      auto period_n = [&](auto parc, const int w) {
+      auto period_nk = [&](auto parc, auto nksc, const int w) {
         const int wn = min(w + 1, w_last);
         const uint32_t kwb_c = (uint32_t)w * ws_b, kwa_n = (uint32_t)wn * ws_a, kwb_n = (uint32_t)wn * ws_b;
-        unroll<6>([&](auto sc) { phase_n(sc, parc, kwb_c, kwa_n, kwb_n); });
+        unroll<6>([&](auto sc) { phase_n(sc, parc, nksc, kwb_c, kwa_n, kwb_n); });
       };
+      auto period_n = [&](auto parc, const int w) { period_nk(parc, KSteps2{}, w); };
       {
         const uint32_t ka = (uint32_t)w_first * ws_a, kb_ = (uint32_t)w_first * ws_b;
         issue_n(1, 0, 0, 0, kb_); issue_n(0, 0, 0, 0, ka);
@@ -661,11 +723,25 @@
       }
       CDML_BARRIER();
       if (grp == 1) CDML_BARRIER();
+      if constexpr (kKTrim) {
+        int w = w_first;
+        for (;;) {
+          period_n(std::integral_constant<int, 0>{}, w);
+          if (++w > w_full) break;
+          period_n(std::integral_constant<int, 1>{}, w);
+          if (++w > w_full) break;
+        }
+        if (half_last) {
+          if ((w - w_first) & 1) period_nk(std::integral_constant<int, 1>{}, KSteps1{}, w);
+          else period_nk(std::integral_constant<int, 0>{}, KSteps1{}, w);
+        }
+      } else {
       for (int w = w_first;;) {
         period_n(std::integral_constant<int, 0>{}, w);
         if (++w > w_last) break;
         period_n(std::integral_constant<int, 1>{}, w);
         if (++w > w_last) break;
+      }
       }
       }
       if (grp == 0) CDML_BARRIER();
diff --git a/collaborative-deep-metric-learning_amd/csrc/gemm_bf16x3.hip b/collaborative-deep-metric-learning_amd/csrc/gemm_bf16x3.hip
--- a/collaborative-deep-metric-learning_amd/csrc/gemm_bf16x3.hip
+++ b/collaborative-deep-metric-learning_amd/csrc/gemm_bf16x3.hip
@@ -1,5 +1,6 @@
 #include "gemm_bf16.h"
 #include "../../include/cdml_x3_wide.h"
+#include "../../include/cdml_x3_ktrim.h"
 #include <stdlib.h>
 
 namespace cdml {
@@ -268,11 +269,12 @@
 }
 
 static int gemm_x3_nt_impl(bool f16, float out_scale, float c_scale, int epilogue, const uint16_t *A, int64_t lda, int64_t plane_a,
-                           const uint16_t *B, int64_t ldb, int64_t plane_b, int M, int N, int K, int products, void *C,
+                           const uint16_t *B, int64_t ldb, int64_t plane_b, int M, int N, int K, int k_valid, int products, void *C,
                            int64_t ldc, int64_t plane_c, const float *bias, const uint16_t *aux,
                            int64_t ldaux, float alpha, float *colsum, void *workspace,
                            size_t workspace_bytes, cdml_stream_t stream) {
   CDML_REQUIRE(A && B && C && M > 0 && N > 0 && K > 0, CDML_E_BADARG, "gemm_bf16x3_nt: bad argument");
+  CDML_REQUIRE(k_valid > 0 && k_valid <= K, CDML_E_BADARG, "gemm_bf16x3_nt_kv: k_valid must be in 1 .. K, got %d (K=%d)", k_valid, K);
   const int np1 = f16 ? 1 : 2;
   CDML_REQUIRE(!f16 || (products == 3 && epilogue != BE_MASKBITS_X3_KI && epilogue != BE_ROWBIAS_LRELU_X3 && !colsum &&
                         out_scale > 0.f && c_scale > 0.f),
@@ -319,8 +321,15 @@
   g.x3_products = (f16 || x3_kmajor()) ? products : 0;
   g.out_scale = out_scale; g.c_scale = c_scale;
   CDML_REQUIRE(products * g.x3_tpp % 2 == 0, CDML_E_UNSUPPORTED, "gemm_bf16x3_nt: products * K / 64 must be even");
-  const KSplitPlan p = x3_plan_nt(M, N, K, products, f16, planes_out, colsum != nullptr, planes_out ? 0 : x3_slab_steps(), 6,
-                                  workspace != nullptr);
+  KSplitPlan p = x3_plan_nt(M, N, K, products, f16, planes_out, colsum != nullptr, planes_out ? 0 : x3_slab_steps(), 6,
+                            workspace != nullptr);
+  const KTrim trim = x3_ktrim(K, k_valid, products, !f16 && !p.slabs && !colsum);
+  if (trim.tiles < g.x3_tpp) {
+    g.x3_tpp = trim.tiles;
+    p = ksplit_plan(M, N, products * trim.tiles, 1, 1, false, false);
+    p.period = 6;
+  }
+  g.k_valid = trim.half ? k_valid : 64 * trim.tiles;
   g.K = p.ktiles * 64; g.k_per_split = g.K;
   g.tiles_m = (M + 255) / 256; g.tiles_n = N / 256;
   hipStream_t s = (hipStream_t)stream;
@@ -354,15 +363,29 @@
                                    int64_t ldc, int64_t plane_c, const float *bias, const uint16_t *aux,
                                    int64_t ldaux, float alpha, float *colsum, void *workspace,
                                    size_t workspace_bytes, cdml_stream_t stream) {
-  return gemm_x3_nt_impl(false, 1.0f, 1.0f, epilogue, A, lda, plane_a, B, ldb, plane_b, M, N, K, products, C, ldc, plane_c, bias, aux,
+  return gemm_x3_nt_impl(false, 1.0f, 1.0f, epilogue, A, lda, plane_a, B, ldb, plane_b, M, N, K, K, products, C, ldc, plane_c, bias, aux,
                          ldaux, alpha, colsum, workspace, workspace_bytes, stream);
+}
+
+extern "C" int cdml_gemm_bf16x3_nt_kv(int epilogue, const uint16_t *A, int64_t lda, int64_t plane_a, const uint16_t *B,
+                                      int64_t ldb, int64_t plane_b, int M, int N, int K, int k_valid, int products, void *C,
+                                      int64_t ldc, int64_t plane_c, const float *bias, const uint16_t *aux,
+                                      int64_t ldaux, float alpha, float *colsum, void *workspace,
+                                      size_t workspace_bytes, cdml_stream_t stream) {
+  return gemm_x3_nt_impl(false, 1.0f, 1.0f, epilogue, A, lda, plane_a, B, ldb, plane_b, M, N, K, k_valid, products, C, ldc, plane_c, bias,
+                         aux, ldaux, alpha, colsum, workspace, workspace_bytes, stream);
+}
+
+extern "C" int cdml_x3_ktrim_ksteps(int K, int k_valid, int products) {
+  if (K <= 0 || K % 64 || k_valid <= 0 || k_valid > K || (products != 3 && products != 6) || (products * (K / 64)) % 2) return -1;
+  return x3_ktrim_ksteps(x3_ktrim(K, k_valid, products, true));
 }
 
 extern "C" int cdml_gemm_f16x2_nt(int epilogue, const uint16_t *A, int64_t lda, int64_t plane_a, const uint16_t *B,
                                   int64_t ldb, int64_t plane_b, int M, int N, int K, void *C, int64_t ldc, int64_t plane_c,
                                   const float *bias, const uint16_t *aux, int64_t ldaux, float alpha, float out_scale,
                                   float c_scale, void *workspace, size_t workspace_bytes, cdml_stream_t stream) {
-  return gemm_x3_nt_impl(true, out_scale, c_scale, epilogue, A, lda, plane_a, B, ldb, plane_b, M, N, K, 3, C, ldc, plane_c, bias, aux,
+  return gemm_x3_nt_impl(true, out_scale, c_scale, epilogue, A, lda, plane_a, B, ldb, plane_b, M, N, K, K, 3, C, ldc, plane_c, bias, aux,
                          ldaux, alpha, nullptr, workspace, workspace_bytes, stream);
 }
 
diff --git a/collaborative-deep-metric-learning_amd/csrc/gemm_plan.h b/collaborative-deep-metric-learning_amd/csrc/gemm_plan.h
--- a/collaborative-deep-metric-learning_amd/csrc/gemm_plan.h
+++ b/collaborative-deep-metric-learning_amd/csrc/gemm_plan.h
@@ -80,6 +80,18 @@
   return p;
 }
 
+struct KTrim { int tiles; bool half; };
+inline KTrim x3_ktrim(int K, int k_valid, int products, bool trimmable) {
+  KTrim t{K / 64, false};
+  if (!trimmable || k_valid <= 0 || k_valid >= K) return t;
+  int tiles = (k_valid + 63) / 64;
+  if ((products * tiles) % 2) ++tiles;
+  t.tiles = tiles < t.tiles ? tiles : t.tiles;
+  t.half = products == 6 && t.tiles >= 2 && t.tiles * 64 - k_valid >= 32;
+  return t;
+}
+inline int x3_ktrim_ksteps(const KTrim &t) { return 2 * t.tiles - (t.half ? 1 : 0); }
+
 inline size_t x3_workspace_bytes(int tn, int M, int N, int K, int products, int slab_steps = 0) {
   if (M <= 0 || N <= 0 || K <= 0 || (products != 3 && products != 6) || K % 64) return 0;
   size_t need = 0;
diff --git a/collaborative-deep-metric-learning_amd/csrc/gemm_tile.h b/collaborative-deep-metric-learning_amd/csrc/gemm_tile.h
--- a/collaborative-deep-metric-learning_amd/csrc/gemm_tile.h
+++ b/collaborative-deep-metric-learning_amd/csrc/gemm_tile.h
@@ -97,6 +97,8 @@
   static constexpr bool kBiasEpi = EPI == BE_BIAS_LRELU_BF16 || EPI == BE_BIAS_LRELU_X3 || kRowBias;
   static constexpr bool kMaskEpi = EPI == BE_MASK_BF16 || EPI == BE_MASK_X3;
   static constexpr bool kPlanes = EPI == BE_BIAS_LRELU_X3 || EPI == BE_MASK_X3 || kRowBias;
+  static constexpr bool kKTrim = kR6 && !TN && !kF16 &&
+                                 (EPI == BE_BIAS_LRELU_X3 || EPI == BE_ROWBIAS_LRELU_X3 || EPI == BE_F32);
   static constexpr int kSmem = R6 ? SMEM_R6 : SMEM;
   static_assert(!TN || EPI == BE_F32, "the k-strided form only serves the weight gradients");
   static_assert(!NARROW || (X3 && S16 && R6 && !TN && (EPI == BE_BIAS_LRELU_X3 || EPI == BE_MASK_X3 || EPI == BE_ROWBIAS_LRELU_X3 || EPI == BE_F32)),
diff --git a/collaborative-deep-metric-learning_amd/engine_x3.py b/collaborative-deep-metric-learning_amd/engine_x3.py
--- a/collaborative-deep-metric-learning_amd/engine_x3.py
+++ b/collaborative-deep-metric-learning_amd/engine_x3.py
@@ -83,7 +83,8 @@
 
     def row_gradient(self, p, dxh):
         L = self.layout
-        ops.gemm_bf16x3_nt(ops.BE_F32, self.dz1, L.Hp, self.W1n, L.Hp, dxh, self.R, L.Fp, L.Hp, products=self.products)
+        ops.gemm_bf16x3_nt(ops.BE_F32, self.dz1, L.Hp, self.W1n, L.Hp, dxh, self.R, L.Fp, L.Hp, products=self.products,
+                           k_valid=L.H)
 
     def _sum_planes(self, t, width):
         return t[:, :width].float() + t[:, width:2 * width].float() + t[:, 2 * width:3 * width].float()
@@ -129,15 +130,15 @@
         ws.x3 = ws.x_hat
     if ws.transposed:
         ops.gemm_bf16x3_nt(ops.BE_ROWBIAS_LRELU_X3, ws.W1T, L.Fp, ws.x3, L.Fp, ws.h1, L.Hp, R, L.Fp, products=q,
-                           plane_c=R, bias=p.b1)
+                           plane_c=R, bias=p.b1, k_valid=L.F)
         ops.gemm_bf16x3_tn(ws.h1, R, ws.W2, L.Dp, ws.z, R, L.Dp, L.Hp, products=q, workspace=ws.gemm_ws, bias=p.b2)
     else:
         if ws.h1_bits is not None:
             ops.gemm_bf16x3_nt(ops.BE_BIAS_LRELU_X3_BITS, ws.x3, L.Fp, ws.W1T, L.Fp, ws.h1, R, L.Hp, L.Fp, products=q,
-                               plane_c=L.Hp, bias=p.b1, aux=ws.h1_bits)
+                               plane_c=L.Hp, bias=p.b1, aux=ws.h1_bits, k_valid=L.F)
         else:
             ops.gemm_bf16x3_nt(ops.BE_BIAS_LRELU_X3, ws.x3, L.Fp, ws.W1T, L.Fp, ws.h1, R, L.Hp, L.Fp, products=q,
-                               plane_c=L.Hp, bias=p.b1)
+                               plane_c=L.Hp, bias=p.b1, k_valid=L.F)
         ops.gemm_bf16x3_nt(ops.BE_BIAS_LRELU_F32, ws.h1, L.Hp, ws.W2T, L.Hp, ws.z, R, L.Dp, L.Hp, products=q,
                            bias=p.b2, workspace=None if ws.fc2_single_pass else ws.gemm_ws,
                            slab_steps=ws.slab_steps)
diff --git a/collaborative-deep-metric-learning_amd/ops.py b/collaborative-deep-metric-learning_amd/ops.py
--- a/collaborative-deep-metric-learning_amd/ops.py
+++ b/collaborative-deep-metric-learning_amd/ops.py
@@ -1,4 +1,5 @@
 import ctypes as C
+import os
 
 import torch
 
@@ -1819,16 +1820,26 @@
     return int(load_library().cdml_gemm_bf16x3_workspace(1 if tn else 0, M, N, K, products))
 
 
+def x3_ktrim():
+    return os.environ.get("CDML_X3_KTRIM", "1") != "0"
+
+
+def x3_ktrim_ksteps(K, k_valid, products=6):
+    return int(load_library().cdml_x3_ktrim_ksteps(K, k_valid, products))
+
+
 def gemm_bf16x3_nt(epilogue, A, plane_a, B, plane_b, C, M, N, K, products=6, plane_c=0, bias=None, aux=None,
-                   alpha=LRELU_ALPHA, workspace=None, colsum=None, ldc=None, slab_steps=None):
+                   alpha=LRELU_ALPHA, workspace=None, colsum=None, ldc=None, slab_steps=None, k_valid=None):
     if slab_steps:
         lib = load_library()
         prev = lib.cdml_x3_slab_steps(int(slab_steps))
         try:
             return gemm_bf16x3_nt(epilogue, A, plane_a, B, plane_b, C, M, N, K, products=products, plane_c=plane_c, bias=bias,
-                                  aux=aux, alpha=alpha, workspace=workspace, colsum=colsum, ldc=ldc)
+                                  aux=aux, alpha=alpha, workspace=workspace, colsum=colsum, ldc=ldc, k_valid=k_valid)
         finally:
             lib.cdml_x3_slab_steps(prev)
+    if k_valid is None or not x3_ktrim():
+        k_valid = K
     ap, ald = _mat16(A)
     bp, bld = _mat16(B)
     if epilogue == BE_MASKBITS_X3_KI:
@@ -1838,7 +1849,7 @@
         raise ValueError("C must be 2-D with unit inner stride")
     if aux is not None and (aux.dtype == torch.uint8) != (epilogue in (BE_BIAS_LRELU_X3_BITS, BE_MASKBITS_X3, BE_MASKBITS_X3_KI)):
         raise ValueError("epilogues 9 / 10 / 12 take a uint8 bitmask as aux, epilogue 7 bf16 values")
-    call("cdml_gemm_bf16x3_nt", epilogue, ap, ald, plane_a, bp, bld, plane_b, M, N, K, products, _p(C), C.stride(0) if ldc is None else ldc,
+    call("cdml_gemm_bf16x3_nt_kv", epilogue, ap, ald, plane_a, bp, bld, plane_b, M, N, K, k_valid, products, _p(C), C.stride(0) if ldc is None else ldc,
          plane_c, _p(bias), _p(aux), aux.stride(0) if aux is not None else 0, alpha, _p(colsum, torch.float32),
          _p(workspace), 0 if workspace is None else workspace.numel() * workspace.element_size(), _stream())
     return C
diff --git a/include/cdml_x3_ktrim.h b/include/cdml_x3_ktrim.h
--- /dev/null
+++ b/include/cdml_x3_ktrim.h
@@ -0,0 +1,16 @@
+#ifndef CDML_X3_KTRIM_H
+#define CDML_X3_KTRIM_H
+#include "cdml.h"
+#ifdef __cplusplus
+extern "C" {
+#endif
+int cdml_gemm_bf16x3_nt_kv(int epilogue, const uint16_t *A, int64_t lda, int64_t plane_a, const uint16_t *B,
+                           int64_t ldb, int64_t plane_b, int M, int N, int K, int k_valid, int products, void *C,
+                           int64_t ldc, int64_t plane_c, const float *bias, const uint16_t *aux,
+                           int64_t ldaux, float alpha, float *colsum, void *workspace,
+                           size_t workspace_bytes, cdml_stream_t stream);
+int cdml_x3_ktrim_ksteps(int K, int k_valid, int products);
+#ifdef __cplusplus
+}
+#endif
+#endif
```

Result: no change. 3.058 million, median of 6 (+0.5%).
